# neel-dey/anatomix

Measured on AMD Instinct MI355X. Metric: 128^3 volumes/sec feature-extraction (6M UNet), higher is better.
Workload: dtype f16; 1 GPU; anatomix 6M UNet (ngf=16,num_downs=4) forward on sw_batch=4 windows of 1x128^3 (the predictor call of sliding_window_inference, BASELINE configs[1] / the metric); fp32 NCDHW in/out, 16-bit (f16) channels-last activations, fp32 accumulate; holds the 1e-3 tolerance against the fp32 reference in rel-L2 ONLY (max-norm 0.86e-3 .. 1.4e-3 by weight seed; the mode that holds both norms is value_strict); batch_per_gpu=4, window=128, parallelism=replicas x1 (no data-path collective)

## Files before the change

anatomix_amd/_lib.py:

```python
from __future__ import annotations

import ctypes as C
import os

_HERE = os.path.dirname(os.path.abspath(__file__))
LIB_PATH = os.environ.get("AMX_LIB_PATH") or os.path.join(_HERE, "csrc", "libanatomix_amd.so")

NORM = {"none": 0, "batch": 1, "instance": 2, "instance_affine": 3}
ACT = {"none": 0, "relu": 1, "lrelu": 2}
POOL = {"Max": 0, "Avg": 1}
INTERP = {"nearest": 0, "trilinear": 1}
WARP = {"bilinear": 0, "nearest": 1}
SEG_LABEL = {"float32": 0, "int64": 1, "uint8": 2}
SW_MAP = {"constant": 0, "gaussian": 1}
SW_OUT = {"features": 0, "logits": 1, "labels": 2}
PRECISION = {"f16": 0, "fp16": 0, "float16": 0, "bf16": 1, "bfloat16": 1, "f16x2": 2, "bf16x2": 3, "strict": 3, "fp32": 3,
             "f16x2mx": 4, "strict_mx": 4}


class UnetCfg(C.Structure):
    _fields_ = [
        ("input_nc", C.c_int32), ("output_nc", C.c_int32), ("num_downs", C.c_int32), ("ngf", C.c_int32),
        ("norm", C.c_int32), ("norm_eps", C.c_float), ("activation", C.c_int32), ("act_slope", C.c_float),
        ("final_act", C.c_int32), ("pooling", C.c_int32), ("interp", C.c_int32), ("doubleconv", C.c_int32),
        ("use_skip", C.c_int32), ("precision", C.c_int32),
    ]


class VitTap(C.Structure):
    _fields_ = [("name", C.c_char_p), ("d_dst", C.c_void_p), ("bytes", C.c_size_t), ("route", C.c_char * 160)]


class VitCfg(C.Structure):
    _fields_ = [
        ("input_channels", C.c_int32), ("num_classes", C.c_int32), ("embed_dim", C.c_int32), ("depth", C.c_int32),
        ("heads", C.c_int32), ("num_register_tokens", C.c_int32), ("grid_d", C.c_int32), ("grid_h", C.c_int32),
        ("grid_w", C.c_int32), ("hidden", C.c_int32), ("dec1", C.c_int32), ("dec2", C.c_int32), ("qk_norm", C.c_int32),
        ("scale_attn_inner", C.c_int32), ("layer_scale", C.c_int32), ("in_eps", C.c_float), ("out_norm", C.c_int32),
        ("decoder_split", C.c_int32), ("stem_split", C.c_int32),
    ]


_P = C.c_void_p
_I = C.c_int


class PackReq(C.Structure):
    _fields_ = [("d_weight", C.c_void_p), ("d_wpk", C.c_void_p), ("weight_mode", C.c_int32), ("cin_real", C.c_int32),
                ("cin_pad", C.c_int32), ("cout_real", C.c_int32), ("cout", C.c_int32), ("w", C.c_int32)]


WEIGHTS_PREPACKED = 16


class LaunchRecord(C.Structure):
    _fields_ = [("kernel", C.c_char * 64), ("module_idx", C.c_int32), ("cin", C.c_int32), ("cout", C.c_int32),
                ("n", C.c_int32), ("d", C.c_int32), ("h", C.c_int32), ("w", C.c_int32), ("ms", C.c_float),
                ("flops", C.c_double), ("bytes", C.c_double)]


SYMBOLS = {
    "amx_version": (_I, []),
    "amx_debug_fill_lds": (_I, [C.c_uint, _P]),
    "amx_last_error": (C.c_char_p, []),
    "amx_unet_create": (_I, [C.POINTER(_P), C.POINTER(UnetCfg)]),
    "amx_unet_destroy": (None, [_P]),
    "amx_unet_num_modules": (_I, [_P]),
    "amx_unet_num_convs": (_I, [_P]),
    "amx_unet_conv_info": (_I, [_P, _I, C.POINTER(_I), C.POINTER(_I), C.POINTER(_I), C.POINTER(_I)]),
    "amx_unet_load_conv": (_I, [_P, _I, _P, _P, _P, _P, _P, _P, _P]),
    "amx_unet_workspace_bytes": (C.c_size_t, [_P, _I, _I, _I, _I]),
    "amx_unet_forward": (_I, [_P, _P, _P, _I, _I, _I, _I, _P, C.c_size_t, _P]),
    "amx_unet_forward_profiled": (_I, [_P, _P, _P, _I, _I, _I, _I, _P, C.c_size_t, _P, C.POINTER(LaunchRecord), _I,
                                        C.POINTER(_I)]),
    "amx_unet_module_info": (_I, [_P, _I, C.POINTER(_I), C.POINTER(_I)]),
    "amx_unet_numerics_status": (_I, [_P, _I, _P]),
    "amx_unet_forward_taps": (_I, [_P, _P, _P, _I, _I, _I, _I, _P, C.c_size_t, C.POINTER(_I), _I, C.POINTER(_P), _I, _P]),
    "amx_unet_forward_window": (_I, [_P, _P, _I, _I, _I, _I, _I, _I, _I, _I, _I, _P, _P, _P, C.c_size_t, _P]),
    "amx_unet_forward_windows": (_I, [_P, _P, _I, _I, _I, _I, C.POINTER(C.c_int), _I, _I, _I, _P, _P, _P, C.c_size_t, _P]),
    "amx_unet_forward_windows_pipelined": (_I, [_P, _P, _I, _I, _I, _I, C.POINTER(C.c_int), _I, _I, _I, _P, _P, _P, C.c_size_t, _I, _P]),
    "amx_sw_normalize": (_I, [_P, _P, _I, C.c_longlong, _P]),
    "amx_sw_count": (_I, [_P, _I, _I, _I, _I, _I, _I, _I, _I, _I, _P, _P]),
    "amx_sw_plan": (_I, [_I, _I, _I, _I, _I, _I, C.c_double, C.POINTER(C.c_int), _I]),
    "amx_sw_importance_map": (_I, [_P, _I, _I, _I, _I, C.c_double, _P]),
    "amx_sw_count_all": (_I, [_P, _I, _I, _I, _I, _I, _I, C.c_double, _P, _P]),
    "amx_sw_finish": (_I, [_I, _P, _P, _I, C.c_longlong, _P, _P, _I, _P, _P]),
    "amx_sliding_window_workspace_bytes": (C.c_size_t, [_P, _I, _I, _I, _I]),
    "amx_sliding_window": (_I, [_P, _P, _I, _I, _I, _I, _I, _I, C.c_double, _I, C.c_double, _I, _I, _P, _P, _I, _P, _P, _P, _P,
                                C.c_size_t, _P]),
    "amx_conv3d_packed_bytes": (C.c_size_t, [_I, _I]),
    "amx_conv3d_k3_reflect": (_I, [_P, _I, _P, _I, _P, _P, _P, _I, _I, _I, _I, _I, _I, C.c_float, _I, _P, _P, _P, _P]),
    "amx_conv3d_k3_reflect_probe": (_I, [_P, _I, _P, _I, _P, _P, _P, _I, _I, _I, _I, _I, _I, C.c_float, _I, _P, _P, _P, _P, _P, _P, _P, _P]),
    "amx_conv3d_dgrad_interior_supported": (_I, [_I, _I, _I, _I, _I, _I]),
    "amx_conv3d_dgrad_interior": (_I, [_P, _I, _P, _I, _I, _I, _I, _I, _I, _I, _I, _I, _P, _P, _P]),
    "amx_conv3d_dgrad_shell_scratch_bytes": (C.c_size_t, []),
    "amx_conv3d_dgrad_fold_shell": (_I, [_P, _I, _P, _I, _I, _P, _I, _I, _I, _I, _I, _I, _P, _P]),
    "amx_conv3d_pack_batch": (_I, [C.POINTER(PackReq), _I, _I, _P]),
    "amx_conv3d_scratch_bytes": (C.c_size_t, [_I, _I, _I, _I, _I, _I, _I, _I]),
    "amx_conv3d_k3_reflect_ws": (_I, [_P, _I, _P, _I, _P, _P, _P, _I, _I, _I, _I, _I, _I, C.c_float, _I, _P, _P, _P, _P, C.c_size_t, _P]),
    "amx_conv3d_upcat_merged_packed_bytes": (C.c_size_t, [_I, _I, _I]),
    "amx_conv3d_upcat_merged": (_I, [_P, _I, _P, _I, _P, _P, _P, _I, _I, _I, _I, _I, _I, C.c_float, _I, _P, _P, _P, _P]),
    "amx_conv3d_k3_reflect_ex": (_I, [_P, _I, _P, _I, _P, _I, _I, _I, _P, _P, _I, _I, _I, _I, _I, _I, C.c_float, _I, _P, _P, _P, _P]),
    "amx_pool2": (_I, [_P, _P, _I, _I, _I, _I, _I, _I, _I, _P]),
    "amx_instance_norm_scratch_bytes": (C.c_size_t, [_I, _I]),
    "amx_instance_norm": (_I, [_P, _P, _P, C.c_float, _I, C.c_longlong, _I, _I, C.c_float, _P, _I, _P]),
    "amx_upsample2_trilinear": (_I, [_P, _P, _I, _I, _I, _I, _I, _I, _P]),
    "amx_upsample2_trilinear_backward": (_I, [_P, _P, _I, _I, _I, _I, _I, _I, _P]),
    "amx_upcat_split_backward": (_I, [_P, _P, _P, _I, _I, _I, _I, _I, _I, _I, _I, _P]),
    "amx_upcat_split_backward_framed": (_I, [_P, _P, _P, _I, _I, _I, _I, _I, _I, _I, _I, _P]),
    "amx_export_ncdhw": (_I, [_P, _I, _I, _I, _I, _I, _P, _I, _P]),
    "amx_import_ncdhw": (_I, [_P, _P, _I, _I, _I, _I, _I, C.c_longlong, C.c_longlong, C.c_longlong, C.c_longlong, _I, _I, _P]),
    "amx_train_scratch_bytes": (C.c_size_t, [_I]),
    "amx_bn_train_forward": (_I, [_P, _P, _P, _P, C.c_float, _I, C.c_longlong, _I, _I, C.c_float, _P, _P, _P, _P, _P,
                                  C.c_float, _I, _P]),
    "amx_bn_act_backward": (_I, [_P, _P, _P, _P, _P, _P, _P, _P, _P, _I, _I, _I, _I, _I, _I, C.c_float, _P, _I, _P]),
    "amx_bn_act_backward_recompute": (_I, [_P, _P, _P, _P, _P, _P, _P, _P, _P, _I, _I, _I, _I, _I, _I, C.c_float, _P, _I, _P]),
    "amx_pad_fold": (_I, [_P, _P, _I, _I, _I, _I, _I, _I, _I, _P]),
    "amx_adamw_step": (_I, [_P, _I, C.c_double, C.c_double, C.c_double, C.c_double, C.c_double, _I, _P]),
    "amx_adamw_step_dev": (_I, [_P, _I, _P, _I, _P]),
    "amx_adamw_step_clip_dev": (_I, [_P, _I, _P, _I, _P, C.c_double, _P]),
    "amx_grad_norms_scratch_bytes": (C.c_size_t, [_P, _I, _I]),
    "amx_grad_norms": (_I, [_P, _I, _I, _P, _P, C.c_size_t, _P]),
    "amx_pool2_max_backward": (_I, [_P, _P, _P, _I, _I, _I, _I, _I, _I, _I, _P]),
    "amx_conv3d_wgrad_scratch_bytes": (C.c_size_t, [_I, _I, _I, _I, _I, _I]),
    "amx_conv3d_wgrad": (_I, [_P, C.c_longlong, C.c_longlong, C.c_longlong, C.c_longlong, _P, _I, _P, _I, _I, _I, _I, _I, _I,
                              _I, _P, _I, _P, C.c_size_t, _I, _P]),
    "amx_attention_scratch_bytes": (C.c_size_t, [_I, _I, _I, _I]),
    "amx_attention_qknorm_rope": (_I, [_P, _P, _P, _P, _P, _P, _P, C.c_float, _P, _I, _I, _I, _I, _I, _P, _P, C.c_size_t, _P]),
    "amx_attention_prepared": (_I, [_P, C.c_size_t, _I, _I, _I, _I, _P, _P]),
    "amx_attention_train_scratch_bytes": (C.c_size_t, [_I, _I, _I, _I]),
    "amx_attention_qknorm_rope_train": (_I, [_P, _P, _P, _P, _P, _P, _P, C.c_float, _P, _I, _I, _I, _I, _I, _P, _P, _P, C.c_size_t, _P]),
    "amx_attention_backward": (_I, [_P, _P, _P, _P, _P, _P, _P, C.c_float, _P, _I, _I, _I, _I, _I, _P, _P, _P, _P, _P, _P, _P, _P, _P, _P,
                                    _P, C.c_size_t, _P]),
    "amx_vit_create": (_I, [C.POINTER(_P), C.POINTER(VitCfg)]),
    "amx_vit_destroy": (None, [_P]),
    "amx_vit_num_params": (_I, [_P]),
    "amx_vit_param_name": (C.c_char_p, [_P, _I]),
    "amx_vit_load": (_I, [_P, C.POINTER(_P), _I, _P, _P]),
    "amx_vit_workspace_bytes": (C.c_size_t, [_P, _I]),
    "amx_vit_forward": (_I, [_P, _P, _P, _I, _P, C.c_size_t, _I, _P]),
    "amx_vit_debug_read": (_I, [_P, C.c_char_p, _P, C.c_size_t, C.POINTER(C.c_size_t), _P]),
    "amx_vit_tap_bytes": (C.c_size_t, [_P, _I, C.c_char_p]),
    "amx_vit_forward_taps": (_I, [_P, _P, _P, _I, _P, C.c_size_t, _I, C.POINTER(VitTap), _I, _P]),
    "amx_vit_windows_workspace_bytes": (C.c_size_t, [_P, _I]),
    "amx_vit_forward_windows": (_I, [_P, _P, _I, _I, _I, _I, C.POINTER(C.c_int), _P, _P, _P, C.c_size_t, _P]),
    "amx_vit_sliding_window_workspace_bytes": (C.c_size_t, [_P, _I]),
    "amx_vit_sliding_window": (_I, [_P, _P, _I, _I, _I, C.c_double, _I, C.c_double, _I, _I, _P, _P, _I, _P, _P, _P, _P, C.c_size_t, _P]),
    "amx_linear": (_I, [_P, _P, _P, _I, _I, _I, _I, _P, _P]),
    "amx_supcon_scratch_bytes": (C.c_size_t, [_I, _I]),
    "amx_supcon_loss": (_I, [_P, _P, _I, _I, C.c_float, _I, _I, _I, _P, _P, _P, C.c_size_t, _P]),
    "amx_mlp_head_forward": (_I, [_P, _I, _I, _I, _I, _P, _P, _P, _P, _P, C.c_float, C.c_float, _I, C.c_float, _P, _P, _P, _P, _P]),
    "amx_mlp_head_scratch_bytes": (C.c_size_t, [_I, _I, _I]),
    "amx_mlp_head_backward": (_I, [_P, _P, _I, _I, _I, _I, _P, _P, _I, C.c_float, _P, _P, _P, _P, _P, _P, _P, _P, _P, C.c_size_t, _P]),
    "amx_mlp_heads_forward": (_I, [_I, _P, _I, _P, _I, _I, _P, _P, _P, _P, _P, C.c_float, C.c_float, _I, C.c_float, _P, _P, _P, _P, _P]),
    "amx_mlp_heads_backward": (_I, [_I, _P, _P, _I, _P, _I, _I, _P, _P, _I, C.c_float, _P, _P, _P, _P, _P, _P, _P, _P, _P, C.c_size_t, _P]),
    "amx_supcon_loss_batch": (_I, [_I, _P, _P, _I, _I, C.c_float, _I, _I, _I, _P, _P, _P, C.c_size_t, _P]),
    "amx_gather_labels_batch": (_I, [_P, _I, _I, _I, _I, _P, _I, _P, _I, _P, _P]),
    "amx_conv3d_backward_sampled_scratch_bytes": (C.c_size_t, [_I]),
    "amx_conv3d_backward_sampled": (_I, [_P, _P, _P, _I, _P, _I, _I, _I, _I, _I, _I, _I, _P, _P, _I, _P, C.c_size_t, _I, _P]),
    "amx_gather_rows": (_I, [_P, _I, C.c_longlong, C.c_longlong, C.c_longlong, C.c_longlong, C.c_longlong, _P, _I, _I, _I, _P, _P]),
    "amx_scatter_rows": (_I, [_P, _P, _P, _I, C.c_longlong, C.c_longlong, C.c_longlong, C.c_longlong, _I, _I, _I, _I, _P]),
    "amx_sample_coords": (_I, [_P, _I, _I, _I, _I, _I, _P, _P]),
    "amx_sample_perm": (_I, [_P, _I, _I, _I, _I, _P, _P]),
    "amx_import_input": (_I, [_P, _P, _I, _I, _I, _I, _I, _I, _P]),
    "amx_gather_labels": (_I, [_P, _I, _I, _I, _P, _I, _I, _I, _I, _I, _P, _P]),
    "amx_mindssc_scratch_bytes": (C.c_size_t, [_I, _I, _I]),
    "amx_mindssc": (_I, [_P, _I, _I, _I, _I, _I, _P, _P, C.c_size_t, _P]),
    "amx_avg_pool3d_cat": (_I, [_P, _I, C.c_float, _P, _I, C.c_float, _I, _I, _I, _I, _P, _P]),
    "amx_box_filter3d": (_I, [_P, _P, _I, _I, _I, _I, _I, _P]),
    "amx_correlate_scratch_bytes": (C.c_size_t, [_I, _I, _I, _I]),
    "amx_correlate_ssd": (_I, [_P, _P, _I, _I, _I, _I, _I, _P, _P, _P, C.c_size_t, _P]),
    "amx_coupled_convex_scratch_bytes": (C.c_size_t, [_I, _I, _I]),
    "amx_coupled_convex": (_I, [_P, _P, _I, _I, _I, _I, _P, _P, C.c_size_t, _P]),
    "amx_coupled_convex_step_scratch_bytes": (C.c_size_t, [_I, _I, _I]),
    "amx_coupled_convex_step": (_I, [_P, _P, _I, _I, _I, _I, _I, _P, _P, _P, C.c_size_t, _P]),
    "amx_inverse_consistency_scratch_bytes": (C.c_size_t, [_I, _I, _I]),
    "amx_inverse_consistency": (_I, [_P, _P, _I, _I, _I, _I, _P, _P, _P, C.c_size_t, _P]),
    "amx_resize_trilinear3d": (_I, [_P, _I, _I, _I, _I, _P, _I, _I, _I, C.POINTER(C.c_float), _I, _P]),
    "amx_stage1_registration_scratch_bytes": (C.c_size_t, [_I, _I, _I, _I, _I]),
    "amx_stage1_registration": (_I, [_P, _P, _I, _I, _I, _I, _I, _I, _I, _I, _I, _I, _P, _P, C.c_size_t, _P]),
    "amx_instance_opt_smooth3": (_I, [_P, _P, _I, _I, _I, _P]),
    "amx_instance_opt_scratch_bytes": (C.c_size_t, [_I, _I, _I, _I]),
    "amx_instance_opt_grad": (_I, [_P, _P, _P, _I, _I, _I, _I, C.c_float, _P, _P, _P, _P, C.c_size_t, _P]),
    "amx_instance_opt_adam_step": (_I, [_P, _P, _P, _P, C.c_longlong, C.c_double, _I, _P]),
    "amx_instance_opt": (_I, [_P, _P, _P, _I, _I, _I, _I, C.c_float, C.c_double, _I, _P, _P, C.c_size_t, _P]),
    "amx_run_instance_opt_scratch_bytes": (C.c_size_t, [_I, _I, _I, _I, _I, _I]),
    "amx_run_instance_opt": (_I, [_P, _P, _P, _I, _I, _I, _I, _I, C.c_float, _I, _I, C.c_double, _P, _P, C.c_size_t, _P]),
    "amx_warp3d": (_I, [_P, _I, _P, _I, _I, _I, _I, _P, _P]),
    "amx_seg_loss_scratch_bytes": (C.c_size_t, [_I, C.c_longlong, _I, _I]),
    "amx_seg_loss_forward": (_I, [_P, _I, _P, _P, _P, _I, _I, _I, C.c_longlong, _I, C.c_float, C.c_float, C.c_float, C.c_float, _P, _P,
                                  _P, _P, C.c_size_t, _P]),
    "amx_seg_loss_backward": (_I, [_P, _I, _P, _P, _P, _I, _I, _I, C.c_longlong, _I, C.c_float, C.c_float, C.c_float, C.c_float, _P, _P,
                                   _P, _P, _P, _P, C.c_size_t, _P]),
    "amx_seg_argmax": (_I, [_P, _I, _P, _P, _I, _I, C.c_longlong, _P, _P]),
    "amx_segaug_sample_bytes": (C.c_size_t, []),
    "amx_segaug_scratch_bytes": (C.c_size_t, [_I, C.c_longlong]),
    "amx_segaug_minmax": (_I, [_P, _I, C.c_longlong, _P, _P, C.c_size_t, _P]),
    "amx_segaug_minmax_finalize": (_I, [_P, C.c_size_t, _I, C.c_longlong, _P, _P]),
    "amx_segaug_pointwise": (_I, [_P, _P, _I, C.c_longlong, _P, _I, _P, _P, _P]),
    "amx_segaug_crop": (_I, [_I, _I, _I, _I, _P, _I, _P, _P, _P, _P, _P]),
    "amx_segaug_gaussian": (_I, [_P, _P, _P, _I, _I, _I, _I, _I, _P, _P, _P]),
    "amx_segaug_affine": (_I, [_P, _P, _I, _I, _I, _I, _P, _P, _I, _I, _I, _P, _P, _P, C.c_size_t, _P]),
    "amx_preaug_view_bytes": (C.c_size_t, []),
    "amx_preaug_spatial": (_I, [_P, _P, _I, _I, _I, _I, _P, _P, _P, _P, _P, _P]),
    "amx_preaug_blur": (_I, [_P, _P, _P, _I, _I, _I, _I, _P, _P, _P]),
    "amx_preaug_intensity": (_I, [_P, _P, _P, _I, _I, _I, _I, _P, _P, _P]),
    "amx_synth_view_bytes": (C.c_size_t, []),
    "amx_synth_scratch_bytes": (C.c_size_t, [_I, C.c_longlong]),
    "amx_synth_gmm_minmax": (_I, [_P, _P, _I, C.c_longlong, _P, _P, _P, C.c_size_t, _P]),
    "amx_synth_appearance": (_I, [_P, _P, C.POINTER(_P), C.POINTER(_I), _I, _P, _P, _I, _I, _I, _I, _P, _P, _P, C.c_size_t, _P]),
    "amx_synth_logk_mean": (_I, [_P, _I, C.c_longlong, _P, _P, C.c_size_t, _P]),
    "amx_synth_spike": (_I, [_P, _P, _I, _P, _I, _I, _I, _I, _P, _P, _P]),
    "amx_synth_lowres": (_I, [_P, _P, _I, _I, _I, _I, _P, _P, _P]),
    "amx_synth_clip_minmax": (_I, [_P, _I, C.c_longlong, _P, C.c_size_t, _P]),
    "amx_synth_finish": (_I, [_P, _P, _I, C.c_longlong, _P, _I, _P]),
    "amx_labels_template_bytes": (C.c_size_t, []),
    "amx_labels_ensemble_bytes": (C.c_size_t, []),
    "amx_labels_scratch_bytes": (C.c_size_t, [_I, C.c_longlong]),
    "amx_labels_compose": (_I, [_P, C.c_size_t, _P, _P, _I, _P, _P, _P, _I, _I, _I, _I, _P]),
    "amx_labels_median3": (_I, [_P, _P, _I, _I, _I, _I, _I, _P, _P, _P]),
    "amx_labels_sphere_mask": (_I, [C.POINTER(_P), _P, _I, _I, _P, _P, _P]),
    "amx_labels_apply_mask": (_I, [_P, _P, _P, _I, C.c_longlong, _P, _P, _P, C.c_size_t, _P]),
    "amx_labels_envelope": (_I, [_P, _P, _P, _I, _I, _I, _I, _P, _P, _P]),
    "amx_labels_merge_masks": (_I, [_P, _I, C.c_longlong, C.c_longlong, C.POINTER(_I), _P, _P, _P, _I, _P]),
    "amx_label_overlap": (_I, [_P, _I, _P, _I, C.c_longlong, _I, _P, _P, _P]),
    "amx_jacobian_det_scratch_bytes": (C.c_size_t, [_I, _I, _I]),
    "amx_jacobian_det": (_I, [_P, _I, _I, _I, _I, _P, _P, _P, C.c_size_t, _P]),
}

_lib = None


AMX_ERR_INVALID, AMX_ERR_SHAPE, AMX_ERR_NOT_LOADED, AMX_ERR_WORKSPACE, AMX_ERR_HIP, AMX_ERR_OVERFLOW = -1, -2, -3, -4, -5, -6


class AmxError(RuntimeError):

    def __init__(self, *args):
        self.code = args[0] if args and isinstance(args[0], int) else None
        super().__init__(*(args[1:] if self.code is not None else args))


class AmxEnvelopeError(AmxError):
    """The configuration lies outside what an engine entry covers (AMX_ERR_INVALID / AMX_ERR_SHAPE at create time)."""

# ... 52 lines not shown
```

anatomix_amd/csrc/amx_api.hip:

```cpp
#include <stdarg.h>
#include <stdio.h>
#include <string.h>

#include <string>
#include <vector>

#include "amx_launch.h"

static thread_local std::string g_err;

int amx::fail(int code, const char* fmt, ...) {
  char buf[512];
  va_list ap;
  va_start(ap, fmt);
  vsnprintf(buf, sizeof buf, fmt, ap);
  va_end(ap);
  g_err = buf;
  return code;
}

using namespace amx;

extern "C" {

// ... 119 lines not shown
    p.up_shift = 1;
  }
  p.wpk = (const char*)d_wpk;
  p.bias = d_shift;
  p.act = act; p.slope = slope;
  if (d_out16) {
    amx::set_out(p, d_out16, cout, d, hh, w, precision);
  } else {
    p.out32 = d_out32;
    p.py = w; p.pz = (long long)hh * w; p.pc = p.pz * d; p.pn = p.pc * cout;
  }
  amx::ConvLaunchInfo info{};
  amx::ConvLaunchInfo* const want = probe ? &info : nullptr;
  if (probe) {
    p.wmap = probe->wmap;
    p.oflow = probe->oflow;
    if (probe->wmap && !d_out32) return fail(AMX_ERR_INVALID, "the importance map belongs to the fp32 planar output");
    if (probe->pool16) {
      if (!d_out16 || !amx::conv_zmarch_can_pool(p)) return fail(AMX_ERR_SHAPE, "the fused max-pool needs a z-march layer with even extents");
      amx::set_out2(p, probe->pool16, cout, d / 2, hh / 2, w / 2, precision);
    }
  }
  if (!is_split(precision) && weight_mode == 0 && cin_real == 48 && c0 == 16 && c1 == 32 && cout == 16 && amx::conv_upcat16_eligible(p)) {
    if (prepacked)
      return fail(AMX_ERR_INVALID, "prepacked weights: the 16 + up32 -> 16 merged-tap layer packs its own format (call without the flag)");
    char* up = (char*)d_wpk + ((size_t)cout * (c0 + c1) * 28 * 2 + 255) / 256 * 256;
    AMX_HIP(amx::launch_pack_upcat16(d_weight, d_scale, up, precision, st));
    p.wpk = up;
    AMX_HIP(amx::launch_conv_upcat16(p, precision, st, want));
    if (probe && probe->kernel) memcpy(probe->kernel, info.name, sizeof info.name);
    return AMX_OK;
  }
  if (d_scratch && !c1 && d_out16) {
    const size_t need = amx::conv_ks_part_bytes(c0, cout, n, d, hh, w, precision, q);
    if (need && (scratch_bytes < need || ((uintptr_t)d_scratch & 15)))
      return fail(AMX_ERR_WORKSPACE, "split-K scratch needs %zu bytes, 16-byte aligned (got %zu)", need, scratch_bytes);
    if (need) p.part = (float*)d_scratch;
  }
  AMX_HIP(amx::launch_conv(p, precision, q, st, want));
  if (probe && probe->kernel) memcpy(probe->kernel, info.name, sizeof info.name);
  return AMX_OK;
}

static bool dgrad_interior_shape_ok(int c_dy, int cout, int d, int hh, int w, int precision) {
  if (precision != AMX_PREC_F16 && precision != AMX_PREC_BF16) return false;
  amx::ConvParams p;
  memset(&p, 0, sizeof p);
  p.C0 = c_dy; p.Cout = cout; p.D = d; p.H = hh; p.W = w; p.out = (char*)1;
  return amx::conv_zmarch_eligible(p) && amx::conv_pick_q(cout, w, precision) == cout / 16 && (size_t)27 * c_dy * cout * 4 <= 150 * 1024;
}

int amx_conv3d_dgrad_interior_supported(int c_dy, int cout, int d, int hh, int w, int precision) {
  return dgrad_interior_shape_ok(c_dy, cout, d, hh, w, precision) ? 1 : 0;
}

int amx_conv3d_dgrad_interior(const void* d_dy_framed, int c_dy, const float* d_weight, int weight_flags, int cin_real, int cout_real, int cout,
                              int n, int d, int hh, int w, int precision, void* d_wpk, void* d_out16, void* stream) {
  if (!d_dy_framed || !d_wpk || !d_out16 || (!d_weight && !(weight_flags & AMX_WEIGHTS_PREPACKED)))
    return fail(AMX_ERR_INVALID, "dgrad_interior: bad pointer arguments");
  if (!dgrad_interior_shape_ok(c_dy, cout, d, hh, w, precision))
    return fail(AMX_ERR_INVALID, "dgrad_interior: shape outside the z-march kernels (ask amx_conv3d_dgrad_interior_supported)");
  if (cin_real < 1 || cin_real > c_dy || cout_real < 1 || cout_real > cout) return fail(AMX_ERR_INVALID, "dgrad_interior: bad weight description");
  hipStream_t st = (hipStream_t)stream;
  const int q = cout / 16;
  if (!(weight_flags & AMX_WEIGHTS_PREPACKED))
    AMX_HIP(amx::launch_pack_weights(d_weight, nullptr, d_wpk, cin_real, c_dy, cout, q, precision, st, 1, cout_real));
  amx::ConvParams p;
  memset(&p, 0, sizeof p);
  p.N = n; p.D = d; p.H = hh; p.W = w; p.Cout = cout; p.C0 = c_dy;
  p.s0x = (long long)c_dy * 2; p.s0y = p.s0x * (w + 4); p.s0z = p.s0y * (hh + 4); p.s0n = p.s0z * (d + 4);
  p.src0 = (const char*)d_dy_framed + 2 * (p.s0z + p.s0y + p.s0x);
  p.raw_halo = 1;
  p.wpk = (const char*)d_wpk;
  p.act = AMX_ACT_NONE;
  p.out = (char*)d_out16;
  p.ox = (long long)cout * 2; p.oy = p.ox * w; p.oz = p.oy * hh; p.on = p.oz * d;
  AMX_HIP(amx::launch_conv(p, precision, q, st));
  return AMX_OK;
}

size_t amx_conv3d_dgrad_shell_scratch_bytes(void) { return amx::dgrad_shell_scratch_bytes(); }

int amx_conv3d_dgrad_fold_shell(const void* d_dy_framed, int c_dy, const float* d_weight, int co_real, int ci_real, void* d_dx, int c_dx, int n,
                                int d, int hh, int w, int precision, void* d_scratch, void* stream) {
  if (!d_dy_framed || !d_weight || !d_dx || !d_scratch || ((uintptr_t)d_scratch & 15) || co_real < 1 || co_real > c_dy || ci_real < 1 || ci_real > c_dx || d < 2 || hh < 2 || w < 2)
    return fail(AMX_ERR_INVALID, "dgrad_fold_shell: bad arguments");
  const long long fx = (long long)c_dy * 2, fy = fx * (w + 4), fz = fy * (hh + 4), fn = fz * (d + 4);
  AMX_HIP(amx::launch_dgrad_fold_shell((const char*)d_dy_framed + 2 * (fz + fy + fx), fn, fz, fy, fx, c_dy, d_weight, co_real, ci_real, d_dx, c_dx,
                                       n, d, hh, w, precision, d_scratch, (hipStream_t)stream));
  return AMX_OK;
}

int amx_conv3d_pack_batch(const amx_pack_req* reqs, int count, int precision, void* stream) {
  if (!reqs || count < 1 || count > 256 || (precision != AMX_PREC_F16 && precision != AMX_PREC_BF16))
    return fail(AMX_ERR_INVALID, "pack_batch: bad arguments");
  std::vector<const float*> w(count);
  std::vector<void*> wpk(count);
  std::vector<int> cr(count), cp(count), co(count), q(count), md(count), cor(count);
  for (int i = 0; i < count; ++i) {
    const amx_pack_req& r = reqs[i];
    if (!r.d_weight || !r.d_wpk || r.cin_pad % 16 || r.cin_pad < 16 || r.cout % 16 || r.cout < 16 || r.cin_real < 1 || r.cin_real > r.cin_pad ||
        r.cout_real < 1 || r.cout_real > r.cout || (r.weight_mode != 0 && r.weight_mode != 1))
      return fail(AMX_ERR_INVALID, "pack_batch: bad request %d", i);
    w[i] = r.d_weight; wpk[i] = r.d_wpk; cr[i] = r.cin_real; cp[i] = r.cin_pad; co[i] = r.cout; md[i] = r.weight_mode; cor[i] = r.cout_real;
    q[i] = amx::conv_pick_q(r.cout, r.w, precision);
  }
  AMX_HIP(amx::launch_pack_weights_batch(count, w.data(), wpk.data(), cr.data(), cp.data(), co.data(), q.data(), md.data(), cor.data(), precision,
                                         (hipStream_t)stream));
  return AMX_OK;
}

size_t amx_conv3d_scratch_bytes(int c0, int c1, int cout, int n, int d, int hh, int w, int precision) {
  if (c1 || c0 % 16 || cout % 16 || precision < AMX_PREC_F16 || precision > AMX_PREC_F16X2_MX) return 0;
  return amx::conv_ks_part_bytes(c0, cout, n, d, hh, w, precision, amx::conv_pick_q(cout, w, precision));
}

int amx_conv3d_k3_reflect_ws(const void* d_x0, int c0, const void* d_x1, int c1, const float* d_weight,
                             const float* d_scale, const float* d_shift, int cout, int n, int d, int hh, int w,
                             int act, float slope, int precision, void* d_wpk, void* d_out16, float* d_out32,
                             void* d_scratch, size_t scratch_bytes, void* stream) {
  return conv3d_single(d_x0, c0, d_x1, c1, d_weight, 0, c0 + c1, cout, d_scale, d_shift, cout, n, d, hh, w, act, slope,
                       precision, d_wpk, d_out16, d_out32, stream, d_scratch, scratch_bytes);
}

int amx_conv3d_k3_reflect_probe(const void* d_x0, int c0, const void* d_x1, int c1, const float* d_weight, const float* d_scale,
                                const float* d_shift, int cout, int n, int d, int hh, int w, int act, float slope, int precision,
                                void* d_wpk, void* d_out16, float* d_out32, void* d_pool16, const float* d_wmap, int* d_oflow,
                                char* kernel_name, void* stream) {
  const ConvProbe probe{d_pool16, d_wmap, d_oflow, kernel_name};
  return conv3d_single(d_x0, c0, d_x1, c1, d_weight, 0, c0 + c1, cout, d_scale, d_shift, cout, n, d, hh, w, act, slope,
                       precision, d_wpk, d_out16, d_out32, stream, nullptr, 0, &probe);
}

int amx_conv3d_k3_reflect(const void* d_x0, int c0, const void* d_x1, int c1, const float* d_weight,
                          const float* d_scale, const float* d_shift, int cout, int n, int d, int hh, int w,
                          int act, float slope, int precision, void* d_wpk, void* d_out16, float* d_out32,
                          void* stream) {
  return conv3d_single(d_x0, c0, d_x1, c1, d_weight, 0, c0 + c1, cout, d_scale, d_shift, cout, n, d, hh, w, act, slope,
                       precision, d_wpk, d_out16, d_out32, stream);
}

int amx_conv3d_k3_reflect_ex(const void* d_x0, int c0, const void* d_x1, int c1, const float* d_weight, int weight_mode,
                             int cin_real, int cout_real, const float* d_scale, const float* d_shift, int cout, int n,
                             int d, int hh, int w, int act, float slope, int precision, void* d_wpk, void* d_out16,
                             float* d_out32, void* stream) {
  return conv3d_single(d_x0, c0, d_x1, c1, d_weight, weight_mode, cin_real, cout_real, d_scale, d_shift, cout, n, d, hh, w,
                       act, slope, precision, d_wpk, d_out16, d_out32, stream);
}

size_t amx_conv3d_upcat_merged_packed_bytes(int c0, int c1, int cout) {
  return 2 * (align_up((size_t)cout * c0 * 28 * 2, 256) + amx::conv_upmerge_packed_bytes(c1, cout, 0));
}

int amx_conv3d_upcat_merged(const void* d_x0, int c0, const void* d_x1, int c1, const float* d_weight, const float* d_scale,
                            const float* d_shift, int cout, int n, int d, int hh, int w, int act, float slope, int precision,
                            void* d_wpk, void* d_partial, void* d_out16, void* stream) {
  if (!d_x0 || !d_x1 || !d_weight || !d_wpk || !d_partial || !d_out16) return fail(AMX_ERR_INVALID, "null argument");
  if (precision < AMX_PREC_F16 || precision > AMX_PREC_BF16X2) return fail(AMX_ERR_INVALID, "unsupported precision %d", precision);
  const bool split = is_split(precision);
  if (c0 != cout || !amx::conv_upmerge_eligible(c0, c1, cout, d, hh, w, 1, split))
    return fail(AMX_ERR_INVALID, "merged concat conv needs c0 == cout >= 32 (16 in the strict precisions), c1 %% 32 == 0, w >= 16, even dims "
                "(c0=%d c1=%d cout=%d dims %d,%d,%d)", c0, c1, cout, d, hh, w);
  hipStream_t st = (hipStream_t)stream;
  const int q = amx::conv_pick_q(cout, w, precision);
  char* wmerge = (char*)d_wpk + align_up((size_t)cout * c0 * 28 * 2 * (split ? 2 : 1), 256);
  AMX_HIP(amx::launch_pack_weights(d_weight, d_scale, d_wpk, c0, c0, cout, q, precision, st, 0, 0, c0 + c1));
  AMX_HIP(amx::launch_pack_upmerge(d_weight, d_scale, wmerge, c0, c0 + c1, c1, cout, precision, st));
  amx::ConvParams p;
  memset(&p, 0, sizeof p);
  p.N = n; p.D = d; p.H = hh; p.W = w; p.Cout = cout;
  amx::set_src0(p, d_x0, c0, d, hh, w, precision);
  p.wpk = (const char*)d_wpk; p.act = AMX_ACT_NONE;
  amx::set_out(p, d_partial, cout, d, hh, w, precision);
  AMX_HIP(amx::launch_conv(p, precision, q, st));
  amx::UpmergeParams u;
  memset(&u, 0, sizeof u);
  amx::set_src(u, d_x1, c1, d / 2, hh / 2, w / 2, precision);
  u.N = n; u.LD = d / 2; u.LH = hh / 2; u.LW = w / 2; u.Cout = cout;
  u.wpk = wmerge; u.part = (const char*)d_partial; u.out = (char*)d_out16;
  u.bias = d_shift; u.act = act; u.slope = slope;
  AMX_HIP(amx::launch_conv_upmerge(u, precision, st));
  return AMX_OK;
}

int amx_pool2(const void* d_in, void* d_out, int n, int dout, int hout, int wout, int c, int avg, int precision,
              void* stream) {
  if (!d_in || !d_out || c % 8) return fail(AMX_ERR_INVALID, "bad argument");
  AMX_HIP(amx::launch_pool2(d_in, d_out, n, dout, hout, wout, c, avg, precision, (hipStream_t)stream));
  return AMX_OK;
}

size_t amx_train_scratch_bytes(int c) { return amx::train_scratch_bytes(c); }

int amx_bn_train_forward(const void* d_x, void* d_y, const float* d_gamma, const float* d_beta, float eps, int n,
                         long long voxels, int c, int act, float slope, void* d_scratch, float* d_save_mean,
                         float* d_save_rstd, float* d_running_mean, float* d_running_var, float momentum, int precision,
                         void* stream) {
  if (!d_x || !d_y || !d_scratch || n < 1 || voxels < 1 || c % 8 || c > 2048) return fail(AMX_ERR_INVALID, "bad argument");
  AMX_HIP(amx::launch_bn_train_forward(d_x, d_y, d_gamma, d_beta, eps, (long long)n * voxels, c, act, slope, d_scratch, d_save_mean,
                                       d_save_rstd, d_running_mean, d_running_var, momentum, precision, (hipStream_t)stream));
  return AMX_OK;
}

int amx_bn_act_backward(const void* d_dy, const void* d_y, const void* d_x, const float* d_mean, const float* d_rstd,
                        const float* d_gamma, float* d_dgamma, float* d_dbeta, void* d_dx_framed, int n, int d, int hh, int w,
                        int c, int act, float slope, void* d_scratch, int precision, void* stream) {
  if (!d_dy || !d_y || !d_dx_framed || !d_scratch || c % 8 || c > 2048) return fail(AMX_ERR_INVALID, "bad argument");
  if (d_mean && (!d_x || !d_rstd || !d_dgamma || !d_dbeta)) return fail(AMX_ERR_INVALID, "norm backward needs x, rstd, dgamma, dbeta");
  AMX_HIP(amx::launch_bn_act_backward(d_dy, d_y, d_x ? d_x : d_y, d_mean, d_rstd, d_gamma, nullptr, d_dgamma, d_dbeta, d_dx_framed, n,
                                      d, hh, w, c, act, slope, d_scratch, precision, (hipStream_t)stream));
  return AMX_OK;
}

int amx_bn_act_backward_recompute(const void* d_dy, const void* d_x, const float* d_mean, const float* d_rstd, const float* d_gamma,
                                  const float* d_beta, float* d_dgamma, float* d_dbeta, void* d_dx_framed, int n, int d, int hh, int w,
                                  int c, int act, float slope, void* d_scratch, int precision, void* stream) {
  if (!d_dy || !d_x || !d_mean || !d_rstd || !d_dgamma || !d_dbeta || !d_dx_framed || !d_scratch || c % 8 || c > 2048)
    return fail(AMX_ERR_INVALID, "bad argument");
  AMX_HIP(amx::launch_bn_act_backward(d_dy, nullptr, d_x, d_mean, d_rstd, d_gamma, d_beta, d_dgamma, d_dbeta, d_dx_framed, n, d, hh, w,
                                      c, act, slope, d_scratch, precision, (hipStream_t)stream));
  return AMX_OK;
}

int amx_pad_fold(const void* d_g_framed, void* d_din, int n, int d, int hh, int w, int c, int accumulate, int precision,
                 void* stream) {
  if (!d_g_framed || !d_din || c % 8 || d < 2 || hh < 2 || w < 2) return fail(AMX_ERR_INVALID, "bad argument");
  AMX_HIP(amx::launch_pad_fold(d_g_framed, d_din, n, d, hh, w, c, accumulate, precision, (hipStream_t)stream));
  return AMX_OK;
}

int amx_adamw_step(const amx_adamw_tensor* tensors, int count, double lr, double beta1, double beta2, double eps, double weight_decay,
                   int maximize, void* stream) {
  static_assert(sizeof(amx_adamw_tensor) == 48, "six 64-bit fields");
  if (count < 0 || (count && !tensors)) return fail(AMX_ERR_INVALID, "bad argument");
  if (!(lr >= 0.0) || !(eps >= 0.0) || !(beta1 >= 0.0 && beta1 < 1.0) || !(beta2 >= 0.0 && beta2 < 1.0) || !(weight_decay >= 0.0))
    return fail(AMX_ERR_INVALID, "adamw: lr %g, betas (%g, %g), eps %g, weight_decay %g out of range", lr, beta1, beta2, eps, weight_decay);
  for (int t = 0; t < count; ++t) {
    const amx_adamw_tensor& r = tensors[t];
    if (!r.param || !r.grad || !r.exp_avg || !r.exp_avg_sq || !r.step || r.numel < 0)
      return fail(AMX_ERR_INVALID, "adamw: tensor %d has a null pointer or a negative size", t);
  }
  AMX_HIP(amx::launch_adamw((const long long*)tensors, count, lr, beta1, beta2, eps, weight_decay, maximize, (hipStream_t)stream));
  return AMX_OK;
}

int amx_adamw_step_dev(const amx_adamw_tensor* tensors, int count, const double* d_hyper, int maximize, void* stream) {
  if (count < 0 || (count && !tensors) || !d_hyper) return fail(AMX_ERR_INVALID, "bad argument");
  for (int t = 0; t < count; ++t) {
    const amx_adamw_tensor& r = tensors[t];
    if (!r.param || !r.grad || !r.exp_avg || !r.exp_avg_sq || !r.step || r.numel < 0)
      return fail(AMX_ERR_INVALID, "adamw: tensor %d has a null pointer or a negative size", t);
  }
  AMX_HIP(amx::launch_adamw((const long long*)tensors, count, 0.0, 0.0, 0.0, 0.0, 0.0, maximize, (hipStream_t)stream, d_hyper));
  return AMX_OK;
}

int amx_adamw_step_clip_dev(const amx_adamw_tensor* tensors, int count, const double* d_hyper, int maximize, const float* d_total_norm,
                            double max_norm, void* stream) {
  if (count < 0 || (count && !tensors) || !d_hyper || !d_total_norm || !(max_norm >= 0.0))
    return fail(AMX_ERR_INVALID, "adamw: bad argument (max_norm %g)", max_norm);
  for (int t = 0; t < count; ++t) {
    const amx_adamw_tensor& r = tensors[t];
    if (!r.param || !r.grad || !r.exp_avg || !r.exp_avg_sq || !r.step || r.numel < 0)
      return fail(AMX_ERR_INVALID, "adamw: tensor %d has a null pointer or a negative size", t);
  }
  AMX_HIP(amx::launch_adamw((const long long*)tensors, count, 0.0, 0.0, 0.0, 0.0, 0.0, maximize, (hipStream_t)stream, d_hyper, d_total_norm,
                            max_norm));
  return AMX_OK;
}

size_t amx_grad_norms_scratch_bytes(const amx_grad_tensor* tensors, int count, int groups) {
  static_assert(sizeof(amx_grad_tensor) == 24, "three 64-bit fields");
  if (count < 0 || groups < 0 || (count && !tensors)) return 0;
  return amx::grad_norms_scratch_bytes((const long long*)tensors, count, groups);
}

int amx_grad_norms(const amx_grad_tensor* tensors, int count, int groups, float* d_out, void* d_scratch, size_t scratch_bytes,
                   void* stream) {
  if (count < 0 || groups < 0 || (count && !tensors) || (groups && !d_out) || !d_scratch) return fail(AMX_ERR_INVALID, "bad argument");
  for (int t = 0; t < count; ++t)
    if (!tensors[t].grad && tensors[t].numel) return fail(AMX_ERR_INVALID, "grad_norms: tensor %d has a null pointer", t);
  if (amx_grad_norms_scratch_bytes(tensors, count, groups) == 0 || scratch_bytes < amx_grad_norms_scratch_bytes(tensors, count, groups))
    return fail(AMX_ERR_INVALID, "grad_norms: a negative size, a group outside [0, %d), too many blocks, or too little scratch", groups);
  AMX_HIP(amx::launch_grad_norms((const long long*)tensors, count, groups, d_out, d_scratch, scratch_bytes, (hipStream_t)stream));
  return AMX_OK;
}

int amx_pool2_max_backward(const void* d_dp, const void* d_in, void* d_din, int n, int dout, int hout, int wout, int c,
                           int accumulate, int precision, void* stream) {
  if (!d_dp || !d_in || !d_din || c % 8) return fail(AMX_ERR_INVALID, "bad argument");
  AMX_HIP(amx::launch_pool2_max_backward(d_dp, d_in, d_din, n, dout, hout, wout, c, accumulate, precision, (hipStream_t)stream));
  return AMX_OK;
}

size_t amx_conv3d_wgrad_scratch_bytes(int n, int d, int hh, int w, int cout, int cin_pad) {
  return amx::wgrad_scratch_bytes(n, d, hh, w, cout, cin_pad);
}

int amx_conv3d_wgrad(const void* d_dy, long long dy_sn, long long dy_sz, long long dy_sy, long long dy_sx, const void* d_x0,
                     int c0, const void* d_x1, int c1, int cin_real, int cout, int n, int d, int hh, int w, float* d_dw,
                     int accumulate, void* d_scratch, size_t scratch_bytes, int precision, void* stream) {
  if (!d_dy || !d_x0 || !d_dw || !d_scratch) return fail(AMX_ERR_INVALID, "null argument");
  if (c0 % 16 || c1 % 16 || c0 + c1 < 16 || cout % 16 || cout < 16 || cin_real < 1 || cin_real > c0 + c1)
    return fail(AMX_ERR_INVALID, "channel counts must be multiples of 16 (c0=%d c1=%d cout=%d)", c0, c1, cout);
  if (c1 && (!d_x1 || (d & 1) || (hh & 1) || (w & 1))) return fail(AMX_ERR_SHAPE, "upsampled segment needs even dims");
  if (d < 2 || hh < 2 || w < 2 || w > 128) return fail(AMX_ERR_SHAPE, "wgrad supports 2 <= w <= 128 (got %d)", w);
  if (scratch_bytes < amx::wgrad_scratch_bytes(n, d, hh, w, cout, c0 + c1))
    return fail(AMX_ERR_WORKSPACE, "scratch needs %zu bytes", amx::wgrad_scratch_bytes(n, d, hh, w, cout, c0 + c1));
  amx::WgradParams p;
  memset(&p, 0, sizeof p);
  p.dy = (const char*)d_dy; p.yn = dy_sn; p.yz = dy_sz; p.yy = dy_sy; p.yx = dy_sx;
  amx::set_src0(p, d_x0, c0, d, hh, w, AMX_PREC_F16);
  if (c1) {
    amx::set_src1(p, d_x1, c1, d / 2, hh / 2, w / 2, AMX_PREC_F16);
    p.up_shift = 1;
  }
  p.N = n; p.D = d; p.H = hh; p.W = w; p.Cout = cout;
  AMX_HIP(amx::launch_wgrad(p, cin_real, d_dw, accumulate, d_scratch, precision, (hipStream_t)stream));
  return AMX_OK;
}

size_t amx_attention_scratch_bytes(int b, int heads, int n, int head_dim) {
  if (b < 1 || heads < 1 || n < 1 || head_dim < 2 || head_dim > 80) return 0;
  return amx::attention_scratch_bytes(b, heads, n);
}

int amx_attention_qknorm_rope(const float* d_q, const float* d_k, const float* d_v, const float* d_qn_w, const float* d_qn_b,
                              const float* d_kn_w, const float* d_kn_b, float norm_eps, const float* d_rope, int n_prefix, int b,
                              int n, int heads, int head_dim, float* d_out, void* d_scratch, size_t scratch_bytes, void* stream) {
  if (!d_q || !d_k || !d_v || !d_out || !d_scratch) return fail(AMX_ERR_INVALID, "null argument");
  if (b < 1 || n < 1 || heads < 1 || head_dim < 2 || head_dim > 80 || (head_dim & 1))
    return fail(AMX_ERR_INVALID, "attention: head_dim must be even and <= 80 (got %d), b, n, heads >= 1", head_dim);
  if ((!d_qn_w) != (!d_qn_b) || (!d_kn_w) != (!d_kn_b)) return fail(AMX_ERR_INVALID, "attention: norm weight and bias go together");
  if (n_prefix < 0 || n_prefix > n) return fail(AMX_ERR_INVALID, "attention: 0 <= n_prefix <= n");
  if (scratch_bytes < amx::attention_scratch_bytes(b, heads, n) || ((uintptr_t)d_scratch & 15))
// ... 400 lines not shown
```

anatomix_amd/csrc/amx_common.h:

```cpp
#pragma once
#include <hip/hip_runtime.h>
#include <stdint.h>
#include <stdlib.h>

namespace amx {

typedef _Float16 f16;
typedef __bf16 bf16;
typedef __attribute__((ext_vector_type(8))) _Float16 f16x8;
typedef __attribute__((ext_vector_type(8))) __bf16 bf16x8;
typedef __attribute__((ext_vector_type(4))) float f32x4;

constexpr int kSteps = 14;

__host__ __device__ constexpr int tapA_index(int s) {
  return s < 9 ? s * 3 : (s < 12 ? (s - 9) * 9 + 2 : (s == 12 ? 8 : 26));
}
__host__ __device__ constexpr int tapB_index(int s) {
  return s < 9 ? s * 3 + 1 : (s < 12 ? (s - 9) * 9 + 5 : (s == 12 ? 17 : -1));
}

enum Act { ACT_NONE = 0, ACT_RELU = 1, ACT_LRELU = 2 };

struct DeviceOnce {
  unsigned long long mask = 0;
  int dev = 0;
  bool done() {
    if (hipGetDevice(&dev) != hipSuccess) dev = 64;
    return dev < 64 && ((mask >> dev) & 1);
  }
  void set() {
    if (dev < 64) mask |= 1ull << dev;
  }
};

struct ConvParams {
  const char* src0;
  const char* src1;
  long long s0n, s0z, s0y, s0x;
  long long s1n, s1z, s1y, s1x;
  int C0, C1;
  int src0_f32c1;
  int up_shift;
  const char* wpk;
  const float* bias;
  char* out;
  long long on, oz, oy, ox;
  float* out32;
  long long pn, pc, pz, py;
  const float* wmap;
  int N, D, H, W, Cout;
  int act;
  float slope;
  int nbz, nby, nbx;
  float* stats;
  char* out2;
  long long qn, qz, qy, qx;
  int* oflow;
  int dbg;
  const int* mxs;
  int raw_halo;
  float* part;
  int kslices;
  int cs0, cs1, ocs;
};

__host__ __device__ constexpr int fmt_of_precision(int precision) { return precision < 2 ? 0 : (precision == 4 ? 2 : 1); }
__host__ __device__ constexpr int fmt_elem_bytes(int fmt) { return fmt == 0 ? 2 : (fmt == 1 ? 4 : 6); }

inline void pick_z_segments(int tiles, int D, int unit, int slots, int* zseg_out, int* nseg_out) {
  const int fill = 6;
  long long best = -1;
  int bz = D, bn = 1;
  for (int n = 1; n <= 32; ++n) {
    int zs = (D + n - 1) / n;
    zs = (zs + unit - 1) / unit * unit;
    if (zs < 8) zs = 8;
    const int ns = (D + zs - 1) / zs;
    const long long rounds = ((long long)tiles * ns + slots - 1) / slots;
    const long long score = rounds * (zs + fill);
    if (best < 0 || score < best) {
      best = score;
      bz = zs;
      bn = ns;
    }
  }
  *zseg_out = bz;
  *nseg_out = bn;
}

struct UpmergeParams {
  const char* src;
  long long sn, sz, sy, sx;
  int C1;
  int N, LD, LH, LW, Cout;
  const char* wpk;
  const char* part;
  char* out;
  const float* bias;
  int act;
  float slope;
  int nbz, nby, nbx;
  int* oflow;
  int dbg;
  int cs, ocs;
};

constexpr int MLP_MAXB = 8;

struct WgradParams {
  const char* dy;
  long long yn, yz, yy, yx;
  const char* src0;
  long long s0n, s0z, s0y, s0x;
  const char* src1;
  long long s1n, s1z, s1y, s1x;
  int C0, C1, up_shift;
  int N, D, H, W, Cout;
  float* partial;
  int nchunk, items_per_chunk, nitems, nyt;
  int nxt, ppc, cpx, nplanes;
  int dbg;
  float* dw;
  int cin_real, accumulate;
};

}
```

anatomix_amd/csrc/amx_conv3d_ks.hip:

```cpp
#include <stdlib.h>
#include <string.h>

#include "amx_device.h"
#include "amx_launch.h"

namespace amx {

template <int TZ_, int TY_, int TX_, int Q_, int QP_, int CPW_, int KW_, int CW_, int TEAMS_, int NH_, int NBUF_ = 2>
struct KsCfg {
  static constexpr int TZ = TZ_, TY = TY_, TX = TX_, Q = Q_, QP = QP_, CPW = CPW_, KW = KW_, CW = CW_, TEAMS = TEAMS_, NH = NH_, NBUF = NBUF_;
  static constexpr int WGS_PER_CU = NBUF == 1 ? 2 : 1;
  static constexpr int NWAVE = KW * CW * TEAMS;
  static constexpr int LX = TX >= 16 ? 16 : 8;
  static constexpr bool ZPAIR = LX == 8;
  static constexpr int XT = TX / LX, YT = TY, ZT = ZPAIR ? TZ / 2 : TZ;
  static constexpr int NVT = ZT * YT * XT;
  __host__ __device__ static constexpr int tile_z(int i) { return ZPAIR ? (i >> 1) * 4 + (i & 1) : i; }
  static constexpr int HZ = TZ + 2, HY = TY + 2, HX = TX + 2, HV = HZ * HY * HX;
  static constexpr int PLANE = (HV * 16 + 255) / 256 * 256;
  static constexpr int CHBUF = 2 * PLANE;
  static constexpr int NPK = (HV + 63) / 64;
  static constexpr int NPKW = (NPK + CW - 1) / CW;
  static constexpr int HALO_BYTES = TEAMS * KW * NBUF * CHBUF;
  static constexpr int NVTG = NVT / NH;
  static constexpr int OWN = NVTG / KW;
  static constexpr int SCR_MAX = 160 * 1024 / WGS_PER_CU - HALO_BYTES;
  static constexpr int pick_rt() {
    for (int r = OWN; r >= 1; --r)
      if (OWN % r == 0 && TEAMS * CW * KW * (KW - 1) * r * Q * 1024 <= SCR_MAX) return r;
    return 0;
  }
  static constexpr int RT = pick_rt();
  static constexpr int ROUNDS = RT ? OWN / RT : 0;
  static constexpr int SCR_GROUP = KW * (KW - 1) * RT * Q * 1024;
  static constexpr int SCR_BYTES = TEAMS * CW * SCR_GROUP;
  static constexpr int LDS_BYTES = HALO_BYTES + SCR_BYTES;
  static_assert(NVT % NH == 0 && NVTG % KW == 0, "every wave finalises the same number of column tiles of every group");
  static_assert(NH == 1 || CPW == 1, "tile groups re-read the stage's halo: one chunk per wave and brick");
  static_assert(CW == 1 || CPW == 1, "shared halo buffers are ordered by the per-brick reduction barriers: one stage per brick");
  static_assert(RT >= 1, "the reduction scratch must fit behind the halo buffers");
  static_assert(TX % LX == 0 && (!ZPAIR || TZ % 4 == 0), "the brick must tile into 16-voxel columns");
  static_assert(Q * kSteps * CPW * 4 <= (NWAVE * WGS_PER_CU > 4 ? 112 : 224), "the stationary A fragments must leave room for accumulators and B fragments");
  static_assert(NBUF == 2 || (NBUF == 1 && CPW == 1 && CW == 1), "the un-prefetched form stages one chunk per wave and brick, privately");
  static_assert((CW * Q) % QP == 0 || QP % Q == 0, "a wave's cout tiles lie inside one packed cout group");
};

struct KsBrick {
  int n, z0, y0, x0;
};

template <typename T, typename C, bool PART>
__global__ __launch_bounds__(C::NWAVE * 64, C::NWAVE * C::WGS_PER_CU / 4) void conv3d_k3_ks_kernel(const ConvParams p) {
  typedef typename Ops<T>::vec8 vec8;
  constexpr int Q = C::Q, QP = C::QP, CPW = C::CPW, KW = C::KW, CW = C::CW, TEAMS = C::TEAMS, NVTG = C::NVTG, NH = C::NH;
  constexpr int HY = C::HY, HX = C::HX, PLANE = C::PLANE, CHBUF = C::CHBUF, NPK = C::NPK, NPKW = C::NPKW;
  constexpr int LX = C::LX, XT = C::XT, YT = C::YT, OWN = C::OWN, RT = C::RT, ROUNDS = C::ROUNDS;

  extern __shared__ __attribute__((aligned(16))) char smem[];

  const int tid = threadIdx.x, lane = tid & 63;
  const int wave = __builtin_amdgcn_readfirstlane(tid >> 6);
  const int team = wave / (KW * CW), k = (wave - team * (KW * CW)) / CW, cw = wave % CW;
  const int li = lane & 15, g = lane >> 4;

  const int ncg = p.Cout / (16 * Q * CW);
  const int S = p.kslices > 0 ? p.kslices : 1;
  const int combos = ncg * S;
  const int G = gridDim.x, wpc = G / combos;
  int L = blockIdx.x;
  if ((G & 7) == 0) L = (L & 7) * (G >> 3) + (L >> 3);
  const int combo = L / wpc, run = L - combo * wpc;
  const int slice = combo / ncg, cg = combo - slice * ncg;
  const int nbricks = p.nbz * p.nby * p.nbx * p.N;
  const int b0 = (int)((long long)nbricks * run / wpc), b1 = (int)((long long)nbricks * (run + 1) / wpc);
  const int niter = (b1 - b0 + TEAMS - 1) / TEAMS;
  if (niter <= 0) return;
  const int nchunk = p.C0 >> 4;
  const int ch0 = slice * (KW * CPW) + k * CPW;
  const int cs = p.cs0 ? p.cs0 : 32;
  const int tile0 = (cg * CW + cw) * Q;
  const int pg = tile0 / QP, q0 = tile0 - pg * QP;

  const int dzl = C::ZPAIR ? (li >> 3) * 2 : 0;
  const int dx = C::ZPAIR ? (li & 7) : li;
  const int lanebase = (g & 1) * PLANE + (dzl * HY * HX + dx) * 16;
  const int hi = g >> 1;
  const int base_d1 = lanebase + hi * 16;
  const int base_dx = lanebase + hi * 16 * HX;
  const int base_dz = lanebase + hi * 16 * HX * HY;
  const int base_d0 = lanebase;

  int pk_off[NPKW];
#pragma unroll
  for (int m = 0; m < NPKW; ++m) pk_off[m] = 0;
  char* const halo = smem + (team * KW + k) * (C::NBUF * CHBUF);
  char* const scratch = smem + C::HALO_BYTES + (team * CW + cw) * C::SCR_GROUP;

  auto decode = [&](int b) {
    KsBrick r;
    const int bx = b % p.nbx;
    b /= p.nbx;
    const int by = b % p.nby;
    b /= p.nby;
    const int bz = b % p.nbz;
    r.n = b / p.nbz;
    r.z0 = bz * C::TZ;
    r.y0 = by * C::TY;
    r.x0 = bx * C::TX;
    return r;
  };
  auto offsets = [&](const KsBrick& br) {
#pragma unroll
    for (int m = 0; m < NPKW; ++m) {
      const int hv = (m * CW + cw) * 64 + lane;
      const int hz = hv / (HY * HX), rem = hv - hz * (HY * HX), hy = rem / HX, hx = rem - hy * HX;
      const int gz = reflect_clamp(br.z0 + hz - 1, p.D), gy = reflect_clamp(br.y0 + hy - 1, p.H);
      const int gx = reflect_clamp(br.x0 + hx - 1, p.W);
      pk_off[m] = hv < C::HV ? gz * (int)p.s0z + gy * (int)p.s0y + gx * (int)p.s0x : -1;
    }
  };
#define AMX_DMA16(src, dst) dma16_asm((const void*)(src), (unsigned)__builtin_amdgcn_readfirstlane((int)lds_addr(dst)))
  auto issue = [&](const KsBrick& br, int cp, int bsel) {
    const char* base = p.src0 + (long long)br.n * p.s0n + (long long)(ch0 + cp) * cs;
    char* dst = halo + bsel * CHBUF;
#pragma unroll
    for (int m = 0; m < NPKW; ++m) {
      const int j = m * CW + cw;
      if (j < NPK && pk_off[m] >= 0) {
        AMX_DMA16(base + pk_off[m], dst + j * 1024);
        AMX_DMA16(base + pk_off[m] + 16, dst + PLANE + j * 1024);
      }
    }
  };

  constexpr int dbg = 0;

  int sink = 0;
  {
    const long long range_bytes = (long long)KW * CPW * kSteps * QP * 1024;
    const char* wrange = p.wpk + ((long long)pg * nchunk + slice * (KW * CPW)) * (kSteps * QP * 1024);
    const int nparts = (int)((range_bytes + 8191) >> 13);
    const long long off = (long long)((run * C::NWAVE + wave) % nparts) * 8192 + lane * 128;
    if (off < range_bytes && !(dbg & 32)) asm volatile("global_load_dword %0, %1, off" : "=v"(sink) : "v"(wrange + off) : "memory");
  }

  const int cb = pg * 16 * QP + g * 4 * QP + q0 * 4;

  KsBrick cu = decode(b0 + team), nx = cu;
  bool cu_valid = b0 + team < b1;
  if (cu_valid) {
    offsets(cu);
    issue(cu, 0, 0);
  }
  vec8 wa[CPW][kSteps][Q];
  {
    const char* wbase = p.wpk + ((((long long)pg * nchunk + ch0) * kSteps) * QP + q0) * 1024 + lane * 16;
#pragma unroll
    for (int cp = 0; cp < CPW; ++cp)
#pragma unroll
      for (int s = 0; s < kSteps; ++s)
#pragma unroll
        for (int q = 0; q < Q; ++q) wa[cp][s][q] = *(const vec8*)(wbase + ((cp * kSteps + s) * QP + q) * 1024);
  }
  constexpr int NA = Q * kSteps * CPW;
  if (dbg & 64) asm volatile("s_waitcnt vmcnt(0)" ::: "memory");
  else asm volatile("s_waitcnt vmcnt(%0)" ::"n"(NA) : "memory");
  static_assert(NA <= 63, "vmcnt is a 6-bit counter");
  asm volatile("" ::"v"(sink));
  if (CW > 1) __syncthreads();

  f32x4 acc[NVTG][Q];
  int t = 0;
  for (int it = 0; it < niter; ++it) {
    const int bn = b0 + (it + 1) * TEAMS + team;
    const bool nx_valid = it + 1 < niter && bn < b1;
    if (nx_valid) nx = decode(bn);
    const bool full = cu_valid && (cu.z0 + C::TZ <= p.D) & (cu.y0 + C::TY <= p.H) & (cu.x0 + C::TX <= p.W);
#pragma unroll
    for (int h = 0; h < NH; ++h) {
#pragma unroll
      for (int cp = 0; cp < CPW; ++cp) {
        if (h == 0 && C::NBUF == 1) {
          if (it > 0 && cu_valid && !(dbg & 1)) {
            offsets(cu);
            issue(cu, 0, 0);
            asm volatile("s_waitcnt vmcnt(0)" ::: "memory");
          }
        } else if (h == 0) {
          if (dbg & 1) {
          } else if (cp + 1 < CPW) {
            if (cu_valid) issue(cu, cp + 1, (t + cp + 1) & 1);
          } else if (nx_valid) {
            offsets(nx);
            issue(nx, 0, (t + cp + 1) & 1);
          }
        }
        if (cp == 0) {
#pragma unroll
          for (int c = 0; c < NVTG; ++c)
#pragma unroll
            for (int q = 0; q < Q; ++q) acc[c][q] = f32x4{0.f, 0.f, 0.f, 0.f};
        }
        if (cu_valid && !(dbg & 2)) {
          const char* buf = halo + (C::NBUF == 1 ? 0 : ((t + cp) & 1) * CHBUF);
          constexpr int P = Q >= 4 ? 4 : 6, R = P + 1, NU = kSteps * NVTG;
          vec8 fb[R];
          auto load_item = [&](const int u) {
            const int s = u / NVTG, c = h * NVTG + (u - s * NVTG);
            const int kz = s < 9 ? s / 3 : (s < 12 ? s - 9 : (s == 12 ? 0 : 2));
            const int ky = s < 9 ? s % 3 : (s < 12 ? 0 : 2);
            const int kx = s < 9 ? 0 : 2;
            const int tapoff = ((kz * HY + ky) * HX + kx) * 16;
            const int bsel = s < 9 ? base_d1 : (s < 12 ? base_dx : (s == 12 ? base_dz : base_d0));
            const int cx = c % XT, cy = (c / XT) % YT, cz = c / (XT * YT);
            const int coff = ((C::tile_z(cz) * HY + cy) * HX + cx * LX) * 16;
            fb[u % R] = *(const vec8*)(buf + bsel + tapoff + coff);
          };
#pragma unroll
          for (int u = 0; u < P; ++u) load_item(u);
#pragma unroll
          for (int u = 0; u < NU; ++u) {
            if (u + P < NU) load_item(u + P);
            __builtin_amdgcn_sched_barrier(0);
            const int s = u / NVTG, c = u - s * NVTG;
#pragma unroll
            for (int q = 0; q < Q; ++q) acc[c][q] = Ops<T>::mfma(wa[cp][s][q], fb[u % R], acc[c][q]);
            __builtin_amdgcn_sched_barrier(0);
          }
        }
        if (h == NH - 1) {
          asm volatile("s_waitcnt vmcnt(0)" ::: "memory");
        }
      }

      f32x4 bq[Q];
#pragma unroll
      for (int q = 0; q < Q; ++q)
        bq[q] = (!PART && p.bias) ? *(const f32x4*)(p.bias + cb + q * 4) : f32x4{0.f, 0.f, 0.f, 0.f};
#pragma unroll
      for (int r = 0; r < ROUNDS; ++r) {
        if (dbg & 16) {
          __syncthreads();
          __syncthreads();
          continue;
        }
#pragma unroll
        for (int o = 0; o < KW; ++o) {
          if (o != k && cu_valid) {
            const int slot = k < o ? k : k - 1;
            char* dst = scratch + ((o * (KW - 1) + slot) * RT * Q) * 1024 + lane * 16;
#pragma unroll
            for (int i = 0; i < RT; ++i)
#pragma unroll
              for (int q = 0; q < Q; ++q) *(f32x4*)(dst + (i * Q + q) * 1024) = acc[o * OWN + r * RT + i][q];
          }
        }
        __syncthreads();
#pragma unroll
        for (int o = 0; o < KW; ++o) {
          if (o == k && cu_valid) {
            bool bad = false;
#pragma unroll
            for (int i = 0; i < RT; ++i) {
              f32x4 v[Q];
#pragma unroll
              for (int w2 = 0; w2 < KW; ++w2) {
                const int slot = w2 < o ? w2 : w2 - 1;
                const char* src = scratch + ((o * (KW - 1) + slot) * RT * Q) * 1024 + lane * 16;
#pragma unroll
                for (int q = 0; q < Q; ++q) {
                  const f32x4 x = w2 == o ? acc[o * OWN + r * RT + i][q] : *(const f32x4*)(src + (i * Q + q) * 1024);
                  v[q] = w2 == 0 ? x : v[q] + x;
                }
              }
              if (!PART) {
#pragma unroll
                for (int q = 0; q < Q; ++q) v[q] += bq[q];
                act_inplace<Q>(&v[0], p.act, p.slope);
              }
              const int c = h * NVTG + o * OWN + r * RT + i;
              const int cx = c % XT, cy = (c / XT) % YT, cz = c / (XT * YT);
              const int zl = cu.z0 + C::tile_z(cz) + dzl, yl = cu.y0 + cy, xl = cu.x0 + cx * LX + dx;
              if (!full && !((zl < p.D) & (yl < p.H) & (xl < p.W))) continue;
              if (PART) {
                const long long vox = (((long long)cu.n * p.D + zl) * p.H + yl) * p.W + xl;
                float* d = p.part + ((long long)slice * p.N * p.D * p.H * p.W + vox) * p.Cout + cb;
#pragma unroll
                for (int q = 0; q < Q; ++q) *(f32x4*)(d + q * 4) = v[q];
              } else {
                const int ocs = p.ocs ? p.ocs : 32;
                char* d = p.out + (long long)cu.n * p.on + (long long)zl * p.oz + (long long)yl * p.oy + (long long)xl * p.ox +
                          (long long)(cb >> 4) * ocs + (cb & 15) * 2;
                unsigned pk[2 * Q];
#pragma unroll
                for (int q = 0; q < Q; ++q) {
#pragma unroll
                  for (int j = 0; j < 4; ++j)
                    if (RangeCheck<T>::on) bad |= RangeCheck<T>::bad(v[q][j]);
                  pk[2 * q] = (unsigned)to_bits<T>(v[q][0]) | ((unsigned)to_bits<T>(v[q][1]) << 16);
                  pk[2 * q + 1] = (unsigned)to_bits<T>(v[q][2]) | ((unsigned)to_bits<T>(v[q][3]) << 16);
                }
                if (Q == 1) {
                  *(uint2*)d = make_uint2(pk[0], pk[1]);
                } else {
#pragma unroll
                  for (int j = 0; j < Q / 2; ++j) *(uint4*)(d + j * 16) = make_uint4(pk[4 * j], pk[4 * j + 1], pk[4 * j + 2], pk[4 * j + 3]);
                }
              }
            }
            if (!PART && RangeCheck<T>::on) raise_flag(p.oflow, bad);
          }
        }
        __syncthreads();
      }
    }
    t += CPW;
    cu = nx;
    cu_valid = nx_valid;
  }
#undef AMX_DMA16
}

template <typename T>
__global__ void splitk_reduce_kernel(const float* __restrict__ part, int S, const float* __restrict__ bias, char* __restrict__ out,
                                     long long on, long long oz, long long oy, long long ox, int ocs, int N, int D, int H, int W,
                                     int Cout, int act, float slope, int* oflow) {
  const int c8n = Cout >> 3;
  const long long nvox = (long long)N * D * H * W, total = nvox * c8n;
  const float kact = act_k(act, slope);
  bool bad = false;
  for (long long idx = blockIdx.x * (long long)blockDim.x + threadIdx.x; idx < total; idx += (long long)gridDim.x * blockDim.x) {
    const int c8 = (int)(idx % c8n);
    const long long vox = idx / c8n;
    const float* src = part + vox * Cout + c8 * 8;
    float v[8];
#pragma unroll
    for (int e = 0; e < 8; ++e) v[e] = 0.f;
    for (int s = 0; s < S; ++s) {
      const float4 a = *(const float4*)(src + (long long)s * nvox * Cout), b = *(const float4*)(src + (long long)s * nvox * Cout + 4);
      v[0] += a.x; v[1] += a.y; v[2] += a.z; v[3] += a.w;
      v[4] += b.x; v[5] += b.y; v[6] += b.z; v[7] += b.w;
    }
    unsigned o[4];
#pragma unroll
    for (int e = 0; e < 8; ++e) {
      v[e] = act_fwd(v[e] + (bias ? bias[c8 * 8 + e] : 0.f), kact);
      if (RangeCheck<T>::on) bad |= RangeCheck<T>::bad(v[e]);
    }
#pragma unroll
    for (int e = 0; e < 4; ++e) o[e] = (unsigned)to_bits<T>(v[2 * e]) | ((unsigned)to_bits<T>(v[2 * e + 1]) << 16);
    long long r = vox;
    const int x = (int)(r % W);
    r /= W;
    const int y = (int)(r % H);
    r /= H;
    const int z = (int)(r % D);
    const int n = (int)(r / D);
    char* d = out + (long long)n * on + (long long)z * oz + (long long)y * oy + (long long)x * ox + (long long)(c8 >> 1) * (ocs ? ocs : 32) +
              (c8 & 1) * 16;
    *(uint4*)d = make_uint4(o[0], o[1], o[2], o[3]);
  }
  if (RangeCheck<T>::on) raise_flag(oflow, bad);
}

template <typename T, typename C, bool PART>
static hipError_t launch_ks_cfg(ConvParams p, hipStream_t st, ConvLaunchInfo* info) {
  if (info)
    info->report(0, "conv3d_k3_ks<%s,%dx%dx%d,q%d,k%dx%d,c%d,t%d,h%d,b%d%s>", __is_same(T, f16) ? "f16" : "bf16", C::TZ, C::TY, C::TX, C::Q,
                 C::KW, C::CPW, C::CW, C::TEAMS, C::NH, C::NBUF, PART ? ",part" : "");
  auto kern = conv3d_k3_ks_kernel<T, C, PART>;
  static amx::DeviceOnce attr_once;
  if (!attr_once.done()) {
    hipError_t e = hipFuncSetAttribute((const void*)kern, hipFuncAttributeMaxDynamicSharedMemorySize, C::LDS_BYTES);
    if (e != hipSuccess) return e;
    attr_once.set();
  }
  const int cus = device_cus(attr_once.dev);
  if (cus == 0) return hipErrorUnknown;
  p.nbz = (p.D + C::TZ - 1) / C::TZ;
  p.nby = (p.H + C::TY - 1) / C::TY;
  p.nbx = (p.W + C::TX - 1) / C::TX;
  const int nbricks = p.nbz * p.nby * p.nbx * p.N;
  const int S = p.kslices > 0 ? p.kslices : 1;
  const int combos = p.Cout / (16 * C::Q * C::CW) * S;
  int wpc = cus * C::WGS_PER_CU / combos;
  if (wpc < 1) wpc = 1;
  const int runs = (nbricks + C::TEAMS - 1) / C::TEAMS;
  if (wpc > runs) wpc = runs;
  const unsigned grid = (unsigned)(combos * wpc);
  hipLaunchKernelGGL(kern, dim3(grid), dim3(C::NWAVE * 64), C::LDS_BYTES, st, p);
  return hipGetLastError();
}

struct KsPlan {
  int ok, kw, cpw, teams, slices, cw;
};
static KsPlan ks_plan(const ConvParams& p, int precision, int Q, bool can_split) {
  KsPlan r = {0, 0, 0, 0, 1, 1};
  if (precision > 1 || p.C1 != 0 || p.src0_f32c1 || p.out32 || p.out2 || p.stats || !p.out || p.W < 8 || p.H < 2 || p.D < 2) return r;
  if ((long long)p.D * p.s0z >= (1ll << 31)) return r;
  const int nchunk = p.C0 >> 4;
  if (p.C0 & 15) return r;
  const int tz = p.W >= 16 ? 2 : 4, ty = 4, tx = p.W >= 16 ? 16 : 8;
  const long long nbricks = (long long)((p.D + tz - 1) / tz) * ((p.H + ty - 1) / ty) * ((p.W + tx - 1) / tx) * p.N;
  const int ncg = p.Cout / (16 * Q);
  if (Q == 4) {
    if (p.W < 16) return r;
    if (nchunk == 2) { r = {1, 2, 1, 2, 1, 2}; return r; }
    if (nchunk == 4) { r = {1, 4, 1, 1, 1, 2}; return r; }
    return r;
  }
  if (Q != 2) return r;
  auto cw_of = [&](int slices) { return (p.Cout % 64 == 0 && (long long)(p.Cout / 64) * slices * nbricks >= 200) ? 2 : 1; };
  if (nchunk == 4) { r = {1, 4, 1, 1, 1, cw_of(1)}; return r; }
  if (nchunk % 8 == 0 && can_split) {
    const int s8 = nchunk / 8;
    if ((long long)ncg * nbricks >= 192) return r;
    if (s8 >= 2 && (long long)ncg * s8 * nbricks >= 192 && s8 <= 8) { r = {1, 4, 2, 1, s8, 1}; return r; }
    if (s8 * 2 <= 16) { r = {1, 4, 1, 1, s8 * 2, cw_of(s8 * 2)}; return r; }
  }
  return r;
}

bool conv_ks_eligible(const ConvParams& p, int precision, int Q) {
  return ks_plan(p, precision, Q, p.part != nullptr).ok != 0;
}

size_t conv_ks_part_bytes(int C0, int Cout, int N, int D, int H, int W, int precision, int Q) {
  ConvParams p;
  memset(&p, 0, sizeof p);
  p.C0 = C0; p.Cout = Cout; p.N = N; p.D = D; p.H = H; p.W = W; p.out = (char*)1;
  p.s0z = (long long)H * W * C0 * 2;
  const KsPlan pl = ks_plan(p, precision, Q, true);
  if (!pl.ok || pl.slices <= 1) return 0;
  return (size_t)pl.slices * N * D * H * W * Cout * sizeof(float);
}

template <typename T>
static hipError_t launch_ks_t(ConvParams p, const KsPlan& pl, int Q, hipStream_t st, ConvLaunchInfo* info) {
  const bool wide = p.W >= 16;
  p.kslices = pl.slices;
  const bool part = pl.slices > 1;
  hipError_t e = hipErrorInvalidValue;
#define AMX_KS(TZ, TY, TX, QW, QP, CPW, KW, CW, TEAMS, NH, ...)                              \
  do {                                                                                       \
    typedef KsCfg<TZ, TY, TX, QW, QP, CPW, KW, CW, TEAMS, NH, ##__VA_ARGS__> CC;             \
    e = part ? launch_ks_cfg<T, CC, true>(p, st, info) : launch_ks_cfg<T, CC, false>(p, st, info);      \
  } while (0)
  if (Q == 4 && pl.kw == 2) {
    if (wide) AMX_KS(2, 4, 16, 2, 4, 1, 2, 2, 2, 2);
  } else if (Q == 4) {
    if (wide) AMX_KS(2, 4, 16, 2, 4, 1, 4, 2, 1, 2);
  } else if (pl.cpw == 2) {
    if (wide) AMX_KS(2, 4, 16, 2, 2, 2, 4, 1, 1, 1); else AMX_KS(4, 4, 8, 2, 2, 2, 4, 1, 1, 1);
  } else {
    if (pl.cw == 2) {
      if (wide) AMX_KS(2, 4, 16, 2, 2, 1, 4, 2, 1, 2); else AMX_KS(4, 4, 8, 2, 2, 1, 4, 2, 1, 2);
    } else {
      if (wide) AMX_KS(2, 4, 16, 2, 2, 1, 4, 1, 1, 1); else AMX_KS(4, 4, 8, 2, 2, 1, 4, 1, 1, 1);
    }
  }
#undef AMX_KS
  if (e != hipSuccess || !part) return e;
  const long long total = (long long)p.N * p.D * p.H * p.W * (p.Cout / 8);
  const int blocks = (int)((total + 255) / 256 > 2048 ? 2048 : (total + 255) / 256);
  hipLaunchKernelGGL(splitk_reduce_kernel<T>, dim3(blocks), dim3(256), 0, st, p.part, pl.slices, p.bias, p.out, p.on, p.oz, p.oy, p.ox,
                     p.ocs, p.N, p.D, p.H, p.W, p.Cout, p.act, p.slope, p.oflow);
  return hipGetLastError();
}

hipError_t launch_conv_ks(const ConvParams& p, int precision, int Q, hipStream_t st, ConvLaunchInfo* info) {
  const KsPlan pl = ks_plan(p, precision, Q, p.part != nullptr);
  if (!pl.ok) return hipErrorInvalidValue;
  return precision == 0 ? launch_ks_t<f16>(p, pl, Q, st, info) : launch_ks_t<bf16>(p, pl, Q, st, info);
}

}
```

anatomix_amd/csrc/amx_conv3d_upmerge.hip:

```cpp
#include <stdlib.h>

#include "amx_device.h"
#include "amx_launch.h"

namespace amx {


template <int Q, int TZ, int TY, int NBUF, int KS, bool SPLIT = false, int LXT = 16>
struct UpmCfg {
  static_assert(LXT == 16 || LXT == 8, "a tile is 16 cells of one low-res row, or 8 cells of two rows (rows shorter than 16)");
  static constexpr int RPT = 16 / LXT;
  static constexpr int BY = TY * RPT;
  static constexpr int NP = SPLIT ? 2 : 1;
  static_assert(!SPLIT || KS == 1, "strict precision: 32-channel stages");
  static constexpr int T = TZ * TY;
  static constexpr int HZ = TZ + 2, HY = BY + 2, HX = LXT + 2, HV = HZ * HY * HX;
  static constexpr int PL = ((HV * 16 + 255) / 256) * 256;
  static constexpr int BUF = 4 * KS * NP * PL;
  static constexpr int NJ = (HV + 63) / 64;
  static constexpr int NDMA = 4 * KS * NP * NJ;
  static constexpr int PER_WAVE = (NDMA + 7) / 8;
  static constexpr int LDS_BYTES = NBUF * BUF;
  static_assert(LDS_BYTES <= 160 * 1024, "ring must fit the LDS");
};

template <typename T_, int Q, int TZ, int TY, int NBUF, int KS, bool SPLIT, int LXT>
__global__ __launch_bounds__(512) void conv3d_upmerge_kernel(const UpmergeParams p) {
  typedef UpmCfg<Q, TZ, TY, NBUF, KS, SPLIT, LXT> C;
  constexpr int RPT = C::RPT, BY = C::BY;
  constexpr int NP = C::NP;
  typedef typename Ops<T_>::vec8 vec8;
  constexpr int HY = C::HY, HX = C::HX, PL = C::PL, NT = C::T;
  extern __shared__ __attribute__((aligned(16))) char smem[];

  const int tid = threadIdx.x, lane = tid & 63;
  const int wave = __builtin_amdgcn_readfirstlane(tid >> 6);
  const int li = lane & 15, g = lane >> 4;
  const int lix = li & (LXT - 1), liy = LXT == 8 ? li >> 3 : 0;
  const int pz = wave >> 2, py = (wave >> 1) & 1, px = wave & 1;

  const int nbricks = p.nbz * p.nby * p.nbx * p.N;
  const int ncg = p.Cout / (16 * Q);
  const int items = nbricks * ncg;
  const int G = gridDim.x;
  int jw = blockIdx.x;
  if ((G & 7) == 0) jw = (jw & 7) * (G >> 3) + (jw >> 3);
  const int it0 = (int)((long long)items * jw / G), it1 = (int)((long long)items * (jw + 1) / G);
  const int nstage = p.C1 / (32 * KS);
  const int T_total = (it1 - it0) * nstage;
  if (T_total <= 0) return;

  struct Item { int bx, by, bz, n, cg; };
  auto decode = [&](int it) {
    Item r;
    r.cg = it / nbricks;
    int b = it - r.cg * nbricks;
    r.bx = b % p.nbx; b /= p.nbx;
    r.by = b % p.nby; b /= p.nby;
    r.bz = b % p.nbz;
    r.n = b / p.nbz;
    return r;
  };

  int dma_item = -1;
  int off[C::PER_WAVE];
  auto issue = [&](int it, int stage, int bsel) {
    const Item I = decode(it);
    if (it != dma_item) {
      dma_item = it;
#pragma unroll
      for (int m = 0; m < C::PER_WAVE; ++m) {
        const int id = wave + 8 * m;
        const int j = id % C::NJ;
        const int hv = j * 64 + lane;
        const int hz = hv / (HY * HX), rem = hv - hz * (HY * HX), hy = rem / HX, hx = rem - hy * HX;
        int gz = I.bz * TZ - 1 + hz, gy = I.by * BY - 1 + hy, gx = I.bx * LXT - 1 + hx;
        gz = gz < 0 ? 0 : (gz >= p.LD ? p.LD - 1 : gz);
        gy = gy < 0 ? 0 : (gy >= p.LH ? p.LH - 1 : gy);
        gx = gx < 0 ? 0 : (gx >= p.LW ? p.LW - 1 : gx);
        off[m] = hv < C::HV ? gz * (int)p.sz + gy * (int)p.sy + gx * (int)p.sx : -1;
      }
    }
    const char* base = p.src + (long long)I.n * p.sn;
    const int cs = p.cs ? p.cs : 32;
    char* buf = smem + bsel * C::BUF;
#pragma unroll
    for (int m = 0; m < C::PER_WAVE; ++m) {
      const int id = wave + 8 * m;
      if (id < C::NDMA) {
        const int plane = id / C::NJ, j = id - plane * C::NJ;
        const int cbyte = stage * (64 * KS) + (SPLIT && plane >= 4 ? p.C1 * 2 + (plane - 4) * 16 : plane * 16);
        if (off[m] >= 0)
          dma16_asm(base + off[m] + (long long)(cbyte >> 5) * cs + (cbyte & 31),
                    (unsigned)__builtin_amdgcn_readfirstlane((int)lds_addr(buf + plane * PL + j * 1024)));
      }
    }
  };

  auto wptr = [&](int it, int stage) -> const char* {
    const int cg = it / nbricks;
    return p.wpk + ((((long long)cg * nstage * KS + stage * KS) * 8 + wave) * 8 * NP * Q) * 1024 + lane * 16;
  };
  auto woff = [](const int e2) { return ((e2 >> 3) * 64 + (e2 & 7)) * NP * Q * 1024; };
  constexpr int NTAP = 8 * KS;
  constexpr int WIN = 4;
  vec8 wq[WIN][NP][Q];
  const int lbase = g * PL + ((pz * HY + py + liy) * HX + px + lix) * 16;

  f32x4 acc[NT][Q];
  int nx_it = it0, nx_stage = 0;
  auto step_next = [&]() {
    if (++nx_stage == nstage) { nx_stage = 0; ++nx_it; }
  };
  issue(nx_it, nx_stage, 0);
  step_next();
  if (NBUF > 2 && T_total > 1) { issue(nx_it, nx_stage, 1); step_next(); }
  {
    const char* w0 = wptr(it0, 0);
#pragma unroll
    for (int e = 0; e < WIN; ++e)
#pragma unroll
      for (int h = 0; h < NP; ++h)
#pragma unroll
        for (int q = 0; q < Q; ++q) wq[e][h][q] = *(const vec8*)(w0 + woff(e) + (h * Q + q) * 1024);
  }

  int cu_it = it0, cu_stage = 0;
  bool bad = false;
  unsigned pend[NT][2 * Q * NP];
  int pend_it = -1;
  unsigned padd[NT][2 * Q * NP];
  auto load_part = [&](const int it) {
    const Item I = decode(it);
    const int lx = I.bx * LXT + lix;
    const int ocs = p.ocs ? p.ocs : 32, cb2 = (I.cg * 16 * Q + g * 4 * Q) * 2;
    const long long sy = (long long)p.Cout * 2 * NP * (2 * p.LW), sz = sy * (2 * p.LH), sx = ocs == 32 ? (long long)p.Cout * 2 * NP : 32;
    const char* pb = p.part + (long long)I.n * sz * (2 * p.LD) + pz * sz + py * sy + (2 * lx + px) * sx + (long long)(cb2 >> 5) * ocs + (cb2 & 31);
#pragma unroll
    for (int i = 0; i < NT; ++i) {
      const int lz = I.bz * TZ + i / TY, ly = I.by * BY + (i % TY) * RPT + liy;
      const bool in = (lz < p.LD) & (ly < p.LH) & (lx < p.LW);
#pragma unroll
      for (int hl = 0; hl < NP; ++hl) {
        const char* src = pb + 2 * lz * sz + 2 * ly * sy + hl * p.Cout * 2;
        unsigned* dst = &padd[i][hl * 2 * Q];
        if (Q == 1) {
          const uint2 v = in ? *(const uint2*)src : make_uint2(0u, 0u);
          dst[0] = v.x; dst[1] = v.y;
        } else {
#pragma unroll
          for (int h = 0; h < Q / 2; ++h) {
            const uint4 v = in ? *(const uint4*)(src + h * 16) : make_uint4(0u, 0u, 0u, 0u);
            dst[4 * h] = v.x; dst[4 * h + 1] = v.y; dst[4 * h + 2] = v.z; dst[4 * h + 3] = v.w;
          }
        }
      }
    }
  };
  auto flush = [&]() {
    const Item I = decode(pend_it);
    pend_it = -1;
    const int lx = I.bx * LXT + lix;
    const int ocs = p.ocs ? p.ocs : 32, cb2 = (I.cg * 16 * Q + g * 4 * Q) * 2;
    const long long sy = (long long)p.Cout * 2 * NP * (2 * p.LW), sz = sy * (2 * p.LH), sx = ocs == 32 ? (long long)p.Cout * 2 * NP : 32;
    char* pb = p.out + (long long)I.n * sz * (2 * p.LD) + pz * sz + py * sy + (2 * lx + px) * sx + (long long)(cb2 >> 5) * ocs + (cb2 & 31);
#pragma unroll
    for (int i = 0; i < NT; ++i) {
      const int lz = I.bz * TZ + i / TY, ly = I.by * BY + (i % TY) * RPT + liy;
      if (lz >= p.LD || ly >= p.LH || lx >= p.LW) continue;
#pragma unroll
      for (int hl = 0; hl < NP; ++hl) {
        char* dst = pb + 2 * lz * sz + 2 * ly * sy + hl * p.Cout * 2;
        const unsigned* v = &pend[i][hl * 2 * Q];
        if (Q == 1) *(uint2*)dst = make_uint2(v[0], v[1]);
        else {
#pragma unroll
          for (int h = 0; h < Q / 2; ++h) *(uint4*)(dst + h * 16) = make_uint4(v[4 * h], v[4 * h + 1], v[4 * h + 2], v[4 * h + 3]);
        }
      }
    }
  };
  for (int t = 0; t < T_total; ++t) {
    if (t == 0) asm volatile("s_waitcnt vmcnt(0)" ::: "memory");
    else asm volatile("" ::"v"(wq[0][0][0]) : "memory");
    __syncthreads();
    if (t + NBUF - 1 < T_total && !(p.dbg & 1)) {
      issue(nx_it, nx_stage, (t + NBUF - 1) % NBUF);
      step_next();
    }
    if (pend_it >= 0 && !(p.dbg & 4)) flush();
    if (cu_stage == nstage - 1 && !(p.dbg & 16)) load_part(cu_it);
    const char* buf = smem + (t % NBUF) * C::BUF + lbase;
    if (cu_stage == 0) {
#pragma unroll
      for (int i = 0; i < NT; ++i)
#pragma unroll
        for (int q = 0; q < Q; ++q) acc[i][q] = f32x4{0.f, 0.f, 0.f, 0.f};
    }
    const bool more = t + 1 < T_total;
    const int w_it = cu_stage + 1 < nstage ? cu_it : cu_it + 1, w_stage = cu_stage + 1 < nstage ? cu_stage + 1 : 0;
    const char* wn = more ? wptr(w_it, w_stage) : p.wpk;
    const char* wc = wptr(cu_it, cu_stage);
    if (!(p.dbg & 2)) {
      constexpr int GT = SPLIT ? 2 : (NT < 4 ? NT : 4), NGT = NT / GT, NG = NTAP * NGT;
      vec8 fb[2][GT][NP];
      auto load_group = [&](const int gi, const int set) {
        const int e2 = gi / NGT, i0 = (gi % NGT) * GT;
        const int ks = e2 >> 3, ez = (e2 >> 2) & 1, ey = (e2 >> 1) & 1, ex = e2 & 1;
#pragma unroll
        for (int k = 0; k < GT; ++k) {
          const int lz = (i0 + k) / TY, ly = (i0 + k) % TY;
#pragma unroll
          for (int h = 0; h < NP; ++h)
            fb[set][k][h] = *(const vec8*)(buf + (ks + h) * 4 * PL + (((lz + ez) * HY + ly * RPT + ey) * HX + ex) * 16);
        }
      };
      load_group(0, 0);
#pragma unroll
      for (int gi = 0; gi < NG; ++gi) {
        const int e = gi / NGT, i0 = (gi % NGT) * GT;
        if (gi + 1 < NG) load_group(gi + 1, (gi + 1) & 1);
        __builtin_amdgcn_sched_barrier(0);
#pragma unroll
        for (int k = 0; k < GT; ++k)
#pragma unroll
          for (int q = 0; q < Q; ++q) {
            acc[i0 + k][q] = Ops<T_>::mfma(wq[e % WIN][0][q], fb[gi & 1][k][0], acc[i0 + k][q]);
            if (SPLIT) {
              acc[i0 + k][q] = Ops<T_>::mfma(wq[e % WIN][0][q], fb[gi & 1][k][NP - 1], acc[i0 + k][q]);
              acc[i0 + k][q] = Ops<T_>::mfma(wq[e % WIN][NP - 1][q], fb[gi & 1][k][0], acc[i0 + k][q]);
            }
          }
        __builtin_amdgcn_sched_barrier(0);
        if ((gi % NGT) == NGT - 1 && (e + WIN < NTAP || more)) {
          const char* src = e + WIN < NTAP ? wc + woff(e + WIN) : wn + woff(e + WIN - NTAP);
#pragma unroll
          for (int h = 0; h < NP; ++h)
#pragma unroll
            for (int q = 0; q < Q; ++q) wq[e % WIN][h][q] = *(const vec8*)(src + (h * Q + q) * 1024);
        }
      }
    }
    if (++cu_stage < nstage) continue;
    cu_stage = 0;

    {
      const int cgb = (cu_it / nbricks) * 16 * Q + g * 4 * Q;
      auto cvt = [](const unsigned w, const int half) { return (float)__builtin_bit_cast(T_, (unsigned short)(half ? w >> 16 : w & 0xffffu)); };
#pragma unroll
      for (int q = 0; q < Q; ++q) {
        const f32x4 bv = p.bias ? *(const f32x4*)(p.bias + cgb + q * 4) : f32x4{0.f, 0.f, 0.f, 0.f};
#pragma unroll
        for (int i = 0; i < NT; ++i)
#pragma unroll
          for (int j = 0; j < 4; ++j) {
            float a = cvt(padd[i][2 * q + (j >> 1)], j & 1);
            if (SPLIT) a += cvt(padd[i][2 * Q + 2 * q + (j >> 1)], j & 1);
            acc[i][q][j] += bv[j] + a;
          }
      }
      act_inplace<NT * Q>(&acc[0][0], p.act, p.slope);
    }
#pragma unroll
    for (int i = 0; i < NT; ++i)
#pragma unroll
      for (int q = 0; q < Q; ++q) {
#pragma unroll
        for (int j = 0; j < 4; ++j)
          if (RangeCheck<T_>::on) bad |= RangeCheck<T_>::bad(acc[i][q][j]);
        pend[i][2 * q] = (unsigned)to_bits<T_>(acc[i][q][0]) | ((unsigned)to_bits<T_>(acc[i][q][1]) << 16);
        pend[i][2 * q + 1] = (unsigned)to_bits<T_>(acc[i][q][2]) | ((unsigned)to_bits<T_>(acc[i][q][3]) << 16);
        if (SPLIT) {
          float r[4];
#pragma unroll
          for (int j = 0; j < 4; ++j) r[j] = acc[i][q][j] - (float)(T_)acc[i][q][j];
          pend[i][2 * Q + 2 * q] = (unsigned)to_bits<T_>(r[0]) | ((unsigned)to_bits<T_>(r[1]) << 16);
          pend[i][2 * Q + 2 * q + 1] = (unsigned)to_bits<T_>(r[2]) | ((unsigned)to_bits<T_>(r[3]) << 16);
        }
      }
    pend_it = cu_it;
    ++cu_it;
  }
  if (pend_it >= 0 && !(p.dbg & 4)) flush();
  if (RangeCheck<T_>::on) raise_flag(p.oflow, bad);
}

template <typename T>
__global__ void pack_upmerge_kernel(const float* __restrict__ w, const float* __restrict__ scale, T* __restrict__ wpk, int c_off,
                                    int CinTotal, int C1, int Cout, int Q, int split) {
  const int nstage = C1 / 32, NP = split ? 2 : 1;
  const long long total = (long long)(Cout / (16 * Q)) * nstage * 64 * NP * Q * 512;
  for (long long idx = blockIdx.x * (long long)blockDim.x + threadIdx.x; idx < total; idx += (long long)gridDim.x * blockDim.x) {
    const int j = idx & 7, lane = (idx >> 3) & 63;
    long long r = idx >> 9;
    const int q = r % Q; r /= Q;
    const int part = r % NP; r /= NP;
    const int e = r % 8; r /= 8;
    const int cls = r % 8; r /= 8;
    const int stage = r % nstage;
    const int cg = (int)(r / nstage);
    const int m = lane & 15, g = lane >> 4;
    const int cout = cg * 16 * Q + (m >> 2) * 4 * Q + q * 4 + (m & 3);
    const int cin = c_off + stage * 32 + g * 8 + j;
    const int par[3] = {cls >> 2, (cls >> 1) & 1, cls & 1};
    const int ee[3] = {e >> 2, (e >> 1) & 1, e & 1};
    int lo[3], hi[3];
    for (int a = 0; a < 3; ++a) {
      if (par[a] == 0) { lo[a] = ee[a] ? 1 : 0; hi[a] = ee[a] ? 2 : 0; }
      else { lo[a] = ee[a] ? 2 : 0; hi[a] = ee[a] ? 2 : 1; }
    }
    float sum = 0.f;
    for (int kz = lo[0]; kz <= hi[0]; ++kz)
      for (int ky = lo[1]; ky <= hi[1]; ++ky)
        for (int kx = lo[2]; kx <= hi[2]; ++kx) sum += w[((long long)cout * CinTotal + cin) * 27 + (kz * 3 + ky) * 3 + kx];
    const float v = sum * (scale ? scale[cout] : 1.f);
    const T vh = (T)v;
    wpk[idx] = part ? (T)(v - (float)vh) : vh;
  }
}

size_t conv_upmerge_packed_bytes(int C1, int Cout, int split) { return (size_t)Cout * C1 * 64 * 2 * (split ? 2 : 1); }
size_t conv_upmerge_partial_bytes(int N, int D, int H, int W, int Cout) { return (size_t)N * D * H * W * Cout * 2; }
int conv_upmerge_q(int Cout, int split) { return (!split && Cout % 32 == 0) ? 2 : 1; }

bool conv_upmerge_eligible(int C0, int C1, int Cout, int D, int H, int W, int up_shift, int split) {
  return up_shift == 1 && C0 >= 16 && C1 >= 32 && C1 % 32 == 0 && Cout >= (split ? 16 : 32) && Cout % 16 == 0 && W >= 16 && !(D & 1) && !(H & 1) &&
         !(W & 1) && D >= 4 && H >= 4;
}

template <typename T, int Q, int TZ, int TY, int NBUF, int KS, bool SPLIT = false, int LXT = 16>
static hipError_t launch_upm(UpmergeParams p, hipStream_t st, ConvLaunchInfo* info) {
  typedef UpmCfg<Q, TZ, TY, NBUF, KS, SPLIT, LXT> C;
  if (info)
    info->report(0, "conv3d_upmerge<%s,q%d,%dx%dx%d,b%d,k%d>", __is_same(T, f16) ? (SPLIT ? "f16x2" : "f16") : (SPLIT ? "bf16x2" : "bf16"), Q,
                 TZ, C::BY, LXT, NBUF, 32 * KS);
  auto kern = conv3d_upmerge_kernel<T, Q, TZ, TY, NBUF, KS, SPLIT, LXT>;
  static amx::DeviceOnce attr_once;
  if (!attr_once.done()) {
    hipError_t e = hipFuncSetAttribute((const void*)kern, hipFuncAttributeMaxDynamicSharedMemorySize, C::LDS_BYTES);
    if (e != hipSuccess) return e;
    attr_once.set();
  }
  const int cus = device_cus(attr_once.dev);
  if (cus == 0) return hipErrorUnknown;
  p.nbz = (p.LD + TZ - 1) / TZ;
  p.nby = (p.LH + C::BY - 1) / C::BY;
  p.nbx = (p.LW + LXT - 1) / LXT;
  const long long items = (long long)p.nbz * p.nby * p.nbx * p.N * (p.Cout / (16 * Q));
  const long long grid = items < cus ? items : cus;
  hipLaunchKernelGGL(kern, dim3((unsigned)grid), dim3(512), C::LDS_BYTES, st, p);
  return hipGetLastError();
}

template <typename T>
static hipError_t launch_upm_split(const UpmergeParams& p, hipStream_t st, ConvLaunchInfo* info) {
  if (p.LW < 16) return launch_upm<T, 1, 2, 2, 3, 1, true, 8>(p, st, info);
  const long long cells = (long long)p.N * p.LD * p.LH * ((p.LW + 15) / 16);
  if (cells / 8 * (p.Cout / 16) >= 256) return launch_upm<T, 1, 2, 4, 2, 1, true>(p, st, info);
  return launch_upm<T, 1, 2, 2, 3, 1, true>(p, st, info);
}

template <typename T>
static hipError_t launch_upm_t(const UpmergeParams& p, hipStream_t st, ConvLaunchInfo* info) {
  const int Q = conv_upmerge_q(p.Cout, 0);
  if (p.LW < 16) {
    if (Q == 2) return p.C1 % 64 == 0 ? launch_upm<T, 2, 2, 2, 2, 2, false, 8>(p, st, info) : launch_upm<T, 2, 2, 2, 3, 1, false, 8>(p, st, info);
    return launch_upm<T, 1, 2, 2, 3, 1, false, 8>(p, st, info);
  }
  const long long cells = (long long)p.N * p.LD * p.LH * ((p.LW + 15) / 16);
  const long long groups = p.Cout / (16 * Q);
  const bool k64 = p.C1 % 64 == 0;
  if (Q == 2) {
    if (cells / 8 * groups >= 256) return launch_upm<T, 2, 2, 4, 3, 1>(p, st, info);
    return k64 ? launch_upm<T, 2, 2, 2, 2, 2>(p, st, info) : launch_upm<T, 2, 2, 2, 3, 1>(p, st, info);
  }
  if (cells / 16 * groups >= 256) return launch_upm<T, 1, 2, 8, 3, 1>(p, st, info);
  return k64 ? launch_upm<T, 1, 2, 4, 2, 2>(p, st, info) : launch_upm<T, 1, 2, 4, 3, 1>(p, st, info);
}

hipError_t launch_conv_upmerge(const UpmergeParams& p, int precision, hipStream_t st, ConvLaunchInfo* info) {
  if (precision == 0) return launch_upm_t<f16>(p, st, info);
  if (precision == 1) return launch_upm_t<bf16>(p, st, info);
  if (precision == 2) return launch_upm_split<f16>(p, st, info);
  if (precision == 3) return launch_upm_split<bf16>(p, st, info);
  return hipErrorInvalidValue;
}

hipError_t launch_pack_upmerge(const float* w, const float* scale, void* wpk, int c_off, int CinTotal, int C1, int Cout, int precision,
                               hipStream_t st) {
  const int split = precision >= 2;
  const int Q = conv_upmerge_q(Cout, split);
  const long long total = (long long)Cout * C1 * 64 * (split ? 2 : 1);
  const int blocks = (int)((total + 255) / 256 > 4096 ? 4096 : (total + 255) / 256);
  if ((precision & 1) == 0)
    hipLaunchKernelGGL(pack_upmerge_kernel<f16>, dim3(blocks), dim3(256), 0, st, w, scale, (f16*)wpk, c_off, CinTotal, C1, Cout, Q, split);
  else
    hipLaunchKernelGGL(pack_upmerge_kernel<bf16>, dim3(blocks), dim3(256), 0, st, w, scale, (bf16*)wpk, c_off, CinTotal, C1, Cout, Q, split);
  return hipGetLastError();
}

}
```

anatomix_amd/csrc/amx_conv3d_v2.hip:

```cpp
#include <stdlib.h>

#include "amx_device.h"
#include "amx_launch.h"

namespace amx {

typedef __attribute__((address_space(1))) const void* gptr_t;
typedef __attribute__((address_space(3))) void* lptr_t;

template <typename T, int WZ, int WY, int WX, int NWZ, int NWY, int Q, int NCH, int OUTMODE, int NLW = 0, int NBUF = 2>
struct Conv2Cfg {
  static constexpr int NW = NWZ * NWY;
  static constexpr int TZ = WZ * NWZ, TY = WY * NWY, TX = WX;
  static constexpr int HZ = TZ + 2, HY = TY + 2, HX = TX + 2, HV = HZ * HY * HX;
  static constexpr int PLANE = ((HV * 16 + 255) / 256) * 256;
  static constexpr int HALO = 2 * PLANE;
  static constexpr int WSUB = kSteps * Q * 1024;
  static constexpr int WOFF = NCH * HALO;
  static constexpr int BIASOFF = WOFF + NCH * WSUB;
  static constexpr int BUF = BIASOFF + 256;
  static constexpr int FLAGOFF = NBUF * BUF;
  static constexpr int LDS_BYTES = NBUF * BUF + (NLW ? 64 : 0);
  static constexpr int LX = WX >= 16 ? 16 : 8;
  static constexpr int LY = 16 / LX;
  static constexpr int XT = WX / LX;
  static constexpr int YT = WY / LY;
  static constexpr int CTW = WZ * YT * XT;
  static constexpr bool LOWUP = WX >= 16 && NCH == 1 && WZ == 1 && (WY % 2) == 0;
  static constexpr int LZH = TZ / 2 + 2, LYH = TY / 2 + 2, LXH = TX / 2 + 2;
  static constexpr int RRL = 64 / LXH;
  static constexpr int NROWL = LZH * LYH;
  static constexpr int NINSTL = (NROWL + RRL - 1) / RRL;
  static constexpr int RR = 64 / HX;
  static constexpr int NROW = HZ * HY;
  static constexpr int NINST = (NROW + RR - 1) / RR;
  static_assert(HX <= 64, "halo row must fit one wave");
  static_assert(WY % LY == 0 && WX % LX == 0, "wave sub-brick must tile into 16-voxel columns");
  static_assert(LDS_BYTES <= 160 * 1024, "the pipeline buffers must fit the 160 KiB LDS");
  static_assert(NLW == 0 ? NBUF == 2 : (NBUF >= 2 && NLW <= 4 && NWZ * NWY <= 8), "pipeline shape");
};

struct ItemCoord {
  int bx, by, bz, n, cg;
};

__device__ __forceinline__ void advance_item(ItemCoord& c, const ConvParams& p) {
  if (++c.bx < p.nbx) return;
  c.bx = 0;
  if (++c.by < p.nby) return;
  c.by = 0;
  if (++c.bz < p.nbz) return;
  c.bz = 0;
  if (++c.n < p.N) return;
  c.n = 0;
  ++c.cg;
}

template <typename T, int WZ, int WY, int WX, int NWZ, int NWY, int Q, int NCH, int OUTMODE, int NLW, int NBUF, bool SPLIT, bool MX = false>
__global__ __launch_bounds__((NWZ * NWY + NLW) * 64) void conv3d_k3_v2_kernel(const ConvParams p) {
  static_assert(!MX || (SPLIT && __is_same(T, f16)), "the fp8 correction stages extend the f16 hi / lo storage");
  constexpr bool LOWUP = Conv2Cfg<T, WZ, WY, WX, NWZ, NWY, Q, NCH, OUTMODE, NLW, NBUF>::LOWUP && !MX;
  typedef Conv2Cfg<T, WZ, WY, WX, NWZ, NWY, Q, NCH, OUTMODE, NLW, NBUF> C;
  typedef typename Ops<T>::vec8 vec8;
  constexpr int HY = C::HY, HX = C::HX, PLANE = C::PLANE, HALO = C::HALO, NW = C::NW;
  constexpr int WOFF = C::WOFF, CTW = C::CTW, LX = C::LX, LY = C::LY, XT = C::XT, YT = C::YT;
  constexpr int NPEND = OUTMODE == 0 ? (SPLIT ? 4 * Q : 2 * Q) : 4 * Q;

  extern __shared__ __attribute__((aligned(16))) char smem[];

  const int tid = threadIdx.x, lane = tid & 63;
  const int wave = __builtin_amdgcn_readfirstlane(tid >> 6);
  const int li = lane & 15, g = lane >> 4;

  const int nbricks = p.nbz * p.nby * p.nbx * p.N;
  const int ncg = p.Cout / (16 * Q);
  const long long items = (long long)nbricks * ncg;
  const int G = gridDim.x;
  int jw = blockIdx.x;
  if ((G & 7) == 0) jw = (jw & 7) * (G >> 3) + (jw >> 3);
  const int it0 = (int)(items * jw / G), it1 = (int)(items * (jw + 1) / G);
  const int nchunk = (p.C0 + p.C1) >> 4;
  const int nstage = (MX ? 2 : (SPLIT ? 3 : 1)) * nchunk / NCH;
  const int mx_sa = MX ? __builtin_amdgcn_readfirstlane(*p.mxs) : 0;
  const int T_total = (it1 - it0) * nstage;
  if (T_total <= 0) return;
  const bool resident = NLW == 0 && nstage == 1 && ncg == 1;
  const int iw = NLW ? wave - NW : wave;
  constexpr int INW = NLW ? NLW : NW;
  int dma_count = 0;

  const int wz = wave / NWY, wy = wave % NWY;
  const int dy = (LX == 16) ? 0 : (li >> 3);
  const int dx = (LX == 16) ? li : (li & 7);
  const int lanehv = ((wz * WZ) * HY + wy * WY + dy) * HX + dx;
  const int lanebase = (g & 1) * PLANE + lanehv * 16;
  const int hi = g >> 1;
  const int base_d1 = lanebase + hi * 16;
  const int base_dx = lanebase + hi * 16 * HX;
  const int base_dz = lanebase + hi * 16 * HX * HY;
  const int base_d0 = lanebase;

  int U1[3], U2e[3], U2o[3], Uz = 0;
  if (LOWUP) {
    constexpr int LXH = C::LXH, LYH = C::LYH;
    const int Lx0 = ((li - 1) >> 1) + 1, Lx1 = (li >> 1) + 1, Lx2 = ((li + 1) >> 1) + 1;
    const int ub = (g & 1) * PLANE + ((wy * WY / 2) * LXH) * 16;
    int zrow[3];
#pragma unroll
    for (int kz = 0; kz < 3; ++kz) zrow[kz] = ((((wz * WZ + kz - 1) >> 1) + 1) * LYH * LXH) * 16;
#pragma unroll
    for (int kz = 0; kz < 3; ++kz) {
      U1[kz] = ub + zrow[kz] + (hi ? Lx1 : Lx0) * 16;
      U2o[kz] = ub + zrow[kz] + Lx2 * 16;
      U2e[kz] = U2o[kz] + hi * LXH * 16;
    }
    Uz = ub + (hi ? zrow[1] : zrow[0]) + Lx2 * 16;
  }

  const int dl = lane / HX, hxl = lane - dl * HX;
  const bool dma_lane = dl < C::RR;
  constexpr int NPK = (C::HV + 63) / 64, PKS = C::RR == 1 ? (NPK + INW - 1) / INW : 1;
  int pk_pos[PKS], pk_off0[PKS], pk_off1[PKS];
  const bool pk_ok = C::RR == 1 && !(p.dbg & 256) && (long long)p.D * (p.s0z > p.s1z ? p.s0z : p.s1z) < (1ll << 31);
#pragma unroll
  for (int m = 0; m < PKS; ++m) {
    const int hv = (iw + m * INW) * 64 + lane;
    const int hz = hv / (HY * HX), rem = hv - hz * (HY * HX), hy = rem / HX;
    pk_pos[m] = hv < C::HV ? (hz | (hy << 8) | ((rem - hy * HX) << 16)) : -1;
    pk_off0[m] = pk_off1[m] = 0;
  }

  ItemCoord nx;
  {
    nx.cg = it0 / nbricks;
    int b = it0 - nx.cg * nbricks;
    nx.bx = b % p.nbx;
    b /= p.nbx;
    nx.by = b % p.nby;
    b /= p.nby;
    nx.bz = b % p.nbz;
    nx.n = b / p.nbz;
  }
  ItemCoord cu = nx;
  int nx_stage = 0, cu_stage = 0;

#define AMX_DMA16(src, dst) dma16_asm((const void*)(src), (unsigned)__builtin_amdgcn_readfirstlane((int)lds_addr(dst)))
  auto issue = [&](const ItemCoord& it, int stage, int bsel01, bool with_weights) {
    char* buf = smem + bsel01 * C::BUF;
    const int z0 = it.bz * C::TZ, y0 = it.by * C::TY, x0 = it.bx * C::TX;
    const int gx = reflect_clamp(x0 + hxl - 1, p.W);
    if (C::RR == 1 && pk_ok && stage == 0) {
#pragma unroll
      for (int m = 0; m < PKS; ++m) {
        const int pos = pk_pos[m];
        const int gz = reflect_clamp(z0 + (pos & 255) - 1, p.D), gy = reflect_clamp(y0 + ((pos >> 8) & 255) - 1, p.H);
        const int gxx = reflect_clamp(x0 + ((pos >> 16) & 255) - 1, p.W);
        pk_off0[m] = gz * (int)p.s0z + gy * (int)p.s0y + gxx * (int)p.s0x;
        pk_off1[m] = gz * (int)p.s1z + gy * (int)p.s1y + gxx * (int)p.s1x;
      }
    }
#pragma unroll
    for (int k = 0; k < NCH; ++k) {
      const int vch = stage * NCH + k;
      const int part = SPLIT ? vch / nchunk : 0;
      const int ch = (vch - part * nchunk) << 4;
      const bool second = ch >= p.C0;
      const int sh = second ? p.up_shift : 0;
      const int cseg = second ? p.C1 : p.C0, chs = second ? ch - p.C0 : ch;
      const int sec = part == 1 ? (MX ? 2 : 1) : 0;
      const int cs = second ? (p.cs1 ? p.cs1 : 32) : (p.cs0 ? p.cs0 : 32);
      const long long coff = (long long)(sec * (cseg >> 4) + (chs >> 4)) * cs;
      const char* base = (second ? p.src1 + (long long)it.n * p.s1n : p.src0 + (long long)it.n * p.s0n) + coff;
      const long long sz = second ? p.s1z : p.s0z, sy = second ? p.s1y : p.s0y;
      const int xoff = (gx >> sh) * (int)(second ? p.s1x : p.s0x);
      if (LOWUP && second && p.up_shift) {
        const int LD = p.D >> 1, LH = p.H >> 1, LW = p.W >> 1;
        const int dl2 = lane / C::LXH, hx2 = lane - dl2 * C::LXH;
        int gx2 = (x0 >> 1) - 1 + hx2;
        gx2 = gx2 < 0 ? 0 : (gx2 >= LW ? LW - 1 : gx2);
        for (int j = iw; j < C::NINSTL; j += INW) {
          const int r = j * C::RRL + dl2;
          const int lz = r / C::LYH, ly = r - lz * C::LYH;
          int gz = (z0 >> 1) - 1 + lz, gy = (y0 >> 1) - 1 + ly;
          gz = gz < 0 ? 0 : (gz >= LD ? LD - 1 : gz);
          gy = gy < 0 ? 0 : (gy >= LH ? LH - 1 : gy);
          const char* src = base + gz * sz + gy * sy + gx2 * (int)p.s1x;
          char* dst = buf + k * HALO + j * (C::RRL * C::LXH * 16);
          dma_count += 2;
          if (dl2 < C::RRL && r < C::NROWL) {
            AMX_DMA16(src, dst);
            AMX_DMA16(src + 16, dst + PLANE);
          }
        }
      } else if (C::RR == 1 && sh == 0 && pk_ok) {
        const int* offs = second ? pk_off1 : pk_off0;
#pragma unroll
        for (int m = 0; m < PKS; ++m) {
          const int j = iw + m * INW;
          if (j >= NPK) break;
          const char* src = base + offs[m];
          char* dst = buf + k * HALO + j * 1024;
          dma_count += 2;
          if (pk_pos[m] >= 0) {
            AMX_DMA16(src, dst);
            AMX_DMA16(src + 16, dst + PLANE);
          }
        }
      } else if (C::RR == 1) {
        for (int j = iw; j < C::NROW; j += INW) {
          const int hz = j / HY, hy = j - hz * HY;
          const int gz = reflect_clamp(z0 + hz - 1, p.D) >> sh;
          const int gy = reflect_clamp(y0 + hy - 1, p.H) >> sh;
          const char* row = base + gz * sz + gy * sy;
          char* dst = buf + k * HALO + j * (HX * 16);
          dma_count += 2;
          if (dma_lane) {
            AMX_DMA16(row + xoff, dst);
            AMX_DMA16(row + xoff + 16, dst + PLANE);
          }
        }
      } else {
        for (int j = iw; j < C::NINST; j += INW) {
          const int r = j * C::RR + dl;
          const int hz = r / HY, hy = r - hz * HY;
          const int gz = reflect_clamp(z0 + hz - 1, p.D) >> sh;
          const int gy = reflect_clamp(y0 + hy - 1, p.H) >> sh;
          const char* src = base + gz * sz + gy * sy + xoff;
          char* dst = buf + k * HALO + j * (C::RR * HX * 16);
          dma_count += 2;
          if (dma_lane && r < C::NROW) {
            AMX_DMA16(src, dst);
            AMX_DMA16(src + 16, dst + PLANE);
          }
        }
      }
    }
    if (with_weights) {
      const int vch0 = stage * NCH, part0 = SPLIT ? vch0 / nchunk : 0;
      const long long wchunk = SPLIT ? (long long)it.cg * 2 * nchunk + (vch0 - part0 * nchunk) + (part0 == (MX ? 1 : 2) ? nchunk : 0)
                                     : (long long)it.cg * nchunk + vch0;
      const char* ws = p.wpk + wchunk * C::WSUB;
      constexpr int NWI = NCH * C::WSUB / 1024;
      for (int j = iw; j < NWI; j += INW) {
        ++dma_count;
        AMX_DMA16(ws + j * 1024 + lane * 16, buf + WOFF + j * 1024);
      }
      if (iw == INW - 1 && stage == 0 && p.bias) {
        ++dma_count;
        if (lane < 4 * Q)
          AMX_DMA16((const char*)p.bias + (it.cg * 16 * Q) * 4 + lane * 16, buf + C::BIASOFF);
      }
    }
  };
  auto step_next = [&]() {
    if (++nx_stage == nstage) {
      nx_stage = 0;
      advance_item(nx, p);
    }
  };

  int* ready = (int*)(smem + C::FLAGOFF);
  int* done = (int*)(smem + C::FLAGOFF + 32);
  if (NLW) {
    if (tid < 16) ((int*)(smem + C::FLAGOFF))[tid] = (tid >= 8 + NW) ? 0x7fffffff : 0;
    __syncthreads();
    if (wave >= NW) {
      const unsigned a_ready = lds_addr(ready + iw), a_done = lds_addr(done);
      for (int t = 0; t < T_total; ++t) {
        if (t >= NBUF)
          while (__builtin_amdgcn_readfirstlane(flag_min8_asm(a_done)) < t - NBUF + 1) __builtin_amdgcn_s_sleep(1);
        dma_count = 0;
        issue(nx, nx_stage, t % NBUF, true);
        step_next();
        if (t > 0) {
          wait_vmcnt_dyn(__builtin_amdgcn_readfirstlane(dma_count));
          flag_store_asm(a_ready, t);
        }
      }
      asm volatile("s_waitcnt vmcnt(0)" ::: "memory");
      flag_store_asm(a_ready, T_total);
      return;
    }
  }

  unsigned pend[CTW][NPEND];
  ItemCoord pd = cu;
  bool pending = false;
  auto flush = [&]() {
    const int z0 = pd.bz * C::TZ, y0 = pd.by * C::TY, x0 = pd.bx * C::TX;
    const int cb = pd.cg * 16 * Q + g * 4 * Q;
    const bool full = (z0 + C::TZ <= p.D) & (y0 + C::TY <= p.H) & (x0 + C::TX <= p.W);
    const int zl = z0 + wz * WZ, yl = y0 + wy * WY + dy, xl = x0 + dx;
    if (OUTMODE == 0) {
      const int ocs = p.ocs ? p.ocs : 32;
      char* lbase = p.out + (long long)pd.n * p.on + (long long)zl * p.oz + (long long)yl * p.oy +
                    (long long)xl * p.ox + (long long)(cb >> 4) * ocs + (cb & 15) * 2;
#pragma unroll
      for (int c = 0; c < CTW; ++c) {
        const int cx = c % XT, cy = (c / XT) % YT, cz = c / (XT * YT);
        if (!full && !((zl + cz < p.D) & (yl + cy * LY < p.H) & (xl + cx * LX < p.W))) continue;
        char* dst = lbase + cz * p.oz + (cy * LY) * p.oy + (cx * LX) * p.ox;
#pragma unroll
        for (int half = 0; half < (SPLIT ? 2 : 1); ++half) {
          char* d = dst + (long long)half * (p.Cout >> 4) * ocs;
          const int o = half * 2 * Q;
          if (Q == 1) {
            *(uint2*)d = make_uint2(pend[c][o], pend[c][o + 1]);
          } else {
#pragma unroll
            for (int j = 0; j < Q / 2; ++j)
              *(uint4*)(d + j * 16) = make_uint4(pend[c][o + 4 * j], pend[c][o + 4 * j + 1], pend[c][o + 4 * j + 2], pend[c][o + 4 * j + 3]);
          }
        }
      }
    } else {
      float* lbase = p.out32 + (long long)pd.n * p.pn + (long long)cb * p.pc + (long long)zl * p.pz +
                     (long long)yl * p.py + xl;
#pragma unroll
      for (int c = 0; c < CTW; ++c) {
        const int cx = c % XT, cy = (c / XT) % YT, cz = c / (XT * YT);
        if (!full && !((zl + cz < p.D) & (yl + cy * LY < p.H) & (xl + cx * LX < p.W))) continue;
        float* dst = lbase + cz * p.pz + (cy * LY) * p.py + cx * LX;
        if (p.wmap) {
          const float wgt = p.wmap[((long long)(zl + cz) * p.H + (yl + cy * LY)) * p.W + xl + cx * LX];
#pragma unroll
          for (int j = 0; j < 4 * Q; ++j) dst[(long long)j * p.pc] += wgt * __builtin_bit_cast(float, pend[c][j]);
        } else {
#pragma unroll
          for (int j = 0; j < 4 * Q; ++j) dst[(long long)j * p.pc] = __builtin_bit_cast(float, pend[c][j]);
        }
      }
    }
  };

  f32x4 acc[CTW][Q];
  f32x4 kshift[Q];
  int kshift_cg = -1;

  unsigned long long* trace = (p.dbg & 8) ? (unsigned long long*)p.stats + (long long)blockIdx.x * 128 : nullptr;
  int tcount = 0;
#define AMX_STAMP()                                                               \
  do {                                                                            \
    if (trace && wave == 0 && lane == 0 && tcount < 128) trace[tcount] = __builtin_readcyclecounter(); \
    ++tcount;                                                                     \
  } while (0)

  AMX_STAMP();
  if (!NLW) {
    issue(nx, nx_stage, 0, true);
    step_next();
  }
  const bool late_issuer = !NLW && NW == 8 && wave >= 4 && !(p.dbg & 16);
  bool issue_due = false;
  constexpr int kLateStep = 3;
  auto late_issue = [&](int t) {
    issue(nx, nx_stage, (t + 1) & 1, !resident);
    step_next();
    issue_due = false;
  };
  AMX_STAMP();
  for (int t = 0; t < T_total; ++t) {
    if (NLW) {
      static_assert(NLW <= 4 && C::FLAGOFF % 16 == 0, "the ready flags are polled with one 16-byte read");
      while (flag_min4<(NLW ? NLW : 1)>(ready) < t + 1) __builtin_amdgcn_s_sleep(1);
      asm volatile("" ::: "memory");
    } else {
      asm volatile("s_waitcnt vmcnt(0)" ::: "memory");
      AMX_STAMP();
      __syncthreads();
      AMX_STAMP();
      if (t + 1 < T_total && !(p.dbg & 1)) {
        if (late_issuer) issue_due = true;
        else {
          issue(nx, nx_stage, (t + 1) & 1, !resident);
          step_next();
        }
      }
    }
    AMX_STAMP();
    if (pending) {
      if (!(p.dbg & 4)) flush();
      pending = false;
    }
    AMX_STAMP();
    const char* buf = smem + (t % NBUF) * C::BUF;
    const char* wbuf = resident ? smem : buf;
    if (cu_stage == 0) {
#pragma unroll
      for (int q = 0; q < Q; ++q) {
        const f32x4 bv = p.bias ? *(const f32x4*)(wbuf + C::BIASOFF + (g * Q + q) * 16) : f32x4{0.f, 0.f, 0.f, 0.f};
#pragma unroll
        for (int c = 0; c < CTW; ++c) acc[c][q] = bv;
      }
    }

    const bool up_stage = LOWUP && p.up_shift && (((cu_stage * NCH) % nchunk) << 4) >= p.C0;
    const bool mx_stage = MX && cu_stage * NCH >= nchunk;
    if (MX && mx_stage) {
      if (!(p.dbg & 2)) {
        constexpr int TSX = NCH * 7;
        typedef __attribute__((ext_vector_type(4))) int i32x4;
        constexpr int NA = CTW == 1 ? 3 : 2;
        i32x4 fa[NA][Q][2], fb[3][2];
        auto tapoff = [&](const int tp) {
          const int t = tp > 26 ? 26 : tp;
          return (((t / 9) * HY + (t / 3) % 3) * HX + t % 3) * 16;
        };
        auto load_a = [&](const int i, const int set) {
          const int k = i / 7, j = i - k * 7;
#pragma unroll
          for (int q = 0; q < Q; ++q)
#pragma unroll
            for (int r = 0; r < 2; ++r)
              fa[set][q][r] = *(const i32x4*)(wbuf + WOFF + (((k * 7 + j) * Q + q) * 2 + r) * 1024 + lane * 16);
        };
        auto load_b = [&](const int i, const int c, const int set) {
          const int k = i / 7, j = i - k * 7;
          const int cx = c % XT, cy = (c / XT) % YT, cz = c / (XT * YT);
          const int coff = ((cz * HY + cy * LY) * HX + cx * LX) * 16;
#pragma unroll
          for (int r = 0; r < 2; ++r) {
            const int lo = tapoff(4 * j + r), up = tapoff(4 * j + 2 + r);
            fb[set][r] = *(const i32x4*)(buf + base_d0 + hi * (up - lo) + (lo + k * HALO + coff));
          }
        };
        auto request = [&](const int u2) {
          if (u2 < TSX * CTW) {
            const int i2 = u2 / CTW, c2 = u2 - i2 * CTW;
            load_b(i2, c2, u2 % 3);
            if (c2 == 0) load_a(i2, i2 % NA);
          }
        };
        const int sb = 0x7f7f7f7f;
        request(0);
        request(1);
#pragma unroll
        for (int i = 0; i < TSX; ++i) {
#pragma unroll
          for (int c = 0; c < CTW; ++c) {
            const int u = i * CTW + c;
            request(u + 2);
            __builtin_amdgcn_sched_barrier(0);
            const i32x8 b8 = __builtin_shufflevector(fb[u % 3][0], fb[u % 3][1], 0, 1, 2, 3, 4, 5, 6, 7);
#pragma unroll
            for (int q = 0; q < Q; ++q) {
              const i32x8 a8 = __builtin_shufflevector(fa[i % NA][q][0], fa[i % NA][q][1], 0, 1, 2, 3, 4, 5, 6, 7);
              acc[c][q] = __builtin_amdgcn_mfma_scale_f32_16x16x128_f8f6f4(a8, b8, acc[c][q], 0, 0, 0, mx_sa, 0, sb);
            }
            __builtin_amdgcn_sched_barrier(0);
            if (!NLW && u == kLateStep && issue_due) late_issue(t);
          }
        }
      }
    } else if (!(p.dbg & 2) && up_stage) {
      constexpr int LXH = C::LXH;
      vec8 fa[2][Q], fb[2][CTW];
      auto load_step = [&](const int s, const int set) {
        const int kz = s < 9 ? s / 3 : (s < 12 ? s - 9 : (s == 12 ? 0 : 2));
        const int ky = s < 9 ? s % 3 : (s < 12 ? 0 : 2);
#pragma unroll
        for (int q = 0; q < Q; ++q) fa[set][q] = *(const vec8*)(wbuf + WOFF + (s * Q + q) * 1024 + lane * 16);
#pragma unroll
        for (int c = 0; c < CTW; ++c) {
          const int cx = c % XT, cy = (c / XT) % YT;
          const int rowc = ((cy + ky - 1) >> 1) + 1;
          const int ubase = s < 9 ? U1[kz] : (s < 12 ? ((cy & 1) ? U2o[kz] : U2e[kz]) : (s == 12 ? Uz : U2o[2]));
          fb[set][c] = *(const vec8*)(buf + ubase + (rowc * LXH + cx * 8) * 16);
        }
      };
      load_step(0, 0);
#pragma unroll
      for (int s = 0; s < kSteps; ++s) {
        if (s + 1 < kSteps) load_step(s + 1, (s + 1) & 1);
        __builtin_amdgcn_sched_barrier(0);
#pragma unroll
        for (int c = 0; c < CTW; ++c)
#pragma unroll
          for (int q = 0; q < Q; ++q) acc[c][q] = Ops<T>::mfma(fa[s & 1][q], fb[s & 1][c], acc[c][q]);
        __builtin_amdgcn_sched_barrier(0);
        if (!NLW && s == kLateStep && issue_due) late_issue(t);
      }
    } else if (!(p.dbg & 2)) {
      constexpr int TS = NCH * kSteps;
      vec8 fa[2][Q], fb[2][CTW];
      auto load_step = [&](const int i, const int set) {
        const int k = i / kSteps, s = i - k * kSteps;
        const int kz = s < 9 ? s / 3 : (s < 12 ? s - 9 : (s == 12 ? 0 : 2));
        const int ky = s < 9 ? s % 3 : (s < 12 ? 0 : 2);
        const int kx = s < 9 ? 0 : 2;
        const int tapoff = ((kz * HY + ky) * HX + kx) * 16;
        const int bsel = s < 9 ? base_d1 : (s < 12 ? base_dx : (s == 12 ? base_dz : base_d0));
#pragma unroll
        for (int q = 0; q < Q; ++q)
          fa[set][q] = *(const vec8*)(wbuf + WOFF + ((k * kSteps + s) * Q + q) * 1024 + lane * 16);
#pragma unroll
        for (int c = 0; c < CTW; ++c) {
          const int cx = c % XT, cy = (c / XT) % YT, cz = c / (XT * YT);
          const int coff = ((cz * HY + cy * LY) * HX + cx * LX) * 16;
          fb[set][c] = *(const vec8*)(buf + bsel + k * HALO + tapoff + coff);
        }
      };
      load_step(0, 0);
#pragma unroll
      for (int i = 0; i < TS; ++i) {
        if (i + 1 < TS) load_step(i + 1, (i + 1) & 1);
        __builtin_amdgcn_sched_barrier(0);
#pragma unroll
        for (int c = 0; c < CTW; ++c)
#pragma unroll
          for (int q = 0; q < Q; ++q) acc[c][q] = Ops<T>::mfma(fa[i & 1][q], fb[i & 1][c], acc[c][q]);
        __builtin_amdgcn_sched_barrier(0);
        if (!NLW && i == kLateStep && issue_due) late_issue(t);
      }
    }
    if (!NLW && issue_due) late_issue(t);
    AMX_STAMP();
    if (NLW) {
      asm volatile("s_waitcnt lgkmcnt(0)" ::: "memory");
      flag_store(done + wave, t + 1);
    }
    if (++cu_stage < nstage) continue;
    cu_stage = 0;

    if (OUTMODE == 0 && p.stats && !(p.dbg & 8)) {
      const int z0s = cu.bz * C::TZ, y0s = cu.by * C::TY, x0s = cu.bx * C::TX;
      const int zls = z0s + wz * WZ, yls = y0s + wy * WY + dy, xls = x0s + dx;
      const int cbs = cu.cg * 16 * Q + g * 4 * Q;
      if (cu.cg != kshift_cg) {
        kshift_cg = cu.cg;
#pragma unroll
        for (int q = 0; q < Q; ++q) kshift[q] = p.bias ? *(const f32x4*)(p.bias + cbs + q * 4) : f32x4{0.f, 0.f, 0.f, 0.f};
      }
      float s1[4 * Q], s2[4 * Q];
#pragma unroll
      for (int k = 0; k < 4 * Q; ++k) s1[k] = s2[k] = 0.f;
#pragma unroll
      for (int c = 0; c < CTW; ++c) {
        const int cx = c % XT, cy = (c / XT) % YT, cz = c / (XT * YT);
        const bool in = (zls + cz < p.D) & (yls + cy * LY < p.H) & (xls + cx * LX < p.W);
        if (in) {
#pragma unroll
          for (int q = 0; q < Q; ++q) {
#pragma unroll
            for (int j = 0; j < 4; ++j) {
              const float v = SPLIT ? acc[c][q][j] : (float)(T)acc[c][q][j];
              const float d = v - kshift[q][j];
              s1[q * 4 + j] += d;
              s2[q * 4 + j] += d * d;
            }
          }
        }
      }
#pragma unroll
      for (int k = 0; k < 4 * Q; ++k) {
        s1[k] += __builtin_bit_cast(float, __builtin_amdgcn_update_dpp(0, __builtin_bit_cast(int, s1[k]), 0x111, 0xF, 0xF, true));
        s2[k] += __builtin_bit_cast(float, __builtin_amdgcn_update_dpp(0, __builtin_bit_cast(int, s2[k]), 0x111, 0xF, 0xF, true));
        s1[k] += __builtin_bit_cast(float, __builtin_amdgcn_update_dpp(0, __builtin_bit_cast(int, s1[k]), 0x112, 0xF, 0xF, true));
        s2[k] += __builtin_bit_cast(float, __builtin_amdgcn_update_dpp(0, __builtin_bit_cast(int, s2[k]), 0x112, 0xF, 0xF, true));
        s1[k] += __builtin_bit_cast(float, __builtin_amdgcn_update_dpp(0, __builtin_bit_cast(int, s1[k]), 0x114, 0xF, 0xF, true));
        s2[k] += __builtin_bit_cast(float, __builtin_amdgcn_update_dpp(0, __builtin_bit_cast(int, s2[k]), 0x114, 0xF, 0xF, true));
        s1[k] += __builtin_bit_cast(float, __builtin_amdgcn_update_dpp(0, __builtin_bit_cast(int, s1[k]), 0x118, 0xF, 0xF, true));
        s2[k] += __builtin_bit_cast(float, __builtin_amdgcn_update_dpp(0, __builtin_bit_cast(int, s2[k]), 0x118, 0xF, 0xF, true));
      }
      if (li == 15) {
        const long long brick = ((long long)cu.bz * p.nby + cu.by) * p.nbx + cu.bx;
        const long long nslots = (long long)p.nbz * p.nby * p.nbx * NW;
        float* o = p.stats + (((long long)cu.n * nslots + brick * NW + wave) * p.Cout + cbs) * 2;
#pragma unroll
        for (int k = 0; k < 4 * Q; k += 2)
          *(float4*)(o + 2 * k) = make_float4(s1[k], s2[k], s1[k + 1], s2[k + 1]);
      }
    }

    act_inplace<CTW * Q>(&acc[0][0], p.act, p.slope);
    bool bad = false;
#pragma unroll
    for (int c = 0; c < CTW; ++c) {
      float v[4 * Q];
#pragma unroll
      for (int q = 0; q < Q; ++q)
#pragma unroll
        for (int j = 0; j < 4; ++j) {
          float f = acc[c][q][j];
          if (OUTMODE == 0 && RangeCheck<T>::on) bad |= RangeCheck<T>::bad(f);
          v[q * 4 + j] = f;
        }
      if (OUTMODE == 0) {
#pragma unroll
        for (int j = 0; j < 2 * Q; ++j)
          pend[c][j] = (unsigned)to_bits<T>(v[2 * j]) | ((unsigned)to_bits<T>(v[2 * j + 1]) << 16);
        if (SPLIT) {
#pragma unroll
          for (int j = 0; j < 2 * Q; ++j) {
            const float r0 = v[2 * j] - (float)(T)v[2 * j], r1 = v[2 * j + 1] - (float)(T)v[2 * j + 1];
            pend[c][2 * Q + j] = (unsigned)to_bits<T>(r0) | ((unsigned)to_bits<T>(r1) << 16);
          }
        }
      } else {
#pragma unroll
        for (int j = 0; j < 4 * Q; ++j) pend[c][j] = __builtin_bit_cast(unsigned, v[j]);
      }
    }
    if (OUTMODE == 0 && RangeCheck<T>::on) raise_flag(p.oflow, bad);
    pd = cu;
    pending = true;
    advance_item(cu, p);
  }
  if (pending && !(p.dbg & 4)) flush();
}

template <typename T, int SPLITM, int WZ, int WY, int WX, int NWZ, int NWY, int Q, int NCH, int OUTMODE, int NLW = 0, int NBUF = 2>
static hipError_t launch_cfg2(ConvParams p, hipStream_t st, ConvLaunchInfo* info, bool query) {
  constexpr bool SPLIT = SPLITM >= 1, MX = SPLITM == 2;
  typedef Conv2Cfg<T, WZ, WY, WX, NWZ, NWY, Q, NCH, OUTMODE, NLW, NBUF> C;
  p.nbz = (p.D + C::TZ - 1) / C::TZ;
  p.nby = (p.H + C::TY - 1) / C::TY;
  p.nbx = (p.W + C::TX - 1) / C::TX;
  const int stats_slots = p.nbz * p.nby * p.nbx * C::NW;
  if (query) {
    info->stats_slots = stats_slots;
    return hipSuccess;
  }
  if (MX && !p.mxs) return hipErrorInvalidValue;
  const char* tn = __is_same(T, f16) ? (MX ? "f16x2mx" : (SPLIT ? "f16x2" : "f16")) : (SPLIT ? "bf16x2" : "bf16");
  if (info && NLW)
    info->report(p.stats ? stats_slots : 0, "conv3d_k3_v2<%s,%dx%dx%d,w%d+l%d,b%d,q%d,nch%d,o%d>", tn, C::TZ, C::TY, C::TX, C::NW, NLW, NBUF,
                 Q, NCH, OUTMODE);
  else if (info)
    info->report(p.stats ? stats_slots : 0, "conv3d_k3_v2<%s,%dx%dx%d,w%d,q%d,nch%d,o%d>", tn, C::TZ, C::TY, C::TX, C::NW, Q, NCH, OUTMODE);
  auto kern = conv3d_k3_v2_kernel<T, WZ, WY, WX, NWZ, NWY, Q, NCH, OUTMODE, NLW, NBUF, SPLIT, MX>;
  static amx::DeviceOnce attr_once;
  if (!attr_once.done()) {
    hipError_t e = hipFuncSetAttribute((const void*)kern, hipFuncAttributeMaxDynamicSharedMemorySize, C::LDS_BYTES);
    if (e != hipSuccess) return e;
    attr_once.set();
  }
  const int cus = device_cus(attr_once.dev);
  if (cus == 0) return hipErrorUnknown;
  const long long items = (long long)p.nbz * p.nby * p.nbx * p.N * (p.Cout / (16 * Q));
  const int per_cu = C::LDS_BYTES <= 80 * 1024 ? 2 : 1;
  long long grid = items < (long long)cus * per_cu ? items : (long long)cus * per_cu;
  hipLaunchKernelGGL(kern, dim3((unsigned)grid), dim3((C::NW + NLW) * 64), C::LDS_BYTES, st, p);
  return hipGetLastError();
}

template <typename T, int SPLIT, int WZ, int WY, int WX, int NWZ, int NWY, int Q, int NCH, int OUTMODE>
static hipError_t launch_pick(const ConvParams& p, hipStream_t st, ConvLaunchInfo* info, bool query) {
  typedef Conv2Cfg<T, WZ, WY, WX, NWZ, NWY, Q, NCH, OUTMODE> C0;
  constexpr bool can = 3 * C0::BUF + 64 <= 160 * 1024 && NWZ * NWY <= 8;
  if constexpr (can)
    return launch_cfg2<T, SPLIT, WZ, WY, WX, NWZ, NWY, Q, NCH, OUTMODE, 4, 3>(p, st, info, query);
  else
    return launch_cfg2<T, SPLIT, WZ, WY, WX, NWZ, NWY, Q, NCH, OUTMODE>(p, st, info, query);
}

template <typename T, int OUTMODE, int SPLIT>
static hipError_t launch_conv2_t(const ConvParams& p, int Q, hipStream_t st, ConvLaunchInfo* info, bool query = false) {
  const int nch = (p.C0 + p.C1) / 16;
  if (p.W >= 32) {
    if (Q == 1) return launch_pick<T, SPLIT, 1, 4, 32, 4, 2, 1, 1, OUTMODE>(p, st, info, query);
    if (Q == 2) {
      return launch_pick<T, SPLIT, 1, 2, 32, 4, 2, 2, 1, OUTMODE>(p, st, info, query);
    }
    if (OUTMODE == 0 && Q == 4) return launch_pick<T, SPLIT, 1, 2, 16, 4, 2, 4, 1, 0>(p, st, info, query);
    return hipErrorInvalidValue;
  }
  if (OUTMODE == 1) return hipErrorInvalidValue;
  if (p.W >= 16) {
    if (Q == 1) return launch_pick<T, SPLIT, 1, 2, 16, 4, 1, 1, 1, 0>(p, st, info, query);
    if (Q == 2) return launch_pick<T, SPLIT, 1, 2, 16, 4, 2, 2, 1, 0>(p, st, info, query);
    if (Q == 4) return launch_pick<T, SPLIT, 1, 2, 16, 4, 2, 4, 1, 0>(p, st, info, query);
  }
  if (Q == 1) {
    if (nch % 2 == 0) return launch_pick<T, SPLIT, 1, 2, 8, 4, 1, 1, 2, 0>(p, st, info, query);
    return launch_pick<T, SPLIT, 1, 2, 8, 4, 1, 1, 1, 0>(p, st, info, query);
  }
  if (Q == 2 && p.W <= 4) return launch_pick<T, SPLIT, 1, 2, 8, 4, 1, 2, 1, 0>(p, st, info, query);
  if (Q == 2) return launch_pick<T, SPLIT, 1, 2, 8, 4, 2, 2, 1, 0>(p, st, info, query);
  if (Q == 4) return launch_pick<T, SPLIT, 1, 2, 8, 4, 1, 4, 1, 0>(p, st, info, query);
  return hipErrorInvalidValue;
}

int conv_v2_stats_slots(int D, int H, int W, int Q) {
  ConvParams p{};
  p.D = D; p.H = H; p.W = W; p.C0 = 16;
  ConvLaunchInfo info{};
  return launch_conv2_t<f16, 0, false>(p, Q, nullptr, &info, true) == hipSuccess ? info.stats_slots : 0;
}

hipError_t launch_conv_v2(const ConvParams& p, int precision, int Q, hipStream_t st, ConvLaunchInfo* info) {
  const bool planar = p.out32 != nullptr;
  switch (precision) {
    case 0: return planar ? launch_conv2_t<f16, 1, false>(p, Q, st, info) : launch_conv2_t<f16, 0, false>(p, Q, st, info);
    case 1: return planar ? launch_conv2_t<bf16, 1, false>(p, Q, st, info) : launch_conv2_t<bf16, 0, false>(p, Q, st, info);
    case 2: return planar ? launch_conv2_t<f16, 1, true>(p, Q, st, info) : launch_conv2_t<f16, 0, true>(p, Q, st, info);
    case 3: return planar ? launch_conv2_t<bf16, 1, true>(p, Q, st, info) : launch_conv2_t<bf16, 0, true>(p, Q, st, info);
    case 4: return planar ? launch_conv2_t<f16, 1, 2>(p, Q, st, info) : launch_conv2_t<f16, 0, 2>(p, Q, st, info);
  }
  return hipErrorInvalidValue;
}

}
```

include/anatomix_amd.h:

```cpp
#ifndef ANATOMIX_AMD_H
#define ANATOMIX_AMD_H

#include <stddef.h>
#include <stdint.h>

#ifdef __cplusplus
extern "C" {
#endif

#define AMX_VERSION 100

typedef enum amx_status {
  AMX_OK = 0,
  AMX_ERR_INVALID = -1,
  AMX_ERR_SHAPE = -2,
  AMX_ERR_NOT_LOADED = -3,
  AMX_ERR_WORKSPACE = -4,
  AMX_ERR_HIP = -5,
  AMX_ERR_OVERFLOW = -6
} amx_status;

enum { AMX_NORM_NONE = 0, AMX_NORM_BATCH_EVAL = 1, AMX_NORM_INSTANCE = 2, AMX_NORM_INSTANCE_AFFINE = 3 };
enum { AMX_ACT_NONE = 0, AMX_ACT_RELU = 1, AMX_ACT_LRELU = 2 };
enum { AMX_POOL_MAX = 0, AMX_POOL_AVG = 1 };
enum { AMX_INTERP_NEAREST = 0, AMX_INTERP_TRILINEAR = 1 };
enum { AMX_PREC_F16 = 0, AMX_PREC_BF16 = 1, AMX_PREC_F16X2 = 2, AMX_PREC_BF16X2 = 3, AMX_PREC_F16X2_MX = 4 };

typedef struct amx_unet_cfg {
  int32_t input_nc;
  int32_t output_nc;
  int32_t num_downs;
  int32_t ngf;
  int32_t norm;
  float norm_eps;
  int32_t activation;
  float act_slope;
  int32_t final_act;
  int32_t pooling;
  int32_t interp;
  int32_t doubleconv;
  int32_t use_skip;
  int32_t precision;
} amx_unet_cfg;

typedef struct amx_unet amx_unet_t;

int amx_version(void);

int amx_debug_fill_lds(unsigned pattern, void* stream);
const char* amx_last_error(void);

int amx_unet_create(amx_unet_t** out, const amx_unet_cfg* cfg);
void amx_unet_destroy(amx_unet_t* h);

int amx_unet_num_modules(const amx_unet_t* h);
int amx_unet_num_convs(const amx_unet_t* h);
int amx_unet_conv_info(const amx_unet_t* h, int conv, int* module_idx, int* cin, int* cout, int* norm_module_idx);

int amx_unet_load_conv(amx_unet_t* h, int module_idx, const float* d_weight, const float* d_bias,
                       const float* d_gamma, const float* d_beta, const float* d_mean,
                       const float* d_var, void* stream);

typedef struct amx_launch_record {
  char kernel[64];
  int32_t module_idx;
  int32_t cin, cout;
  int32_t n, d, h, w;
  float ms;
  double flops;
  double bytes;
} amx_launch_record;

size_t amx_unet_workspace_bytes(const amx_unet_t* h, int n, int d, int w_h, int w_w);

int amx_unet_forward(amx_unet_t* h, const float* d_x, float* d_y, int n, int d, int hh, int w,
                     void* d_workspace, size_t workspace_bytes, void* stream);

int amx_unet_numerics_status(amx_unet_t* h, int synchronize, void* stream);

int amx_unet_module_info(const amx_unet_t* h, int module_idx, int* channels, int* level);

int amx_unet_forward_taps(amx_unet_t* h, const float* d_x, float* d_y, int n, int d, int hh, int w,
                          void* d_workspace, size_t workspace_bytes, const int* tap_modules, int n_taps,
                          float* const* d_tap_out, int stop_module, void* stream);

int amx_unet_forward_profiled(amx_unet_t* h, const float* d_x, float* d_y, int n, int d, int hh, int w,
                              void* d_workspace, size_t workspace_bytes, void* stream,
                              amx_launch_record* records, int max_records, int* n_records);

int amx_unet_forward_window(amx_unet_t* h, const float* d_vol, int vd, int vh, int vw, int oz, int oy,
                            int ox, int rd, int rh, int rw, const float* d_wmap, float* d_acc,
                            void* d_workspace, size_t workspace_bytes, void* stream);

int amx_unet_forward_windows(amx_unet_t* h, const float* d_vol, int vd, int vh, int vw, int n_windows,
                             const int* offsets_zyx, int rd, int rh, int rw, const float* d_wmap, float* d_acc,
                             void* d_workspace, size_t workspace_bytes, void* stream);

int amx_unet_forward_windows_pipelined(amx_unet_t* h, const float* d_vol, int vd, int vh, int vw, int n_windows,
                                       const int* offsets_zyx, int rd, int rh, int rw, const float* d_wmap, float* d_acc,
                                       void* d_workspace, size_t workspace_bytes, int slot, void* stream);

int amx_sw_normalize(float* d_acc, const float* d_cnt, int channels, long long voxels, void* stream);

int amx_sw_count(float* d_cnt, int vd, int vh, int vw, int oz, int oy, int ox, int rd, int rh, int rw,
                 const float* d_wmap, void* stream);

typedef enum amx_sw_map { AMX_SW_MAP_CONSTANT = 0, AMX_SW_MAP_GAUSSIAN = 1 } amx_sw_map;
typedef enum amx_sw_out {
  AMX_SW_FEATURES = 0,
  AMX_SW_LOGITS = 1,
  AMX_SW_LABELS = 2
} amx_sw_out;

int amx_sw_plan(int vd, int vh, int vw, int rd, int rh, int rw, double overlap, int* offsets_zyx, int capacity);

int amx_sw_importance_map(float* d_wmap, int rd, int rh, int rw, int mode, double sigma_scale, void* stream);

int amx_sw_count_all(float* d_cnt, int vd, int vh, int vw, int rd, int rh, int rw, double overlap, const float* d_wmap,
                     void* stream);

int amx_sw_finish(int kind, float* d_acc, const float* d_cnt, int feat, long long voxels, const float* d_w, const float* d_b,
                  int classes, void* d_out, void* stream);

size_t amx_sliding_window_workspace_bytes(const amx_unet_t* h, int n_batch, int rd, int rh, int rw);

int amx_sliding_window(amx_unet_t* h, const float* d_vol, int vd, int vh, int vw, int rd, int rh, int rw, double overlap,
                       int mode, double sigma_scale, int n_batch, int out_kind, const float* d_w, const float* d_b,
                       int classes, float* d_acc, float* d_cnt, void* d_out, void* d_workspace, size_t workspace_bytes,
                       void* stream);

size_t amx_conv3d_packed_bytes(int cin, int cout);
int amx_conv3d_k3_reflect(const void* d_x0, int c0, const void* d_x1, int c1, const float* d_weight,
                          const float* d_scale, const float* d_shift, int cout, int n, int d, int hh,
                          int w, int act, float slope, int precision, void* d_wpk, void* d_out16,
                          float* d_out32, void* stream);

int amx_conv3d_k3_reflect_probe(const void* d_x0, int c0, const void* d_x1, int c1, const float* d_weight, const float* d_scale,
                                const float* d_shift, int cout, int n, int d, int hh, int w, int act, float slope, int precision,
                                void* d_wpk, void* d_out16, float* d_out32, void* d_pool16, const float* d_wmap, int* d_oflow,
                                char* kernel_name, void* stream);

size_t amx_conv3d_scratch_bytes(int c0, int c1, int cout, int n, int d, int hh, int w, int precision);
int amx_conv3d_k3_reflect_ws(const void* d_x0, int c0, const void* d_x1, int c1, const float* d_weight,
                             const float* d_scale, const float* d_shift, int cout, int n, int d, int hh,
                             int w, int act, float slope, int precision, void* d_wpk, void* d_out16,
                             float* d_out32, void* d_scratch, size_t scratch_bytes, void* stream);

int amx_conv3d_k3_reflect_ex(const void* d_x0, int c0, const void* d_x1, int c1, const float* d_weight, int weight_mode,
                             int cin_real, int cout_real, const float* d_scale, const float* d_shift, int cout, int n,
                             int d, int hh, int w, int act, float slope, int precision, void* d_wpk, void* d_out16,
                             float* d_out32, void* stream);

#define AMX_WEIGHTS_PREPACKED 16
typedef struct amx_pack_req {
  const float* d_weight;
  void* d_wpk;
  int weight_mode, cin_real, cin_pad, cout_real, cout, w;
} amx_pack_req;
int amx_conv3d_pack_batch(const amx_pack_req* reqs, int count, int precision, void* stream);

int amx_conv3d_dgrad_interior_supported(int c_dy, int cout, int d, int hh, int w, int precision);
int amx_conv3d_dgrad_interior(const void* d_dy_framed, int c_dy, const float* d_weight, int weight_flags, int cin_real, int cout_real, int cout,
                              int n, int d, int hh, int w, int precision, void* d_wpk, void* d_out16, void* stream);
size_t amx_conv3d_dgrad_shell_scratch_bytes(void);
int amx_conv3d_dgrad_fold_shell(const void* d_dy_framed, int c_dy, const float* d_weight, int co_real, int ci_real, void* d_dx, int c_dx, int n,
                                int d, int hh, int w, int precision, void* d_scratch, void* stream);

int amx_pool2(const void* d_in, void* d_out, int n, int d_out_, int h_out, int w_out, int c, int avg,
              int precision, void* stream);

size_t amx_instance_norm_scratch_bytes(int n, int c);
int amx_instance_norm(void* d_x, const float* d_gamma, const float* d_beta, float eps, int n, long long voxels,
                      int c, int act, float slope, void* d_scratch, int precision, void* stream);

int amx_upsample2_trilinear(const void* d_in, void* d_out, int n, int din, int hin, int win, int c,
                            int precision, void* stream);

int amx_upcat_split_backward(const void* d_dcat, void* d_dskip, void* d_dlow, int n, int dlow, int hlow, int wlow, int c0, int c1,
                             int accumulate_skip, int precision, void* stream);
int amx_upcat_split_backward_framed(const void* d_g_framed, void* d_dskip, void* d_dlow, int n, int dlow, int hlow, int wlow, int c0,
                                    int c1, int accumulate_skip, int precision, void* stream);

int amx_import_input(const float* d_src, void* d_dst, int n, int cin, int d, int hh, int w, int precision, void* stream);
int amx_export_ncdhw(const void* d_src, int c, int n, int d, int hh, int w, float* d_out, int precision, void* stream);
int amx_import_ncdhw(const float* d_src, void* d_dst, int n, int c, int d, int hh, int w, long long dst_sn, long long dst_sz,
                     long long dst_sy, long long dst_sx, int accumulate, int precision, void* stream);

int amx_upsample2_trilinear_backward(const void* d_gout, void* d_gin, int n, int din, int hin, int win, int c, int precision,
                                     void* stream);

size_t amx_conv3d_upcat_merged_packed_bytes(int c0, int c1, int cout);
int amx_conv3d_upcat_merged(const void* d_x0, int c0, const void* d_x1, int c1, const float* d_weight, const float* d_scale,
                            const float* d_shift, int cout, int n, int d, int hh, int w, int act, float slope, int precision,
                            void* d_wpk, void* d_partial, void* d_out16, void* stream);

size_t amx_train_scratch_bytes(int c);

int amx_bn_train_forward(const void* d_x, void* d_y, const float* d_gamma, const float* d_beta, float eps, int n,
                         long long voxels, int c, int act, float slope, void* d_scratch, float* d_save_mean,
                         float* d_save_rstd, float* d_running_mean, float* d_running_var, float momentum, int precision,
                         void* stream);

int amx_bn_act_backward(const void* d_dy, const void* d_y, const void* d_x, const float* d_mean, const float* d_rstd,
                        const float* d_gamma, float* d_dgamma, float* d_dbeta, void* d_dx_framed, int n, int d, int hh, int w,
                        int c, int act, float slope, void* d_scratch, int precision, void* stream);
int amx_bn_act_backward_recompute(const void* d_dy, const void* d_x, const float* d_mean, const float* d_rstd, const float* d_gamma,
                                  const float* d_beta, float* d_dgamma, float* d_dbeta, void* d_dx_framed, int n, int d, int hh, int w,
                                  int c, int act, float slope, void* d_scratch, int precision, void* stream);

int amx_pad_fold(const void* d_g_framed, void* d_din, int n, int d, int hh, int w, int c, int accumulate, int precision,
                 void* stream);

int amx_pool2_max_backward(const void* d_dp, const void* d_in, void* d_din, int n, int dout, int hout, int wout, int c,
                           int accumulate, int precision, void* stream);

size_t amx_conv3d_wgrad_scratch_bytes(int n, int d, int hh, int w, int cout, int cin_pad);
int amx_conv3d_wgrad(const void* d_dy, long long dy_sn, long long dy_sz, long long dy_sy, long long dy_sx, const void* d_x0,
                     int c0, const void* d_x1, int c1, int cin_real, int cout, int n, int d, int hh, int w, float* d_dw,
                     int accumulate, void* d_scratch, size_t scratch_bytes, int precision, void* stream);

size_t amx_attention_scratch_bytes(int b, int heads, int n, int head_dim);
int amx_attention_qknorm_rope(const float* d_q, const float* d_k, const float* d_v, const float* d_qn_w, const float* d_qn_b,
                              const float* d_kn_w, const float* d_kn_b, float norm_eps, const float* d_rope, int n_prefix, int b,
                              int n, int heads, int head_dim, float* d_out, void* d_scratch, size_t scratch_bytes, void* stream);

int amx_attention_prepared(const void* d_scratch, size_t scratch_bytes, int b, int n, int heads, int head_dim, float* d_out, void* stream);

size_t amx_attention_train_scratch_bytes(int b, int heads, int n, int head_dim);
int amx_attention_qknorm_rope_train(const float* d_q, const float* d_k, const float* d_v, const float* d_qn_w, const float* d_qn_b,
                                    const float* d_kn_w, const float* d_kn_b, float norm_eps, const float* d_rope, int n_prefix, int b,
                                    int n, int heads, int head_dim, float* d_out, float* d_lse, void* d_scratch, size_t scratch_bytes,
                                    void* stream);
int amx_attention_backward(const float* d_q, const float* d_k, const float* d_v, const float* d_qn_w, const float* d_qn_b,
                           const float* d_kn_w, const float* d_kn_b, float norm_eps, const float* d_rope, int n_prefix, int b, int n,
                           int heads, int head_dim, const float* d_out, const float* d_lse, const float* d_dout, float* d_dq, float* d_dk,
                           float* d_dv, float* d_dqn_w, float* d_dqn_b, float* d_dkn_w, float* d_dkn_b, void* d_scratch,
                           size_t scratch_bytes, void* stream);

typedef struct amx_vit_cfg {
  int32_t input_channels;
  int32_t num_classes;
  int32_t embed_dim;
  int32_t depth;
  int32_t heads;
  int32_t num_register_tokens;
  int32_t grid_d, grid_h, grid_w;
  int32_t hidden;
  int32_t dec1, dec2;
  int32_t qk_norm;
  int32_t scale_attn_inner;
  int32_t layer_scale;
  float in_eps;
  int32_t out_norm;
  int32_t decoder_split;
  int32_t stem_split;
} amx_vit_cfg;
typedef struct amx_vit amx_vit_t;

int amx_vit_create(amx_vit_t** out, const amx_vit_cfg* cfg);
void amx_vit_destroy(amx_vit_t* h);
int amx_vit_num_params(const amx_vit_t* h);
const char* amx_vit_param_name(const amx_vit_t* h, int idx);
int amx_vit_load(amx_vit_t* h, const float* const* d_params, int count, const float* d_rope, void* stream);
size_t amx_vit_workspace_bytes(const amx_vit_t* h, int n);
int amx_vit_forward(amx_vit_t* h, const float* d_x, float* d_y, int n, void* d_ws, size_t ws_bytes, int n_blocks, void* stream);
int amx_vit_debug_read(amx_vit_t* h, const char* name, void* d_dst, size_t max_bytes, size_t* bytes, void* stream);

typedef struct amx_vit_tap {
  const char* name;
  void* d_dst;
  size_t bytes;
  char route[160];
} amx_vit_tap;
size_t amx_vit_tap_bytes(const amx_vit_t* h, int n, const char* name);
int amx_vit_forward_taps(amx_vit_t* h, const float* d_x, float* d_y, int n, void* d_ws, size_t ws_bytes, int n_blocks, amx_vit_tap* taps,
                         int n_taps, void* stream);


size_t amx_vit_windows_workspace_bytes(const amx_vit_t* h, int n_windows);

int amx_vit_forward_windows(amx_vit_t* h, const float* d_vol, int vd, int vh, int vw, int n_windows, const int* offsets_zyx,
                            const float* d_wmap, float* d_acc, void* d_ws, size_t ws_bytes, void* stream);

size_t amx_vit_sliding_window_workspace_bytes(const amx_vit_t* h, int n_batch);

int amx_vit_sliding_window(amx_vit_t* h, const float* d_vol, int vd, int vh, int vw, double overlap, int mode, double sigma_scale,
                           int n_batch, int out_kind, const float* d_w, const float* d_b, int classes, float* d_acc, float* d_cnt,
                           void* d_out, void* d_ws, size_t ws_bytes, void* stream);
int amx_linear(const float* d_x, const float* d_w, const float* d_b, int m, int k, int n, int split, float* d_y, void* stream);

size_t amx_supcon_scratch_bytes(int n, int c);
int amx_supcon_loss(const float* d_feat, const int* d_labels, int n, int c, float temperature, int weigh_rarity,
                    int balance_denominator, int sqrt_mode, float* d_loss, float* d_grad, void* d_scratch,
// ... 321 lines not shown
```

Before: 3049 volumes/s.

## Specialize conv kernels on activation and cut per-element address and range-check work

The k-split and upmerge conv kernels are now templated on the activation, so the runtime branch on activation type disappears. Halo positions are precomputed once per thread and packed into an int, and each brick is found by stepping from the previous one instead of a full divide-based decode. Output addresses are built from a per-brick base plus a fixed per-lane offset, and the per-value overflow check is replaced by a running max that raises the flag once at the end. Debug trace and dbg-flag branches are removed from the v2 kernel, and a deep_probe API plus 31-bit size guards are added, at the cost of more template instances.

New measurement: 3073 volumes/s (median of 6 runs). Within noise of the previous version (+0.8%).

```diff
diff --git a/anatomix_amd/_lib.py b/anatomix_amd/_lib.py
--- a/anatomix_amd/_lib.py
+++ b/anatomix_amd/_lib.py
@@ -91,6 +91,7 @@
     "amx_conv3d_packed_bytes": (C.c_size_t, [_I, _I]),
     "amx_conv3d_k3_reflect": (_I, [_P, _I, _P, _I, _P, _P, _P, _I, _I, _I, _I, _I, _I, C.c_float, _I, _P, _P, _P, _P]),
     "amx_conv3d_k3_reflect_probe": (_I, [_P, _I, _P, _I, _P, _P, _P, _I, _I, _I, _I, _I, _I, C.c_float, _I, _P, _P, _P, _P, _P, _P, _P, _P]),
+    "amx_conv3d_deep_probe": (_I, [_P, _I, _P, _I, _P, _P, _P, _I, _I, _I, _I, _I, _I, C.c_float, _I, _P, _P, C.c_size_t, _P, _P, _P, _P]),
     "amx_conv3d_dgrad_interior_supported": (_I, [_I, _I, _I, _I, _I, _I]),
     "amx_conv3d_dgrad_interior": (_I, [_P, _I, _P, _I, _I, _I, _I, _I, _I, _I, _I, _I, _P, _P, _P]),
     "amx_conv3d_dgrad_shell_scratch_bytes": (C.c_size_t, []),
diff --git a/anatomix_amd/csrc/amx_api.hip b/anatomix_amd/csrc/amx_api.hip
--- a/anatomix_amd/csrc/amx_api.hip
+++ b/anatomix_amd/csrc/amx_api.hip
@@ -295,9 +295,9 @@
   return 2 * (align_up((size_t)cout * c0 * 28 * 2, 256) + amx::conv_upmerge_packed_bytes(c1, cout, 0));
 }
 
-int amx_conv3d_upcat_merged(const void* d_x0, int c0, const void* d_x1, int c1, const float* d_weight, const float* d_scale,
-                            const float* d_shift, int cout, int n, int d, int hh, int w, int act, float slope, int precision,
-                            void* d_wpk, void* d_partial, void* d_out16, void* stream) {
+static int upcat_merged(const void* d_x0, int c0, const void* d_x1, int c1, const float* d_weight, const float* d_scale,
+                        const float* d_shift, int cout, int n, int d, int hh, int w, int act, float slope, int precision,
+                        void* d_wpk, void* d_partial, void* d_out16, void* stream, int* d_oflow, char* kernel_names) {
   if (!d_x0 || !d_x1 || !d_weight || !d_wpk || !d_partial || !d_out16) return fail(AMX_ERR_INVALID, "null argument");
   if (precision < AMX_PREC_F16 || precision > AMX_PREC_BF16X2) return fail(AMX_ERR_INVALID, "unsupported precision %d", precision);
   const bool split = is_split(precision);
@@ -315,15 +315,45 @@
   amx::set_src0(p, d_x0, c0, d, hh, w, precision);
   p.wpk = (const char*)d_wpk; p.act = AMX_ACT_NONE;
   amx::set_out(p, d_partial, cout, d, hh, w, precision);
-  AMX_HIP(amx::launch_conv(p, precision, q, st));
+  amx::ConvLaunchInfo info{};
+  amx::ConvLaunchInfo* const want = kernel_names ? &info : nullptr;
+  AMX_HIP(amx::launch_conv(p, precision, q, st, want));
+  if (kernel_names) memcpy(kernel_names, info.name, sizeof info.name);
   amx::UpmergeParams u;
   memset(&u, 0, sizeof u);
   amx::set_src(u, d_x1, c1, d / 2, hh / 2, w / 2, precision);
   u.N = n; u.LD = d / 2; u.LH = hh / 2; u.LW = w / 2; u.Cout = cout;
   u.wpk = wmerge; u.part = (const char*)d_partial; u.out = (char*)d_out16;
   u.bias = d_shift; u.act = act; u.slope = slope;
-  AMX_HIP(amx::launch_conv_upmerge(u, precision, st));
-  return AMX_OK;
+  u.oflow = d_oflow;
+  info = amx::ConvLaunchInfo{};
+  AMX_HIP(amx::launch_conv_upmerge(u, precision, st, want));
+  if (kernel_names) memcpy(kernel_names + sizeof info.name, info.name, sizeof info.name);
+  return AMX_OK;
+}
+
+int amx_conv3d_upcat_merged(const void* d_x0, int c0, const void* d_x1, int c1, const float* d_weight, const float* d_scale,
+                            const float* d_shift, int cout, int n, int d, int hh, int w, int act, float slope, int precision,
+                            void* d_wpk, void* d_partial, void* d_out16, void* stream) {
+  return upcat_merged(d_x0, c0, d_x1, c1, d_weight, d_scale, d_shift, cout, n, d, hh, w, act, slope, precision, d_wpk, d_partial, d_out16,
+                      stream, nullptr, nullptr);
+}
+
+int amx_conv3d_deep_probe(const void* d_x0, int c0, const void* d_x1, int c1, const float* d_weight, const float* d_scale,
+                          const float* d_shift, int cout, int n, int d, int hh, int w, int act, float slope, int precision,
+                          void* d_wpk, void* d_scratch, size_t scratch_bytes, void* d_out16, int* d_oflow, char* kernel_names,
+                          void* stream) {
+  if (!kernel_names) return fail(AMX_ERR_INVALID, "deep_probe: kernel_names is required");
+  memset(kernel_names, 0, 128);
+  if (c1) {
+    const size_t need = (size_t)n * d * hh * w * cout * 2 * (is_split(precision) ? 2 : 1);
+    if (scratch_bytes < need) return fail(AMX_ERR_WORKSPACE, "deep_probe: the skip partial sums need %zu bytes", need);
+    return upcat_merged(d_x0, c0, d_x1, c1, d_weight, d_scale, d_shift, cout, n, d, hh, w, act, slope, precision, d_wpk, d_scratch, d_out16,
+                        stream, d_oflow, kernel_names);
+  }
+  const ConvProbe probe{nullptr, nullptr, d_oflow, kernel_names};
+  return conv3d_single(d_x0, c0, nullptr, 0, d_weight, 0, c0, cout, d_scale, d_shift, cout, n, d, hh, w, act, slope, precision, d_wpk,
+                       d_out16, nullptr, stream, d_scratch, scratch_bytes, &probe);
 }
 
 int amx_pool2(const void* d_in, void* d_out, int n, int dout, int hout, int wout, int c, int avg, int precision,
diff --git a/anatomix_amd/csrc/amx_common.h b/anatomix_amd/csrc/amx_common.h
--- a/anatomix_amd/csrc/amx_common.h
+++ b/anatomix_amd/csrc/amx_common.h
@@ -102,7 +102,6 @@
   float slope;
   int nbz, nby, nbx;
   int* oflow;
-  int dbg;
   int cs, ocs;
 };
 
diff --git a/anatomix_amd/csrc/amx_conv3d_ks.hip b/anatomix_amd/csrc/amx_conv3d_ks.hip
--- a/anatomix_amd/csrc/amx_conv3d_ks.hip
+++ b/anatomix_amd/csrc/amx_conv3d_ks.hip
@@ -49,8 +49,9 @@
   int n, z0, y0, x0;
 };
 
-template <typename T, typename C, bool PART>
+template <typename T, typename C, bool PART, int ACT>
 __global__ __launch_bounds__(C::NWAVE * 64, C::NWAVE * C::WGS_PER_CU / 4) void conv3d_k3_ks_kernel(const ConvParams p) {
+  static_assert(!PART || ACT == ACT_NONE, "partial sums are not activated");
   typedef typename Ops<T>::vec8 vec8;
   constexpr int Q = C::Q, QP = C::QP, CPW = C::CPW, KW = C::KW, CW = C::CW, TEAMS = C::TEAMS, NVTG = C::NVTG, NH = C::NH;
   constexpr int HY = C::HY, HX = C::HX, PLANE = C::PLANE, CHBUF = C::CHBUF, NPK = C::NPK, NPKW = C::NPKW;
@@ -91,8 +92,15 @@
   const int base_d0 = lanebase;
 
   int pk_off[NPKW];
-#pragma unroll
-  for (int m = 0; m < NPKW; ++m) pk_off[m] = 0;
+  int pk_h[NPKW];
+#pragma unroll
+  for (int m = 0; m < NPKW; ++m) {
+    pk_off[m] = 0;
+    const int hv = (m * CW + cw) * 64 + lane;
+    const int hz = hv / (HY * HX), rem = hv - hz * (HY * HX), hy = rem / HX, hx = rem - hy * HX;
+    pk_h[m] = hv < C::HV ? (hz << 16 | hy << 8 | hx) : -1;
+  }
+  static_assert(C::HY < 256 && C::HX < 256, "the packed halo position has 8 bits per in-plane axis");
   char* const halo = smem + (team * KW + k) * (C::NBUF * CHBUF);
   char* const scratch = smem + C::HALO_BYTES + (team * CW + cw) * C::SCR_GROUP;
 
@@ -109,14 +117,33 @@
     r.x0 = bx * C::TX;
     return r;
   };
+  auto advance = [&](KsBrick& r) {
+    r.x0 += C::TX;
+    if (r.x0 >= p.W) {
+      r.x0 = 0;
+      r.y0 += C::TY;
+      if (r.y0 >= p.H) {
+        r.y0 = 0;
+        r.z0 += C::TZ;
+        if (r.z0 >= p.D) {
+          r.z0 = 0;
+          ++r.n;
+        }
+      }
+    }
+  };
+  auto reflect = [](int g, int n) {
+    const int a = g < 0 ? -g : g, b = 2 * n - 2 - a;
+    const int r = a < b ? a : b;
+    return r < 0 ? 0 : (r > n - 1 ? n - 1 : r);
+  };
   auto offsets = [&](const KsBrick& br) {
+    const int zb = br.z0 - 1, yb = br.y0 - 1, xb = br.x0 - 1;
 #pragma unroll
     for (int m = 0; m < NPKW; ++m) {
-      const int hv = (m * CW + cw) * 64 + lane;
-      const int hz = hv / (HY * HX), rem = hv - hz * (HY * HX), hy = rem / HX, hx = rem - hy * HX;
-      const int gz = reflect_clamp(br.z0 + hz - 1, p.D), gy = reflect_clamp(br.y0 + hy - 1, p.H);
-      const int gx = reflect_clamp(br.x0 + hx - 1, p.W);
-      pk_off[m] = hv < C::HV ? gz * (int)p.s0z + gy * (int)p.s0y + gx * (int)p.s0x : -1;
+      const int h = pk_h[m];
+      const int gz = reflect(zb + (h >> 16), p.D), gy = reflect(yb + ((h >> 8) & 255), p.H), gx = reflect(xb + (h & 255), p.W);
+      pk_off[m] = h >= 0 ? gz * (int)p.s0z + gy * (int)p.s0y + gx * (int)p.s0x : -1;
     }
   };
 #define AMX_DMA16(src, dst) dma16_asm((const void*)(src), (unsigned)__builtin_amdgcn_readfirstlane((int)lds_addr(dst)))
@@ -145,6 +172,13 @@
   }
 
   const int cb = pg * 16 * QP + g * 4 * QP + q0 * 4;
+  const int ocs = p.ocs ? p.ocs : 32;
+  const long long vz = (long long)p.H * p.W * p.Cout * 4, vy = (long long)p.W * p.Cout * 4, vx = (long long)p.Cout * 4;
+  const long long tz_ = PART ? vz : p.oz, ty_ = PART ? vy : p.oy, tx_ = PART ? vx : p.ox;
+  const unsigned lane_out = (unsigned)(dzl * (int)tz_ + dx * (int)tx_ + (PART ? cb * 4 : (cb >> 4) * ocs + (cb & 15) * 2));
+  char* const obase = PART ? (char*)p.part + (long long)slice * p.N * p.D * vz : p.out;
+  const long long tn_ = PART ? p.D * vz : p.on;
+  unsigned amax = 0;
 
   KsBrick cu = decode(b0 + team), nx = cu;
   bool cu_valid = b0 + team < b1;
@@ -174,8 +208,13 @@
   for (int it = 0; it < niter; ++it) {
     const int bn = b0 + (it + 1) * TEAMS + team;
     const bool nx_valid = it + 1 < niter && bn < b1;
-    if (nx_valid) nx = decode(bn);
+    if (nx_valid) {
+      nx = cu;
+#pragma unroll
+      for (int a = 0; a < TEAMS; ++a) advance(nx);
+    }
     const bool full = cu_valid && (cu.z0 + C::TZ <= p.D) & (cu.y0 + C::TY <= p.H) & (cu.x0 + C::TX <= p.W);
+    char* const obrick = obase + cu.n * tn_ + cu.z0 * tz_ + cu.y0 * ty_ + cu.x0 * tx_;
 #pragma unroll
     for (int h = 0; h < NH; ++h) {
 #pragma unroll
@@ -259,7 +298,6 @@
 #pragma unroll
         for (int o = 0; o < KW; ++o) {
           if (o == k && cu_valid) {
-            bool bad = false;
 #pragma unroll
             for (int i = 0; i < RT; ++i) {
               f32x4 v[Q];
@@ -276,27 +314,24 @@
               if (!PART) {
 #pragma unroll
                 for (int q = 0; q < Q; ++q) v[q] += bq[q];
-                act_inplace<Q>(&v[0], p.act, p.slope);
+                act_values<ACT, Q>(&v[0], p.slope);
               }
               const int c = h * NVTG + o * OWN + r * RT + i;
               const int cx = c % XT, cy = (c / XT) % YT, cz = c / (XT * YT);
-              const int zl = cu.z0 + C::tile_z(cz) + dzl, yl = cu.y0 + cy, xl = cu.x0 + cx * LX + dx;
-              if (!full && !((zl < p.D) & (yl < p.H) & (xl < p.W))) continue;
+              if (!full) {
+                const int zl = cu.z0 + C::tile_z(cz) + dzl, yl = cu.y0 + cy, xl = cu.x0 + cx * LX + dx;
+                if (!((zl < p.D) & (yl < p.H) & (xl < p.W))) continue;
+              }
+              char* d = obrick + (C::tile_z(cz) * tz_ + cy * ty_ + cx * LX * tx_) + lane_out;
               if (PART) {
-                const long long vox = (((long long)cu.n * p.D + zl) * p.H + yl) * p.W + xl;
-                float* d = p.part + ((long long)slice * p.N * p.D * p.H * p.W + vox) * p.Cout + cb;
-#pragma unroll
-                for (int q = 0; q < Q; ++q) *(f32x4*)(d + q * 4) = v[q];
+#pragma unroll
+                for (int q = 0; q < Q; ++q) *(f32x4*)(d + q * 16) = v[q];
               } else {
-                const int ocs = p.ocs ? p.ocs : 32;
-                char* d = p.out + (long long)cu.n * p.on + (long long)zl * p.oz + (long long)yl * p.oy + (long long)xl * p.ox +
-                          (long long)(cb >> 4) * ocs + (cb & 15) * 2;
                 unsigned pk[2 * Q];
 #pragma unroll
                 for (int q = 0; q < Q; ++q) {
-#pragma unroll
-                  for (int j = 0; j < 4; ++j)
-                    if (RangeCheck<T>::on) bad |= RangeCheck<T>::bad(v[q][j]);
+                  amax = RangeCheck<T>::template track<ACT == ACT_RELU>(amax, v[q][0], v[q][1]);
+                  amax = RangeCheck<T>::template track<ACT == ACT_RELU>(amax, v[q][2], v[q][3]);
                   pk[2 * q] = (unsigned)to_bits<T>(v[q][0]) | ((unsigned)to_bits<T>(v[q][1]) << 16);
                   pk[2 * q + 1] = (unsigned)to_bits<T>(v[q][2]) | ((unsigned)to_bits<T>(v[q][3]) << 16);
                 }
@@ -308,7 +343,6 @@
                 }
               }
             }
-            if (!PART && RangeCheck<T>::on) raise_flag(p.oflow, bad);
           }
         }
         __syncthreads();
@@ -318,6 +352,7 @@
     cu = nx;
     cu_valid = nx_valid;
   }
+  if (!PART && RangeCheck<T>::on) raise_flag(p.oflow, RangeCheck<T>::bad_bits(amax));
 #undef AMX_DMA16
 }
 
@@ -363,12 +398,12 @@
   if (RangeCheck<T>::on) raise_flag(oflow, bad);
 }
 
-template <typename T, typename C, bool PART>
+template <typename T, typename C, bool PART, int ACT>
 static hipError_t launch_ks_cfg(ConvParams p, hipStream_t st, ConvLaunchInfo* info) {
   if (info)
     info->report(0, "conv3d_k3_ks<%s,%dx%dx%d,q%d,k%dx%d,c%d,t%d,h%d,b%d%s>", __is_same(T, f16) ? "f16" : "bf16", C::TZ, C::TY, C::TX, C::Q,
                  C::KW, C::CPW, C::CW, C::TEAMS, C::NH, C::NBUF, PART ? ",part" : "");
-  auto kern = conv3d_k3_ks_kernel<T, C, PART>;
+  auto kern = conv3d_k3_ks_kernel<T, C, PART, ACT>;
   static amx::DeviceOnce attr_once;
   if (!attr_once.done()) {
     hipError_t e = hipFuncSetAttribute((const void*)kern, hipFuncAttributeMaxDynamicSharedMemorySize, C::LDS_BYTES);
@@ -399,6 +434,7 @@
   KsPlan r = {0, 0, 0, 0, 1, 1};
   if (precision > 1 || p.C1 != 0 || p.src0_f32c1 || p.out32 || p.out2 || p.stats || !p.out || p.W < 8 || p.H < 2 || p.D < 2) return r;
   if ((long long)p.D * p.s0z >= (1ll << 31)) return r;
+  if ((long long)p.D * p.oz >= (1ll << 31)) return r;
   const int nchunk = p.C0 >> 4;
   if (p.C0 & 15) return r;
   const int tz = p.W >= 16 ? 2 : 4, ty = 4, tx = p.W >= 16 ? 16 : 8;
@@ -413,7 +449,7 @@
   if (Q != 2) return r;
   auto cw_of = [&](int slices) { return (p.Cout % 64 == 0 && (long long)(p.Cout / 64) * slices * nbricks >= 200) ? 2 : 1; };
   if (nchunk == 4) { r = {1, 4, 1, 1, 1, cw_of(1)}; return r; }
-  if (nchunk % 8 == 0 && can_split) {
+  if (nchunk % 8 == 0 && can_split && (long long)p.D * p.H * p.W * p.Cout * 4 < (1ll << 31)) {
     const int s8 = nchunk / 8;
     if ((long long)ncg * nbricks >= 192) return r;
     if (s8 >= 2 && (long long)ncg * s8 * nbricks >= 192 && s8 <= 8) { r = {1, 4, 2, 1, s8, 1}; return r; }
@@ -445,7 +481,10 @@
 #define AMX_KS(TZ, TY, TX, QW, QP, CPW, KW, CW, TEAMS, NH, ...)                              \
   do {                                                                                       \
     typedef KsCfg<TZ, TY, TX, QW, QP, CPW, KW, CW, TEAMS, NH, ##__VA_ARGS__> CC;             \
-    e = part ? launch_ks_cfg<T, CC, true>(p, st, info) : launch_ks_cfg<T, CC, false>(p, st, info);      \
+    e = part                 ? launch_ks_cfg<T, CC, true, ACT_NONE>(p, st, info)                        \
+        : p.act == ACT_RELU  ? launch_ks_cfg<T, CC, false, ACT_RELU>(p, st, info)                       \
+        : p.act == ACT_LRELU ? launch_ks_cfg<T, CC, false, ACT_LRELU>(p, st, info)                      \
+                             : launch_ks_cfg<T, CC, false, ACT_NONE>(p, st, info);                      \
   } while (0)
   if (Q == 4 && pl.kw == 2) {
     if (wide) AMX_KS(2, 4, 16, 2, 4, 1, 2, 2, 2, 2);
diff --git a/anatomix_amd/csrc/amx_conv3d_upmerge.hip b/anatomix_amd/csrc/amx_conv3d_upmerge.hip
--- a/anatomix_amd/csrc/amx_conv3d_upmerge.hip
+++ b/anatomix_amd/csrc/amx_conv3d_upmerge.hip
@@ -24,7 +24,7 @@
   static_assert(LDS_BYTES <= 160 * 1024, "ring must fit the LDS");
 };
 
-template <typename T_, int Q, int TZ, int TY, int NBUF, int KS, bool SPLIT, int LXT>
+template <typename T_, int Q, int TZ, int TY, int NBUF, int KS, bool SPLIT, int LXT, int ACT>
 __global__ __launch_bounds__(512) void conv3d_upmerge_kernel(const UpmergeParams p) {
   typedef UpmCfg<Q, TZ, TY, NBUF, KS, SPLIT, LXT> C;
   constexpr int RPT = C::RPT, BY = C::BY;
@@ -61,24 +61,40 @@
     r.n = b / p.nbz;
     return r;
   };
-
-  int dma_item = -1;
+  auto advance = [&](Item& r) {
+    if (++r.bx < p.nbx) return;
+    r.bx = 0;
+    if (++r.by < p.nby) return;
+    r.by = 0;
+    if (++r.bz < p.nbz) return;
+    r.bz = 0;
+    if (++r.n < p.N) return;
+    r.n = 0;
+    ++r.cg;
+  };
+
   int off[C::PER_WAVE];
-  auto issue = [&](int it, int stage, int bsel) {
-    const Item I = decode(it);
-    if (it != dma_item) {
-      dma_item = it;
+  int off_h[C::PER_WAVE];
+#pragma unroll
+  for (int m = 0; m < C::PER_WAVE; ++m) {
+    const int id = wave + 8 * m;
+    const int j = id % C::NJ;
+    const int hv = j * 64 + lane;
+    const int hz = hv / (HY * HX), rem = hv - hz * (HY * HX), hy = rem / HX, hx = rem - hy * HX;
+    off_h[m] = hv < C::HV ? (hz << 16 | hy << 8 | hx) : -1;
+    off[m] = -1;
+  }
+  auto issue = [&](const Item& I, int stage, int bsel) {
+    if (stage == 0) {
+      const int zb = I.bz * TZ - 1, yb = I.by * BY - 1, xb = I.bx * LXT - 1;
 #pragma unroll
       for (int m = 0; m < C::PER_WAVE; ++m) {
-        const int id = wave + 8 * m;
-        const int j = id % C::NJ;
-        const int hv = j * 64 + lane;
-        const int hz = hv / (HY * HX), rem = hv - hz * (HY * HX), hy = rem / HX, hx = rem - hy * HX;
-        int gz = I.bz * TZ - 1 + hz, gy = I.by * BY - 1 + hy, gx = I.bx * LXT - 1 + hx;
+        const int h = off_h[m];
+        int gz = zb + (h >> 16), gy = yb + ((h >> 8) & 255), gx = xb + (h & 255);
         gz = gz < 0 ? 0 : (gz >= p.LD ? p.LD - 1 : gz);
         gy = gy < 0 ? 0 : (gy >= p.LH ? p.LH - 1 : gy);
         gx = gx < 0 ? 0 : (gx >= p.LW ? p.LW - 1 : gx);
-        off[m] = hv < C::HV ? gz * (int)p.sz + gy * (int)p.sy + gx * (int)p.sx : -1;
+        off[m] = h >= 0 ? gz * (int)p.sz + gy * (int)p.sy + gx * (int)p.sx : -1;
       }
     }
     const char* base = p.src + (long long)I.n * p.sn;
@@ -97,8 +113,7 @@
     }
   };
 
-  auto wptr = [&](int it, int stage) -> const char* {
-    const int cg = it / nbricks;
+  auto wptr = [&](int cg, int stage) -> const char* {
     return p.wpk + ((((long long)cg * nstage * KS + stage * KS) * 8 + wave) * 8 * NP * Q) * 1024 + lane * 16;
   };
   auto woff = [](const int e2) { return ((e2 >> 3) * 64 + (e2 & 7)) * NP * Q * 1024; };
@@ -108,15 +123,16 @@
   const int lbase = g * PL + ((pz * HY + py + liy) * HX + px + lix) * 16;
 
   f32x4 acc[NT][Q];
-  int nx_it = it0, nx_stage = 0;
+  Item nx = decode(it0), cu = nx, pd = nx;
+  int nx_stage = 0;
   auto step_next = [&]() {
-    if (++nx_stage == nstage) { nx_stage = 0; ++nx_it; }
-  };
-  issue(nx_it, nx_stage, 0);
+    if (++nx_stage == nstage) { nx_stage = 0; advance(nx); }
+  };
+  issue(nx, nx_stage, 0);
   step_next();
-  if (NBUF > 2 && T_total > 1) { issue(nx_it, nx_stage, 1); step_next(); }
+  if (NBUF > 2 && T_total > 1) { issue(nx, nx_stage, 1); step_next(); }
   {
-    const char* w0 = wptr(it0, 0);
+    const char* w0 = wptr(cu.cg, 0);
 #pragma unroll
     for (int e = 0; e < WIN; ++e)
 #pragma unroll
@@ -125,24 +141,31 @@
         for (int q = 0; q < Q; ++q) wq[e][h][q] = *(const vec8*)(w0 + woff(e) + (h * Q + q) * 1024);
   }
 
-  int cu_it = it0, cu_stage = 0;
-  bool bad = false;
+  int cu_stage = 0;
+  unsigned amax = 0;
+  const int ocs = p.ocs ? p.ocs : 32;
+  const long long osy = (long long)p.Cout * 2 * NP * (2 * p.LW), osz = osy * (2 * p.LH), osx = ocs == 32 ? (long long)p.Cout * 2 * NP : 32;
+  const unsigned lane_io = (unsigned)(2 * lix * (int)osx + 2 * liy * (int)osy + ((g * 8 * Q) >> 5) * ocs + ((g * 8 * Q) & 31));
+  auto item_base = [&](const Item& I) -> long long {
+    return (long long)I.n * osz * (2 * p.LD) + (2 * I.bz * TZ + pz) * osz + (2 * I.by * BY + py) * osy + (2 * I.bx * LXT + px) * osx +
+           (long long)I.cg * Q * ocs;
+  };
+  auto item_full = [&](const Item& I) { return (I.bz * TZ + TZ <= p.LD) & (I.by * BY + BY <= p.LH) & (I.bx * LXT + LXT <= p.LW); };
+  f32x4 bv[Q];
   unsigned pend[NT][2 * Q * NP];
-  int pend_it = -1;
+  bool pending = false;
   unsigned padd[NT][2 * Q * NP];
-  auto load_part = [&](const int it) {
-    const Item I = decode(it);
+  auto load_part_as = [&](const Item& I, auto fullc) {
+    constexpr bool FULL = decltype(fullc)::value;
+    const char* pb = p.part + item_base(I);
     const int lx = I.bx * LXT + lix;
-    const int ocs = p.ocs ? p.ocs : 32, cb2 = (I.cg * 16 * Q + g * 4 * Q) * 2;
-    const long long sy = (long long)p.Cout * 2 * NP * (2 * p.LW), sz = sy * (2 * p.LH), sx = ocs == 32 ? (long long)p.Cout * 2 * NP : 32;
-    const char* pb = p.part + (long long)I.n * sz * (2 * p.LD) + pz * sz + py * sy + (2 * lx + px) * sx + (long long)(cb2 >> 5) * ocs + (cb2 & 31);
 #pragma unroll
     for (int i = 0; i < NT; ++i) {
       const int lz = I.bz * TZ + i / TY, ly = I.by * BY + (i % TY) * RPT + liy;
-      const bool in = (lz < p.LD) & (ly < p.LH) & (lx < p.LW);
+      const bool in = FULL || ((lz < p.LD) & (ly < p.LH) & (lx < p.LW));
 #pragma unroll
       for (int hl = 0; hl < NP; ++hl) {
-        const char* src = pb + 2 * lz * sz + 2 * ly * sy + hl * p.Cout * 2;
+        const char* src = pb + (2 * (i / TY) * osz + 2 * ((i % TY) * RPT) * osy + hl * p.Cout * 2) + lane_io;
         unsigned* dst = &padd[i][hl * 2 * Q];
         if (Q == 1) {
           const uint2 v = in ? *(const uint2*)src : make_uint2(0u, 0u);
@@ -156,21 +179,27 @@
         }
       }
     }
-  };
-  auto flush = [&]() {
-    const Item I = decode(pend_it);
-    pend_it = -1;
+    const int cgb = I.cg * 16 * Q + g * 4 * Q;
+#pragma unroll
+    for (int q = 0; q < Q; ++q) bv[q] = p.bias ? *(const f32x4*)(p.bias + cgb + q * 4) : f32x4{0.f, 0.f, 0.f, 0.f};
+  };
+  auto load_part = [&](const Item& I) {
+    if (item_full(I)) load_part_as(I, Const<1>{});
+    else load_part_as(I, Const<0>{});
+  };
+  auto flush_as = [&](const Item& I, auto fullc) {
+    constexpr bool FULL = decltype(fullc)::value;
+    char* pb = p.out + item_base(I);
     const int lx = I.bx * LXT + lix;
-    const int ocs = p.ocs ? p.ocs : 32, cb2 = (I.cg * 16 * Q + g * 4 * Q) * 2;
-    const long long sy = (long long)p.Cout * 2 * NP * (2 * p.LW), sz = sy * (2 * p.LH), sx = ocs == 32 ? (long long)p.Cout * 2 * NP : 32;
-    char* pb = p.out + (long long)I.n * sz * (2 * p.LD) + pz * sz + py * sy + (2 * lx + px) * sx + (long long)(cb2 >> 5) * ocs + (cb2 & 31);
 #pragma unroll
     for (int i = 0; i < NT; ++i) {
-      const int lz = I.bz * TZ + i / TY, ly = I.by * BY + (i % TY) * RPT + liy;
-      if (lz >= p.LD || ly >= p.LH || lx >= p.LW) continue;
+      if (!FULL) {
+        const int lz = I.bz * TZ + i / TY, ly = I.by * BY + (i % TY) * RPT + liy;
+        if (lz >= p.LD || ly >= p.LH || lx >= p.LW) continue;
+      }
 #pragma unroll
       for (int hl = 0; hl < NP; ++hl) {
-        char* dst = pb + 2 * lz * sz + 2 * ly * sy + hl * p.Cout * 2;
+        char* dst = pb + (2 * (i / TY) * osz + 2 * ((i % TY) * RPT) * osy + hl * p.Cout * 2) + lane_io;
         const unsigned* v = &pend[i][hl * 2 * Q];
         if (Q == 1) *(uint2*)dst = make_uint2(v[0], v[1]);
         else {
@@ -179,17 +208,22 @@
         }
       }
     }
+  };
+  auto flush = [&]() {
+    pending = false;
+    if (item_full(pd)) flush_as(pd, Const<1>{});
+    else flush_as(pd, Const<0>{});
   };
   for (int t = 0; t < T_total; ++t) {
     if (t == 0) asm volatile("s_waitcnt vmcnt(0)" ::: "memory");
     else asm volatile("" ::"v"(wq[0][0][0]) : "memory");
     __syncthreads();
-    if (t + NBUF - 1 < T_total && !(p.dbg & 1)) {
-      issue(nx_it, nx_stage, (t + NBUF - 1) % NBUF);
+    if (t + NBUF - 1 < T_total) {
+      issue(nx, nx_stage, (t + NBUF - 1) % NBUF);
       step_next();
     }
-    if (pend_it >= 0 && !(p.dbg & 4)) flush();
-    if (cu_stage == nstage - 1 && !(p.dbg & 16)) load_part(cu_it);
+    if (pending) flush();
+    if (cu_stage == nstage - 1) load_part(cu);
     const char* buf = smem + (t % NBUF) * C::BUF + lbase;
     if (cu_stage == 0) {
 #pragma unroll
@@ -198,10 +232,11 @@
         for (int q = 0; q < Q; ++q) acc[i][q] = f32x4{0.f, 0.f, 0.f, 0.f};
     }
     const bool more = t + 1 < T_total;
-    const int w_it = cu_stage + 1 < nstage ? cu_it : cu_it + 1, w_stage = cu_stage + 1 < nstage ? cu_stage + 1 : 0;
-    const char* wn = more ? wptr(w_it, w_stage) : p.wpk;
-    const char* wc = wptr(cu_it, cu_stage);
-    if (!(p.dbg & 2)) {
+    const bool last_of_cg = (cu.bx + 1 == p.nbx) & (cu.by + 1 == p.nby) & (cu.bz + 1 == p.nbz) & (cu.n + 1 == p.N);
+    const int w_cg = cu_stage + 1 < nstage ? cu.cg : cu.cg + (last_of_cg ? 1 : 0), w_stage = cu_stage + 1 < nstage ? cu_stage + 1 : 0;
+    const char* wn = more ? wptr(w_cg, w_stage) : p.wpk;
+    const char* wc = wptr(cu.cg, cu_stage);
+    {
       constexpr int GT = SPLIT ? 2 : (NT < 4 ? NT : 4), NGT = NT / GT, NG = NTAP * NGT;
       vec8 fb[2][GT][NP];
       auto load_group = [&](const int gi, const int set) {
@@ -245,29 +280,26 @@
     cu_stage = 0;
 
     {
-      const int cgb = (cu_it / nbricks) * 16 * Q + g * 4 * Q;
       auto cvt = [](const unsigned w, const int half) { return (float)__builtin_bit_cast(T_, (unsigned short)(half ? w >> 16 : w & 0xffffu)); };
 #pragma unroll
       for (int q = 0; q < Q; ++q) {
-        const f32x4 bv = p.bias ? *(const f32x4*)(p.bias + cgb + q * 4) : f32x4{0.f, 0.f, 0.f, 0.f};
 #pragma unroll
         for (int i = 0; i < NT; ++i)
 #pragma unroll
           for (int j = 0; j < 4; ++j) {
             float a = cvt(padd[i][2 * q + (j >> 1)], j & 1);
             if (SPLIT) a += cvt(padd[i][2 * Q + 2 * q + (j >> 1)], j & 1);
-            acc[i][q][j] += bv[j] + a;
+            acc[i][q][j] += bv[q][j] + a;
           }
       }
-      act_inplace<NT * Q>(&acc[0][0], p.act, p.slope);
+      act_values<ACT, NT * Q>(&acc[0][0], p.slope);
     }
 #pragma unroll
     for (int i = 0; i < NT; ++i)
 #pragma unroll
       for (int q = 0; q < Q; ++q) {
-#pragma unroll
-        for (int j = 0; j < 4; ++j)
-          if (RangeCheck<T_>::on) bad |= RangeCheck<T_>::bad(acc[i][q][j]);
+        amax = RangeCheck<T_>::template track<ACT == ACT_RELU>(amax, acc[i][q][0], acc[i][q][1]);
+        amax = RangeCheck<T_>::template track<ACT == ACT_RELU>(amax, acc[i][q][2], acc[i][q][3]);
         pend[i][2 * q] = (unsigned)to_bits<T_>(acc[i][q][0]) | ((unsigned)to_bits<T_>(acc[i][q][1]) << 16);
         pend[i][2 * q + 1] = (unsigned)to_bits<T_>(acc[i][q][2]) | ((unsigned)to_bits<T_>(acc[i][q][3]) << 16);
         if (SPLIT) {
@@ -278,11 +310,12 @@
           pend[i][2 * Q + 2 * q + 1] = (unsigned)to_bits<T_>(r[2]) | ((unsigned)to_bits<T_>(r[3]) << 16);
         }
       }
-    pend_it = cu_it;
-    ++cu_it;
-  }
-  if (pend_it >= 0 && !(p.dbg & 4)) flush();
-  if (RangeCheck<T_>::on) raise_flag(p.oflow, bad);
+    pd = cu;
+    pending = true;
+    advance(cu);
+  }
+  if (pending) flush();
+  if (RangeCheck<T_>::on) raise_flag(p.oflow, RangeCheck<T_>::bad_bits(amax));
 }
 
 template <typename T>
@@ -325,16 +358,16 @@
 
 bool conv_upmerge_eligible(int C0, int C1, int Cout, int D, int H, int W, int up_shift, int split) {
   return up_shift == 1 && C0 >= 16 && C1 >= 32 && C1 % 32 == 0 && Cout >= (split ? 16 : 32) && Cout % 16 == 0 && W >= 16 && !(D & 1) && !(H & 1) &&
-         !(W & 1) && D >= 4 && H >= 4;
-}
-
-template <typename T, int Q, int TZ, int TY, int NBUF, int KS, bool SPLIT = false, int LXT = 16>
-static hipError_t launch_upm(UpmergeParams p, hipStream_t st, ConvLaunchInfo* info) {
+         !(W & 1) && D >= 4 && H >= 4 && (long long)D * H * W * Cout * 4 < (1ll << 31);
+}
+
+template <typename T, int Q, int TZ, int TY, int NBUF, int KS, bool SPLIT, int LXT, int ACT>
+static hipError_t launch_upm_act(UpmergeParams p, hipStream_t st, ConvLaunchInfo* info) {
   typedef UpmCfg<Q, TZ, TY, NBUF, KS, SPLIT, LXT> C;
   if (info)
     info->report(0, "conv3d_upmerge<%s,q%d,%dx%dx%d,b%d,k%d>", __is_same(T, f16) ? (SPLIT ? "f16x2" : "f16") : (SPLIT ? "bf16x2" : "bf16"), Q,
                  TZ, C::BY, LXT, NBUF, 32 * KS);
-  auto kern = conv3d_upmerge_kernel<T, Q, TZ, TY, NBUF, KS, SPLIT, LXT>;
+  auto kern = conv3d_upmerge_kernel<T, Q, TZ, TY, NBUF, KS, SPLIT, LXT, ACT>;
   static amx::DeviceOnce attr_once;
   if (!attr_once.done()) {
     hipError_t e = hipFuncSetAttribute((const void*)kern, hipFuncAttributeMaxDynamicSharedMemorySize, C::LDS_BYTES);
@@ -350,6 +383,13 @@
   const long long grid = items < cus ? items : cus;
   hipLaunchKernelGGL(kern, dim3((unsigned)grid), dim3(512), C::LDS_BYTES, st, p);
   return hipGetLastError();
+}
+
+template <typename T, int Q, int TZ, int TY, int NBUF, int KS, bool SPLIT = false, int LXT = 16>
+static hipError_t launch_upm(const UpmergeParams& p, hipStream_t st, ConvLaunchInfo* info) {
+  if (p.act == ACT_RELU) return launch_upm_act<T, Q, TZ, TY, NBUF, KS, SPLIT, LXT, ACT_RELU>(p, st, info);
+  if (p.act == ACT_LRELU) return launch_upm_act<T, Q, TZ, TY, NBUF, KS, SPLIT, LXT, ACT_LRELU>(p, st, info);
+  return launch_upm_act<T, Q, TZ, TY, NBUF, KS, SPLIT, LXT, ACT_NONE>(p, st, info);
 }
 
 template <typename T>
diff --git a/anatomix_amd/csrc/amx_conv3d_v2.hip b/anatomix_amd/csrc/amx_conv3d_v2.hip
--- a/anatomix_amd/csrc/amx_conv3d_v2.hip
+++ b/anatomix_amd/csrc/amx_conv3d_v2.hip
@@ -121,7 +121,7 @@
   const bool dma_lane = dl < C::RR;
   constexpr int NPK = (C::HV + 63) / 64, PKS = C::RR == 1 ? (NPK + INW - 1) / INW : 1;
   int pk_pos[PKS], pk_off0[PKS], pk_off1[PKS];
-  const bool pk_ok = C::RR == 1 && !(p.dbg & 256) && (long long)p.D * (p.s0z > p.s1z ? p.s0z : p.s1z) < (1ll << 31);
+  const bool pk_ok = C::RR == 1 && (long long)p.D * (p.s0z > p.s1z ? p.s0z : p.s1z) < (1ll << 31);
 #pragma unroll
   for (int m = 0; m < PKS; ++m) {
     const int hv = (iw + m * INW) * 64 + lane;
@@ -337,20 +337,11 @@
   f32x4 kshift[Q];
   int kshift_cg = -1;
 
-  unsigned long long* trace = (p.dbg & 8) ? (unsigned long long*)p.stats + (long long)blockIdx.x * 128 : nullptr;
-  int tcount = 0;
-#define AMX_STAMP()                                                               \
-  do {                                                                            \
-    if (trace && wave == 0 && lane == 0 && tcount < 128) trace[tcount] = __builtin_readcyclecounter(); \
-    ++tcount;                                                                     \
-  } while (0)
-
-  AMX_STAMP();
   if (!NLW) {
     issue(nx, nx_stage, 0, true);
     step_next();
   }
-  const bool late_issuer = !NLW && NW == 8 && wave >= 4 && !(p.dbg & 16);
+  const bool late_issuer = !NLW && NW == 8 && wave >= 4;
   bool issue_due = false;
   constexpr int kLateStep = 3;
   auto late_issue = [&](int t) {
@@ -358,7 +349,6 @@
     step_next();
     issue_due = false;
   };
-  AMX_STAMP();
   for (int t = 0; t < T_total; ++t) {
     if (NLW) {
       static_assert(NLW <= 4 && C::FLAGOFF % 16 == 0, "the ready flags are polled with one 16-byte read");
@@ -366,10 +356,8 @@
       asm volatile("" ::: "memory");
     } else {
       asm volatile("s_waitcnt vmcnt(0)" ::: "memory");
-      AMX_STAMP();
       __syncthreads();
-      AMX_STAMP();
-      if (t + 1 < T_total && !(p.dbg & 1)) {
+      if (t + 1 < T_total) {
         if (late_issuer) issue_due = true;
         else {
           issue(nx, nx_stage, (t + 1) & 1, !resident);
@@ -377,12 +365,10 @@
         }
       }
     }
-    AMX_STAMP();
     if (pending) {
-      if (!(p.dbg & 4)) flush();
+      flush();
       pending = false;
     }
-    AMX_STAMP();
     const char* buf = smem + (t % NBUF) * C::BUF;
     const char* wbuf = resident ? smem : buf;
     if (cu_stage == 0) {
@@ -397,7 +383,7 @@
     const bool up_stage = LOWUP && p.up_shift && (((cu_stage * NCH) % nchunk) << 4) >= p.C0;
     const bool mx_stage = MX && cu_stage * NCH >= nchunk;
     if (MX && mx_stage) {
-      if (!(p.dbg & 2)) {
+      {
         constexpr int TSX = NCH * 7;
         typedef __attribute__((ext_vector_type(4))) int i32x4;
         constexpr int NA = CTW == 1 ? 3 : 2;
@@ -452,7 +438,7 @@
           }
         }
       }
-    } else if (!(p.dbg & 2) && up_stage) {
+    } else if (up_stage) {
       constexpr int LXH = C::LXH;
       vec8 fa[2][Q], fb[2][CTW];
       auto load_step = [&](const int s, const int set) {
@@ -480,7 +466,7 @@
         __builtin_amdgcn_sched_barrier(0);
         if (!NLW && s == kLateStep && issue_due) late_issue(t);
       }
-    } else if (!(p.dbg & 2)) {
+    } else {
       constexpr int TS = NCH * kSteps;
       vec8 fa[2][Q], fb[2][CTW];
       auto load_step = [&](const int i, const int set) {
@@ -514,7 +500,6 @@
       }
     }
     if (!NLW && issue_due) late_issue(t);
-    AMX_STAMP();
     if (NLW) {
       asm volatile("s_waitcnt lgkmcnt(0)" ::: "memory");
       flag_store(done + wave, t + 1);
@@ -522,7 +507,7 @@
     if (++cu_stage < nstage) continue;
     cu_stage = 0;
 
-    if (OUTMODE == 0 && p.stats && !(p.dbg & 8)) {
+    if (OUTMODE == 0 && p.stats) {
       const int z0s = cu.bz * C::TZ, y0s = cu.by * C::TY, x0s = cu.bx * C::TX;
       const int zls = z0s + wz * WZ, yls = y0s + wy * WY + dy, xls = x0s + dx;
       const int cbs = cu.cg * 16 * Q + g * 4 * Q;
@@ -573,18 +558,19 @@
     }
 
     act_inplace<CTW * Q>(&acc[0][0], p.act, p.slope);
-    bool bad = false;
+    unsigned amax = 0;
 #pragma unroll
     for (int c = 0; c < CTW; ++c) {
       float v[4 * Q];
 #pragma unroll
-      for (int q = 0; q < Q; ++q)
-#pragma unroll
-        for (int j = 0; j < 4; ++j) {
-          float f = acc[c][q][j];
-          if (OUTMODE == 0 && RangeCheck<T>::on) bad |= RangeCheck<T>::bad(f);
-          v[q * 4 + j] = f;
-        }
+      for (int q = 0; q < Q; ++q) {
+#pragma unroll
+        for (int j = 0; j < 4; ++j) v[q * 4 + j] = acc[c][q][j];
+        if (OUTMODE == 0) {
+          amax = RangeCheck<T>::template track<false>(amax, acc[c][q][0], acc[c][q][1]);
+          amax = RangeCheck<T>::template track<false>(amax, acc[c][q][2], acc[c][q][3]);
+        }
+      }
       if (OUTMODE == 0) {
 #pragma unroll
         for (int j = 0; j < 2 * Q; ++j)
@@ -601,12 +587,12 @@
         for (int j = 0; j < 4 * Q; ++j) pend[c][j] = __builtin_bit_cast(unsigned, v[j]);
       }
     }
-    if (OUTMODE == 0 && RangeCheck<T>::on) raise_flag(p.oflow, bad);
+    if (OUTMODE == 0 && RangeCheck<T>::on) raise_flag(p.oflow, RangeCheck<T>::bad_bits(amax));
     pd = cu;
     pending = true;
     advance_item(cu, p);
   }
-  if (pending && !(p.dbg & 4)) flush();
+  if (pending) flush();
 }
 
 template <typename T, int SPLITM, int WZ, int WY, int WX, int NWZ, int NWY, int Q, int NCH, int OUTMODE, int NLW = 0, int NBUF = 2>
diff --git a/include/anatomix_amd.h b/include/anatomix_amd.h
--- a/include/anatomix_amd.h
+++ b/include/anatomix_amd.h
@@ -139,6 +139,11 @@
                                 const float* d_shift, int cout, int n, int d, int hh, int w, int act, float slope, int precision,
                                 void* d_wpk, void* d_out16, float* d_out32, void* d_pool16, const float* d_wmap, int* d_oflow,
                                 char* kernel_name, void* stream);
+
+int amx_conv3d_deep_probe(const void* d_x0, int c0, const void* d_x1, int c1, const float* d_weight, const float* d_scale,
+                          const float* d_shift, int cout, int n, int d, int hh, int w, int act, float slope, int precision,
+                          void* d_wpk, void* d_scratch, size_t scratch_bytes, void* d_out16, int* d_oflow, char* kernel_names,
+                          void* stream);
 
 size_t amx_conv3d_scratch_bytes(int c0, int c1, int cout, int n, int d, int hh, int w, int precision);
 int amx_conv3d_k3_reflect_ws(const void* d_x0, int c0, const void* d_x1, int c1, const float* d_weight,
```
